# yancie-yjr/StreamYOLO

Hardware: AMD Instinct MI355X
Metric: frame-pairs/sec (600x960) StreamYOLO-l fwd+bwd (higher is better)
Workload: dtype bf16; 1 GPU; StreamYOLO-l 600x960 training step: dual-frame forward + TAL loss + backward, 8 frame pairs/GPU/step, random-init synthetic weights (utils/synth.py); per_gpu_batch=8, global_batch=8, parallelism=dp1, hipgraph=False, launch_tape=True, optimizer_in_step=False, u8_input=False

## Files before the change

include/streamyolo_hip.h:

```cpp
#ifndef STREAMYOLO_HIP_H
#define STREAMYOLO_HIP_H

#include <stdint.h>

#ifdef __cplusplus
extern "C" {
#endif

#define SY_ABI_VERSION 7
#define SY_API __attribute__((visibility("default")))

enum { SY_DT_BF16 = 0, SY_DT_F16 = 1, SY_DT_F32 = 2 };

enum {
    SY_EPI_LINEAR = 0,
    SY_EPI_SILU = 1,
    SY_EPI_SIGMOID = 2,
    SY_EPI_DECODE = 3,
    SY_EPI_BNR = 4
};

enum { SY_TILE_AUTO = 0, SY_TILE_256x256 = 1, SY_TILE_128x256 = 2, SY_TILE_128x128 = 3, SY_TILE_64x256 = 4, SY_TILE_32x256 = 5,
       SY_TILE_128x64 = 6, SY_TILE_64x64 = 7, SY_TILE_256x64 = 8, SY_TILE_256x128 = 9,
       SY_TILE_RS = 16,
       SY_TILE_DMA2 = 32,
       SY_TILE_DMA3 = 48,
       SY_TILE_WR = 80,
       SY_TILE_HALO = 112,
       SY_TILE_1X1K = 121  };

enum {
    SY_CONV_FWD = 0,
    SY_CONV_DGRAD = 1
};

typedef struct sy_conv_desc {
    const void* x;
    const void* w;
    const float* scale;
    const float* shift;
    const void* res;
    void* y;
    float* stat_sum;
    float* stat_sqsum;
    int32_t N, H, W, Cin;
    int32_t Ho, Wo, Cout;
    int32_t KH, KW, stride, pad;
    int32_t ldx, ldy, ldr;
    int64_t xbs, ybs, rbs;
    int32_t dtype;
    int32_t y_f32;
    int32_t mode;
    int32_t epilogue;
    int32_t accumulate;
    float dec_stride;
    int32_t stat_copies;
    int32_t stat_segments;
    int32_t tile;
    int64_t x_bytes, w_bytes;
    const void* wfrag;
    int64_t wfrag_bytes;
    int32_t k_splits;
    int32_t pre_cin;
    const void* pre_w;
    int64_t pre_w_bytes;
    const float* pre_scale;
    const float* pre_shift;
} sy_conv_desc;

SY_API int sy_conv2d(const sy_conv_desc* d, void* stream);

typedef struct sy_wgrad_desc {
    const void* x;  const void* dy;  float* dw;
    int32_t N, H, W, Cin, Ho, Wo, Cout, KH, KW, stride, pad;
    int32_t ldx, lddy;  int64_t xbs, dybs;
    int32_t dtype;
    int32_t dw_oihw;
    void* workspace;
    int64_t workspace_bytes;
    int32_t tile, target_blocks;
    int64_t x_bytes, dy_bytes;
} sy_wgrad_desc;
SY_API int sy_conv2d_wgrad(const sy_wgrad_desc* d, void* stream);

SY_API int sy_focus_pack(const float* in, int N, int Ctot, int c0, int H, int W, void* out, int dtype, void* stream);

enum { SY_FRAMES_NCHW = 0, SY_FRAMES_FOCUS = 1 };
SY_API int sy_frames_u8_pack(const uint8_t* cur, const uint8_t* sup, int B, int Hs, int Ws, int64_t image_stride,
                             int row_stride, int decimate, const uint8_t* mirror, int H, int W, int Ho, int Wo,
                             int layout, void* out_cur, void* out_sup, int dtype, void* stream);

SY_API int sy_resize_bilinear_nchw(const float* in, int N, int C, int H, int W, float* out, int Ho, int Wo, void* stream);

SY_API int sy_resize_nearest(const void* in, int N, int Hi, int Wi, int C, int ldi, int64_t ibs,
                      void* out, int Ho, int Wo, int ldo, int64_t obs, int dtype, void* stream);

SY_API int sy_spp_pool(void* buf, int N, int H, int W, int C, int ld, int64_t bs, void* argmax, int dtype,
                       void* stream);

SY_API int sy_head_decode(float* out, int B, int A, int nch, const int32_t* level_h, const int32_t* level_w,
                          const float* level_stride, int nlevels, int flags, void* stream);

SY_API int64_t sy_postprocess_workspace_bytes(int B, int A);
SY_API int sy_postprocess(const float* pred, int B, int A, int num_classes, float conf_thre, float nms_thre,
                   int max_det, float* out_det, int32_t* out_index, int32_t* out_count,
                   void* workspace, void* stream);

typedef struct sy_optim_entry {
    float* p;
    const float* g;
    float* buf;
    float* ema;
    int64_t n;
    float weight_decay;
    float lr_mult;
    int32_t chunk0;
    int32_t reserved;
} sy_optim_entry;
SY_API int sy_sgd_ema_step(const sy_optim_entry* entries, int n_entries, int total_chunks, float lr, float momentum,
                           float grad_scale, float ema_decay, int first_step, void* stream);

typedef struct sy_scaler_state {
    float scale;
    float inv_scale;
    int32_t growth_tracker;
    int32_t found_inf;
    int32_t steps_taken;
    int32_t steps_skipped;
    int32_t reserved[2];
} sy_scaler_state;
SY_API int sy_grad_nonfinite(const sy_optim_entry* entries, int n_entries, int total_chunks, void* scaler_state, void* stream);
SY_API int sy_sgd_ema_step_scaled(const sy_optim_entry* entries, int n_entries, int total_chunks, float lr, float momentum,
                                  float extra_scale, float ema_decay, const void* scaler_state, void* stream);
SY_API int sy_loss_scale_update(void* scaler_state, float growth_factor, float backoff_factor, int growth_interval, void* stream);

typedef struct sy_pack_entry {
    const float* w;
    void* packed;
    void* packed_t;
    void* frag;
    void* frag_t;
    int32_t co_n, ci_n, taps, r0, R, R_t, CI, dtype;
    int32_t tile0;
    int32_t reserved;
} sy_pack_entry;
SY_API int sy_pack_weights(const sy_pack_entry* entries, int n_entries, int total_tiles, void* stream);

SY_API int sy_bn_finalize(const float* sum, const float* sqsum, int C, int copies, double count, const float* gamma,
                   const float* beta, float eps, float momentum, float* running_mean,
                   float* running_var, float* scale, float* shift, float* mean, float* invstd,
                   int nseg, void* stream);
typedef struct sy_bn_running_entry {
    float* running_mean;
    float* running_var;
    const float* sum[2];
    const float* sqsum[2];
    double count[2];
    int32_t C, copies, calls;
    float momentum;
    int32_t ld;
    int32_t reserved;
    int64_t* num_batches_tracked;
} sy_bn_running_entry;
SY_API int sy_bn_running_update(const sy_bn_running_entry* entries, int n_entries, int max_C, void* stream);
SY_API int sy_bn_finalize_apply(const float* sum, const float* sqsum, int copies, double count, const float* gamma,
                                const float* beta, float eps, float* scale, float* shift, float* mean, float* invstd,
                                const void* y, int ldy, const void* res, int ldr, void* out, int ldo, int64_t pixels, int C,
                                int dtype, int nseg, void* stream);

SY_API int sy_bn_silu_apply(const void* y, int ldy, const float* scale, const float* shift, const void* res,
                     int ldr, void* out, int ldo, int64_t pixels, int C, int dtype, int nseg, void* stream);
SY_API int sy_bn_silu_bwd_reduce(const void* y, int ldy, const void* da, int ldda, const float* scale,
                                 const float* shift, const float* mean, const float* invstd, float* sums,
                                 int copies, int64_t pixels, int C, int dtype, int nseg, void* stream);
SY_API int sy_bn_silu_bwd_apply(const void* y, int ldy, const void* da, int ldda, const float* scale,
                                const float* shift, const float* mean, const float* invstd,
                                const float* gamma, const float* sums, int copies, void* dy, int lddy,
                                int64_t pixels, int C, float* dgamma, float* dbeta, void* dres, int lddres,
                                int dres_accumulate, int dtype, int nseg, void* stream);

SY_API int64_t sy_tal_loss_workspace_bytes(int B, int A, int max_gt);
SY_API int sy_tal_loss(const float* raw, int B, int A, int num_classes, const float* labels,
                       const float* support, int max_labels, const int32_t* level_h,
                       const int32_t* level_w, const float* level_stride, int nlevels, float gamma,
                       float ignore_thr, float ignore_value, int use_l1, float* d_raw, float* losses,
                       int32_t* fg_mask, void* workspace, void* d_pad, int pad_dtype, void* stream);
SY_API int sy_tal_loss_scaled(const float* raw, int B, int A, int num_classes, const float* labels,
                              const float* support, int max_labels, const int32_t* level_h,
                              const int32_t* level_w, const float* level_stride, int nlevels, float gamma,
                              float ignore_thr, float ignore_value, int use_l1, float* d_raw, float* losses,
                              int32_t* fg_mask, void* workspace, void* d_pad, int pad_dtype, const void* scaler_state,
                              void* stream);

SY_API int sy_tal_loss_assignment(const void* workspace, int B, int A, int max_labels, int32_t* matched_gt,
                                  float* matched_iou, void* stream);

SY_API int sy_bn_grid_caps(const int32_t* set4, int32_t* get4);

SY_API int sy_zero_rows(void* ptr, int64_t rows, int64_t row_bytes, int64_t pitch_bytes, void* stream);

SY_API int sy_view_copy(const void* in, int ldi, void* out, int ldo, int64_t pixels, int C, int dtype,
                 int accumulate, void* stream);

SY_API int sy_stream_state_gather(const void* cur, int ld_cur, int64_t cur_bs, const void* pool, int n_slots, void* sup,
                                  int ld_sup, int64_t sup_bs, int B, int H, int W, int C, const int32_t* row_slot,
                                  const uint8_t* row_first, int dtype, void* stream);
typedef struct sy_stream_level {
    const void* cur;
    void* pool;
    int64_t bs;
    int32_t H, W, C, ld;
} sy_stream_level;
SY_API int sy_stream_state_scatter(const sy_stream_level* levels, int n_levels, int n_slots, int B, const int32_t* row_slot,
                                   int dtype, void* stream);

SY_API int sy_resize_nearest_bwd(const void* dout, int N, int Ho, int Wo, int C, int lddo, int64_t dobs,
                          void* din, int Hi, int Wi, int lddi, int64_t dibs, int accumulate,
                          int dtype, void* stream);
SY_API int sy_spp_pool_bwd(void* dbuf, const void* argmax, int N, int H, int W, int C, int ld, int64_t bs,
                    int dtype, void* stream);

SY_API int sy_splitk_epilogue(const float* part, int splits, int64_t pixels, int C, const float* scale, const float* shift,
                              const void* res, int ldr, void* y, int ldy, int dtype, int epilogue, void* stream);

SY_API int sy_rows_add_f32(float* dst, int64_t ldd, float* src, int64_t lds, int rows, int cols, int zero_src, void* stream);
SY_API int64_t sy_pred_grad_fold_workspace_floats(int num_classes);
SY_API int sy_pred_grad_fold(const float* d_raw, int B, int64_t batch_stride, int rows, int num_classes, float* scratch,
                             int scratch_rows, int ld, int cin, float* g_reg, float* g_obj, float* g_cls, float* gb_reg, float* gb_obj, float* gb_cls,
                             float* workspace, void* stream);

enum { SY_TAPE_END = -1, SY_TAPE_LAUNCH = 0,
       SY_TAPE_SIDE = 1,
       SY_TAPE_FORK = 2,
       SY_TAPE_SIDE_NW = 3,
       SY_TAPE_MAIN = 4,
       SY_TAPE_ACQUIRE = 5,
       SY_TAPE_JOIN = 6,
       SY_TAPE_BREAK = 7,
       SY_TAPE_BUCKET = 8,
       SY_TAPE_CUR = 9,
       SY_TAPE_DEP = 10,
       SY_TAPE_SLOT_DONE = 11,
       SY_TAPE_ACQUIRE_CUR = 12   };
SY_API void* sy_tape_begin(void);
SY_API int sy_tape_mark(int kind, int arg);
SY_API void* sy_tape_end(void);
SY_API int sy_tape_size(const void* tape, int* n_entries, int* n_launches);
SY_API int sy_tape_counters(const void* tape, int* n_events, int* n_waits);
SY_API int sy_tape_replay(void* tape, void* main_stream, void* side_stream, int* pos, int stop_buckets, int* stop_kind,
                          int* stop_arg, int* stop_on_side);
SY_API int sy_tape_replay_n(void* tape, void* const* streams, int n_streams, int* pos, int stop_buckets, int* stop_kind,
                            int* stop_arg, int* stop_stream);
SY_API void sy_tape_free(void* tape);

SY_API const char* sy_version(void);
SY_API int sy_abi_version(void);

#ifdef __cplusplus
}
#endif
#endif
```

streamyolo_amd/_lib.py:

```python
import ctypes as C
import os

_HERE = os.path.dirname(os.path.abspath(__file__))
DEFAULT_PATH = os.path.join(_HERE, "lib", "libstreamyolo_hip.so")

DT_BF16, DT_F16, DT_F32 = 0, 1, 2
EPI_LINEAR, EPI_SILU, EPI_SIGMOID, EPI_DECODE, EPI_BNR = 0, 1, 2, 3, 4
CONV_FWD, CONV_DGRAD = 0, 1

ABI_VERSION = 7
_ERR = {1: "bad argument", 2: "kernel launch failed", 3: "unsupported shape"}
SY_ERR_UNSUPPORTED = 3


class HipLibraryError(RuntimeError):
    pass


class ConvDesc(C.Structure):
    _fields_ = [
        ("x", C.c_void_p), ("w", C.c_void_p), ("scale", C.c_void_p), ("shift", C.c_void_p),
        ("res", C.c_void_p), ("y", C.c_void_p), ("stat_sum", C.c_void_p), ("stat_sqsum", C.c_void_p),
        ("N", C.c_int32), ("H", C.c_int32), ("W", C.c_int32), ("Cin", C.c_int32),
        ("Ho", C.c_int32), ("Wo", C.c_int32), ("Cout", C.c_int32),
        ("KH", C.c_int32), ("KW", C.c_int32), ("stride", C.c_int32), ("pad", C.c_int32),
        ("ldx", C.c_int32), ("ldy", C.c_int32), ("ldr", C.c_int32),
        ("xbs", C.c_int64), ("ybs", C.c_int64), ("rbs", C.c_int64),
        ("dtype", C.c_int32), ("y_f32", C.c_int32), ("mode", C.c_int32), ("epilogue", C.c_int32),
        ("accumulate", C.c_int32), ("dec_stride", C.c_float), ("stat_copies", C.c_int32), ("stat_segments", C.c_int32), ("tile", C.c_int32), ("x_bytes", C.c_int64), ("w_bytes", C.c_int64), ("wfrag", C.c_void_p), ("wfrag_bytes", C.c_int64),
        ("k_splits", C.c_int32), ("pre_cin", C.c_int32), ("pre_w", C.c_void_p), ("pre_w_bytes", C.c_int64),
        ("pre_scale", C.c_void_p), ("pre_shift", C.c_void_p),
    ]


class BnRunningEntry(C.Structure):
    _fields_ = [("running_mean", C.c_void_p), ("running_var", C.c_void_p), ("sum", C.c_void_p * 2),
                ("sqsum", C.c_void_p * 2), ("count", C.c_double * 2), ("C", C.c_int32), ("copies", C.c_int32),
                ("calls", C.c_int32), ("momentum", C.c_float), ("ld", C.c_int32), ("reserved", C.c_int32),
                ("num_batches_tracked", C.c_void_p)]


class PackEntry(C.Structure):
    _fields_ = [("w", C.c_void_p), ("packed", C.c_void_p), ("packed_t", C.c_void_p), ("frag", C.c_void_p),
                ("frag_t", C.c_void_p), ("co_n", C.c_int32), ("ci_n", C.c_int32), ("taps", C.c_int32),
                ("r0", C.c_int32), ("R", C.c_int32), ("R_t", C.c_int32), ("CI", C.c_int32), ("dtype", C.c_int32),
                ("tile0", C.c_int32), ("reserved", C.c_int32)]


class ScalerState(C.Structure):
    _fields_ = [("scale", C.c_float), ("inv_scale", C.c_float), ("growth_tracker", C.c_int32), ("found_inf", C.c_int32),
                ("steps_taken", C.c_int32), ("steps_skipped", C.c_int32), ("reserved", C.c_int32 * 2)]


class OptimEntry(C.Structure):
    _fields_ = [("p", C.c_void_p), ("g", C.c_void_p), ("buf", C.c_void_p), ("ema", C.c_void_p), ("n", C.c_int64),
                ("weight_decay", C.c_float), ("lr_mult", C.c_float), ("chunk0", C.c_int32), ("reserved", C.c_int32)]


class StreamLevel(C.Structure):
    _fields_ = [("cur", C.c_void_p), ("pool", C.c_void_p), ("bs", C.c_int64), ("H", C.c_int32), ("W", C.c_int32),
                ("C", C.c_int32), ("ld", C.c_int32)]


def pack_table(rows):
    t = 0
    for e in rows:
        e.tile0 = t
        t += -(-e.co_n // 32) * -(-e.ci_n // 32)
    return (PackEntry * len(rows))(*rows), t


class WgradDesc(C.Structure):
    _fields_ = [
        ("x", C.c_void_p), ("dy", C.c_void_p), ("dw", C.c_void_p),
        ("N", C.c_int32), ("H", C.c_int32), ("W", C.c_int32), ("Cin", C.c_int32),
        ("Ho", C.c_int32), ("Wo", C.c_int32), ("Cout", C.c_int32),
        ("KH", C.c_int32), ("KW", C.c_int32), ("stride", C.c_int32), ("pad", C.c_int32),
        ("ldx", C.c_int32), ("lddy", C.c_int32), ("xbs", C.c_int64), ("dybs", C.c_int64),
        ("dtype", C.c_int32), ("dw_oihw", C.c_int32), ("workspace", C.c_void_p), ("workspace_bytes", C.c_int64), ("tile", C.c_int32), ("target_blocks", C.c_int32), ("x_bytes", C.c_int64), ("dy_bytes", C.c_int64),
    ]


_P, _I, _L, _F, _D = C.c_void_p, C.c_int, C.c_int64, C.c_float, C.c_double

SIGNATURES = {
    "sy_conv2d": (_I, [C.POINTER(ConvDesc), _P]),
    "sy_conv2d_wgrad": (_I, [C.POINTER(WgradDesc), _P]),
    "sy_focus_pack": (_I, [_P, _I, _I, _I, _I, _I, _P, _I, _P]),
    "sy_frames_u8_pack": (_I, [_P, _P, _I, _I, _I, _L, _I, _I, _P, _I, _I, _I, _I, _I, _P, _P, _I, _P]),
    "sy_resize_bilinear_nchw": (_I, [_P, _I, _I, _I, _I, _P, _I, _I, _P]),
    "sy_resize_nearest": (_I, [_P, _I, _I, _I, _I, _I, _L, _P, _I, _I, _I, _L, _I, _P]),
    "sy_resize_nearest_bwd": (_I, [_P, _I, _I, _I, _I, _I, _L, _P, _I, _I, _I, _L, _I, _I, _P]),
    "sy_spp_pool": (_I, [_P, _I, _I, _I, _I, _I, _L, _P, _I, _P]),
    "sy_spp_pool_bwd": (_I, [_P, _P, _I, _I, _I, _I, _I, _L, _I, _P]),
    "sy_postprocess_workspace_bytes": (_L, [_I, _I]),
    "sy_head_decode": (_I, [_P, _I, _I, _I, _P, _P, _P, _I, _I, _P]),
    "sy_postprocess": (_I, [_P, _I, _I, _I, _F, _F, _I, _P, _P, _P, _P, _P]),
    "sy_sgd_ema_step": (_I, [_P, _I, _I, _F, _F, _F, _F, _I, _P]),
    "sy_grad_nonfinite": (_I, [_P, _I, _I, _P, _P]),
    "sy_sgd_ema_step_scaled": (_I, [_P, _I, _I, _F, _F, _F, _F, _P, _P]),
    "sy_loss_scale_update": (_I, [_P, _F, _F, _I, _P]),
    "sy_pack_weights": (_I, [_P, _I, _I, _P]),
    "sy_bn_running_update": (_I, [_P, _I, _I, _P]),
    "sy_bn_finalize": (_I, [_P, _P, _I, _I, _D, _P, _P, _F, _F, _P, _P, _P, _P, _P, _P, _I, _P]),
    "sy_bn_silu_apply": (_I, [_P, _I, _P, _P, _P, _I, _P, _I, _L, _I, _I, _I, _P]),
    "sy_bn_finalize_apply": (_I, [_P, _P, _I, _D, _P, _P, _F, _P, _P, _P, _P, _P, _I, _P, _I, _P, _I, _L, _I, _I, _I, _P]),
    "sy_bn_silu_bwd_reduce": (_I, [_P, _I, _P, _I, _P, _P, _P, _P, _P, _I, _L, _I, _I, _I, _P]),
    "sy_bn_silu_bwd_apply": (_I, [_P, _I, _P, _I, _P, _P, _P, _P, _P, _P, _I, _P, _I, _L, _I, _P, _P, _P, _I, _I, _I, _I, _P]),
    "sy_tal_loss_workspace_bytes": (_L, [_I, _I, _I]),
    "sy_tal_loss": (_I, [_P, _I, _I, _I, _P, _P, _I, _P, _P, _P, _I, _F, _F, _F, _I, _P, _P, _P, _P, _P, _I, _P]),
    "sy_tal_loss_scaled": (_I, [_P, _I, _I, _I, _P, _P, _I, _P, _P, _P, _I, _F, _F, _F, _I, _P, _P, _P, _P, _P, _I, _P, _P]),
    "sy_tal_loss_assignment": (_I, [_P, _I, _I, _I, _P, _P, _P]),
    "sy_zero_rows": (_I, [_P, _L, _L, _L, _P]),
    "sy_bn_grid_caps": (_I, [C.POINTER(C.c_int32), C.POINTER(C.c_int32)]),
    "sy_view_copy": (_I, [_P, _I, _P, _I, _L, _I, _I, _I, _P]),
    "sy_stream_state_gather": (_I, [_P, _I, _L, _P, _I, _P, _I, _L, _I, _I, _I, _I, _P, _P, _I, _P]),
    "sy_stream_state_scatter": (_I, [_P, _I, _I, _I, _P, _I, _P]),
    "sy_splitk_epilogue": (_I, [_P, _I, _L, _I, _P, _P, _P, _I, _P, _I, _I, _I, _P]),
    "sy_rows_add_f32": (_I, [_P, _L, _P, _L, _I, _I, _I, _P]),
    "sy_pred_grad_fold_workspace_floats": (_L, [_I]),
    "sy_pred_grad_fold": (_I, [_P, _I, _L, _I, _I, _P, _I, _I, _I, _P, _P, _P, _P, _P, _P, _P, _P]),
    "sy_tape_begin": (_P, []),
    "sy_tape_mark": (_I, [_I, _I]),
    "sy_tape_end": (_P, []),
    "sy_tape_size": (_I, [_P, C.POINTER(C.c_int), C.POINTER(C.c_int)]),
    "sy_tape_counters": (_I, [_P, C.POINTER(C.c_int), C.POINTER(C.c_int)]),
    "sy_tape_replay": (_I, [_P, _P, _P, C.POINTER(C.c_int), _I, C.POINTER(C.c_int), C.POINTER(C.c_int), C.POINTER(C.c_int)]),
    "sy_tape_replay_n": (_I, [_P, C.POINTER(C.c_void_p), _I, C.POINTER(C.c_int), _I, C.POINTER(C.c_int), C.POINTER(C.c_int),
                               C.POINTER(C.c_int)]),
    "sy_tape_free": (None, [_P]),
    "sy_version": (C.c_char_p, []),
    "sy_abi_version": (_I, []),
}

_lib = None
_lib_path = None


def _bind(path):
    if not os.path.exists(path):
        raise HipLibraryError(
            "streamyolo_amd: %s not found. The MI355X kernels are the ONLY implementation of this "
            "package (no CPU/eager fallback). Build them: make -C streamyolo_amd/csrc" % path)
    lib = C.CDLL(path)
    for name, (res, args) in SIGNATURES.items():
        try:
            fn = getattr(lib, name)
        except AttributeError as e:
            raise HipLibraryError("streamyolo_amd: %s lacks symbol %s (stale build?)" % (path, name)) from e
        fn.restype = res
        fn.argtypes = args
    if lib.sy_abi_version() != ABI_VERSION:
        raise HipLibraryError("streamyolo_amd: ABI version mismatch in %s" % path)
    return lib


def lib():
    global _lib, _lib_path
    if _lib is None:
        path = os.environ.get("STREAMYOLO_HIP_LIB") or DEFAULT_PATH
        _lib = _bind(path)
        _lib_path = path
    return _lib if _tape is None else _TapeProxy(_lib, _tape)


_tape = None


class _TapeProxy:
    __slots__ = ("real", "tape")

    def __init__(self, real, tape):
        self.real, self.tape = real, tape

    def __getattr__(self, name):
        fn = getattr(self.real, name)
        tape = self.tape
        if name.endswith("_supported") or name.endswith("_bytes") or name.endswith("_floats") or name.endswith("version") or name.endswith("_caps") or name.startswith("sy_tape_"):
            return fn

        def call(*args):
            tape.append((fn, args[:-1], name))
            return fn(*args)
        return call


class record:

    def __enter__(self):
        global _tape
        assert _tape is None, "launch tapes do not nest"
        lib()
        _tape = []
        return _tape

    def __exit__(self, *exc):
        global _tape
        _tape = None
        return False


def replay(tape, stream):
    for fn, args, name in tape:
        rc = fn(*args, stream)
        if rc != 0:
            check(rc, name)


TAPE_END, TAPE_LAUNCH, TAPE_SIDE, TAPE_FORK, TAPE_SIDE_NW, TAPE_MAIN, TAPE_ACQUIRE, TAPE_JOIN, TAPE_BREAK, TAPE_BUCKET = \
    -1, 0, 1, 2, 3, 4, 5, 6, 7, 8
TAPE_CUR, TAPE_DEP, TAPE_SLOT_DONE, TAPE_ACQUIRE_CUR = 9, 10, 11, 12
TAPE_MARKS = {"side": TAPE_SIDE, "fork": TAPE_FORK, "side_nw": TAPE_SIDE_NW, "main": TAPE_MAIN, "acquire": TAPE_ACQUIRE,
              "join": TAPE_JOIN, "bucket": TAPE_BUCKET, "cur": TAPE_CUR, "dep": TAPE_DEP, "slot_done": TAPE_SLOT_DONE,
              "acquire_cur": TAPE_ACQUIRE_CUR}


class NativeTape:

    def __init__(self):
        self.handle, self.snippets, self._lib = None, [], lib()
        self._pos, self._kind, self._arg, self._side = C.c_int(0), C.c_int(0), C.c_int(0), C.c_int(0)

    def __enter__(self):
        assert _tape is None, "a Python launch tape is open"
        if not self._lib.sy_tape_begin():
            raise HipLibraryError("streamyolo_amd: sy_tape_begin failed (a recording is already open on this thread)")
        return self

    def __exit__(self, et, ev, tb):
        h = self._lib.sy_tape_end()
        if et is not None:
            self._lib.sy_tape_free(h)
        else:
            self.handle = h
        return False

    def mark(self, name, arg=None):
        if name == "dep":
            arg = arg[0] * 16 + arg[1]
        check(self._lib.sy_tape_mark(TAPE_MARKS[name], -1 if arg is None else int(arg)), "sy_tape_mark")

    def snippet(self, fn):
        self.snippets.append(fn)
        check(self._lib.sy_tape_mark(TAPE_BREAK, len(self.snippets) - 1), "sy_tape_mark")

    def size(self):
        n, l = C.c_int(0), C.c_int(0)
        check(self._lib.sy_tape_size(self.handle, C.byref(n), C.byref(l)), "sy_tape_size")
        return n.value, l.value

    def counters(self):
        e, w = C.c_int(0), C.c_int(0)
        check(self._lib.sy_tape_counters(self.handle, C.byref(e), C.byref(w)), "sy_tape_counters")
        return e.value, w.value

    def replay(self, main, side=None, on_snippet=None, on_bucket=None, more=()):
        fn, h = self._lib.sy_tape_replay_n, self.handle
        pos, kind, arg, ons = self._pos, self._kind, self._arg, self._side
        pos.value = 0
        stop_b = 0 if on_bucket is None else 1
        lst = [main] + ([side] if side is not None else []) + (list(more) if side is not None else [])
# ... 58 lines not shown
```

streamyolo_amd/csrc/conv_igemm.hip:

```cpp
#include "conv_igemm_impl.h"

using sy_conv::ConvArgs;
int sy_conv_launch_bf16(const ConvArgs& a, void* stream);
int sy_conv_launch_f16(const ConvArgs& a, void* stream);
int sy_conv_launch_f32(const ConvArgs& a, void* stream);

constexpr long long kWtMinBytes = 8ll << 20;

extern "C" int sy_conv2d(const sy_conv_desc* d, void* stream) {
    if (d == nullptr || d->x == nullptr || d->w == nullptr || d->y == nullptr) return SY_ERR_ARG;
    if (d->N <= 0 || d->Cin <= 0 || d->Cout <= 0 || d->Ho <= 0 || d->Wo <= 0) return SY_ERR_ARG;
    if (d->dtype < SY_DT_BF16 || d->dtype > SY_DT_F32) return SY_ERR_ARG;
    const int epc = d->dtype == SY_DT_F32 ? 4 : 8;
    if (d->Cin % epc != 0 || d->ldx % epc != 0) return SY_ERR_UNSUPPORTED;
    if (d->stride != 1 && d->stride != 2) return SY_ERR_UNSUPPORTED;
    if (d->KH < 1 || d->KW < 1 || d->KH * d->KW > 49) return SY_ERR_UNSUPPORTED;
    if ((d->stat_sum == nullptr) != (d->stat_sqsum == nullptr)) return SY_ERR_ARG;
    if (d->epilogue < SY_EPI_LINEAR || d->epilogue > SY_EPI_BNR) return SY_ERR_ARG;
    if (d->epilogue == SY_EPI_BNR) {
        if (d->mode != SY_CONV_DGRAD || d->accumulate || d->y_f32 || d->dtype == SY_DT_F32 || d->res == nullptr || d->scale == nullptr ||
            d->shift == nullptr || d->stat_sum == nullptr || d->ldr != d->ldy || d->rbs != d->ybs || d->stat_segments > 1)
            return SY_ERR_UNSUPPORTED;
        const int t = d->tile & 0xff;
        if (t != 98 && t != 100 && t != 101 && t != 109 && t != 104 && t != 107 && t != 117 && t != 118) return SY_ERR_UNSUPPORTED;
        if (d->KH != 3 || d->stride != 1 || (d->ldy & 7) != 0 || (d->Cout & 7) != 0) return SY_ERR_UNSUPPORTED;
        if ((((uintptr_t)d->y | (uintptr_t)d->res) & 15) != 0 || (d->ybs & 7) != 0) return SY_ERR_UNSUPPORTED;
    }
    if ((long long)d->N * d->Ho * d->Wo > 0x7fffffffLL) return SY_ERR_UNSUPPORTED;
    ConvArgs a;
    a.x = (const unsigned char*)d->x; a.w = (const unsigned char*)d->w;
    a.scale = d->scale; a.shift = d->shift; a.res = (const unsigned char*)d->res; a.y = (unsigned char*)d->y;
    a.stat_sum = d->stat_sum; a.stat_sq = d->stat_sqsum;
    a.N = d->N; a.H = d->H; a.W = d->W; a.Cin = d->Cin; a.Ho = d->Ho; a.Wo = d->Wo; a.Cout = d->Cout;
    a.KH = d->KH; a.KW = d->KW; a.stride = d->stride; a.pad = d->pad;
    a.ldx = d->ldx; a.ldy = d->ldy; a.ldr = d->ldr; a.xbs = d->xbs; a.ybs = d->ybs; a.rbs = d->rbs;
    a.y_f32 = d->y_f32; a.mode = d->mode; a.epilogue = d->epilogue; a.accumulate = d->accumulate;
    a.dec_stride = d->dec_stride;
    a.stat_copies = d->stat_copies > 0 ? d->stat_copies : 1;
    a.seg_M = 0;
    a.s2_classes = 0;
    if (d->stat_segments > 1) {
        if (d->stat_sum == nullptr || d->N % d->stat_segments != 0 || d->mode != SY_CONV_FWD) return SY_ERR_ARG;
        a.seg_M = (d->N / d->stat_segments) * d->Ho * d->Wo;
    }
    a.x_extent = (d->x_bytes > 0 && d->x_bytes < 0xFFFFFFF0LL) ? (unsigned)d->x_bytes : 0u;
    a.w_extent = (d->w_bytes > 0 && d->w_bytes < 0xFFFFFFF0LL) ? (unsigned)d->w_bytes : 0u;
    a.wfrag = (const unsigned char*)d->wfrag;
    a.wfrag_extent = (d->wfrag != nullptr && d->wfrag_bytes > 0 && d->wfrag_bytes < 0xFFFFFFF0LL) ? (unsigned)d->wfrag_bytes : 0u;
    a.pre_w = (const unsigned char*)d->pre_w; a.pre_scale = d->pre_scale; a.pre_shift = d->pre_shift; a.pre_cin = d->pre_cin;
    a.pre_w_extent = (d->pre_w != nullptr && d->pre_w_bytes > 0 && d->pre_w_bytes < 0xFFFFFFF0LL) ? (unsigned)d->pre_w_bytes : 0u;
    if ((d->pre_w != nullptr) != ((d->tile & 0xff) == 119)) return SY_ERR_ARG;
    a.ksplit = 0;
    if (d->k_splits > 1) {
        if (((d->tile & 0xff) != 117 && (d->tile & 0xff) != 118) || d->mode != SY_CONV_FWD || !d->y_f32 || d->epilogue != SY_EPI_LINEAR ||
            d->scale != nullptr || d->shift != nullptr || d->res != nullptr || d->stat_sum != nullptr || d->accumulate || d->k_splits > 16)
            return SY_ERR_UNSUPPORTED;
        a.ksplit = d->k_splits;
    }
    {
        static const long long wt_min = [] { const char* e = std::getenv("SY_WT_MIN_BYTES"); return e ? std::atoll(e) : (long long)kWtMinBytes; }();
        const long long out_bytes = (long long)d->N * d->Ho * d->Wo * d->Cout * (d->y_f32 ? 4 : (d->dtype == SY_DT_F32 ? 4 : 2));
        a.wt = out_bytes >= wt_min ? 1 : 0;
    }
    a.tile = d->tile & 0xff;
    a.ablate = (d->tile >> 8) & 1023;
    a.HoWo = d->Ho * d->Wo; a.M = d->N * a.HoWo; a.K = d->KH * d->KW * d->Cin;
    switch (d->dtype) {
        case SY_DT_BF16: return sy_conv_launch_bf16(a, stream);
        case SY_DT_F16: return sy_conv_launch_f16(a, stream);
        default: return sy_conv_launch_f32(a, stream);
    }
}
```

streamyolo_amd/csrc/conv_igemm_impl.h:

```cpp
#pragma once
#include "sy_device.h"
#include "../../include/streamyolo_hip.h"

namespace sy_conv {

struct ConvArgs {
    const unsigned char* x;
    const unsigned char* w;
    const float* scale;
    const float* shift;
    const unsigned char* res;
    unsigned char* y;
    float* stat_sum;
    float* stat_sq;
    int N, H, W, Cin, Ho, Wo, Cout, KH, KW, stride, pad;
    int ldx, ldy, ldr;
    long long xbs, ybs, rbs;
    int y_f32, mode, epilogue, accumulate;
    float dec_stride;
    int M, K, HoWo;
    int stat_copies;
    int seg_M;
    int s2_classes;
    int tile;
    unsigned x_extent, w_extent;
    const unsigned char* wfrag;
    unsigned wfrag_extent;
    const unsigned char* pre_w;
    unsigned pre_w_extent;
    const float* pre_scale;
    const float* pre_shift;
    int pre_cin;
    int ksplit;
    int wt;
    int ablate;
};

template <int WC, int WP, int TC, int TP> struct StageLimit { static constexpr size_t kBytes = 48 * 1024; };

template <int WP, int CT> struct EpiLds { static constexpr int kStatBytes = WP * CT * 8; };

constexpr int kRowB = 64;
constexpr int kPitchRS = 80;

static __device__ uint4 g_zero16[4] = {};

struct LinearPixels {
    int m0, m_end, cls_hw, Wc, Wo, cls_ph, cls_pw, s2, seg, rep;
    template <typename Args> __device__ __forceinline__ LinearPixels(const Args& p, int by, int bz, int PT) {
        cls_ph = 0; cls_pw = 0; Wc = p.Wo; Wo = p.Wo; s2 = p.s2_classes;
        int Hc = p.Ho, cls_M = p.M;
        if (p.s2_classes) {
            cls_ph = bz >> 1; cls_pw = bz & 1;
            Hc = (p.Ho - cls_ph + 1) >> 1; Wc = (p.Wo - cls_pw + 1) >> 1;
            cls_M = p.N * Hc * Wc;
        }
        cls_hw = Hc * Wc;
        m_end = p.seg_M > 0 ? (bz + 1) * p.seg_M : cls_M;
        m0 = (p.s2_classes ? 0 : bz * p.seg_M) + by * PT;
        seg = bz; rep = by;
    }
    __device__ __forceinline__ bool map(int lp, int& n, int& rem) const {
        const int m = m0 + lp;
        if (m >= m_end) { n = 0; rem = 0; return false; }
        n = m / cls_hw;
        rem = m - n * cls_hw;
        if (s2) { const int i2 = rem / Wc; rem = (2 * i2 + cls_ph) * Wo + 2 * (rem - i2 * Wc) + cls_pw; }
        return true;
    }
};
struct TilePixels {
    int n, h0, w0, Ho, Wo, seg, rep;
    __device__ __forceinline__ bool map(int lp, int& n_, int& rem) const {
        const int h = h0 + (lp >> 5), w = w0 + (lp & 31);
        n_ = n;
        if (h >= Ho || w >= Wo) { rem = 0; return false; }
        rem = h * Wo + w;
        return true;
    }
};

template <typename T, int WC, int WP, int TC, int TP, typename Args, typename Map>
__device__ __forceinline__ void conv_epilogue(const Args& p, const Map& mp, int bx, f32x16 (&acc)[TC][TP],
                                              unsigned char* smem, int tid);

template <typename T, int WC, int WP, int TC, int TP, int STG, int FAST>
__global__ __launch_bounds__(WC * WP * 64, ((TC * TP <= 4 && !(STG == 6 && TC * TP == 4)) ? 4 : 2)) void conv_igemm_kernel(ConvArgs p) {
    SY_TL_BEGIN(1 + (p.mode == SY_CONV_DGRAD ? 32 : 0));
    typedef typename T::elem elem;
    constexpr int RS = (STG == 1 || STG == 5 || STG == 6) ? 1 : 0;
    constexpr int WR = (STG == 5 || STG == 6) ? 1 : 0;
    constexpr int WR3 = (STG == 6) ? 1 : 0;
    constexpr int kStages = RS ? 1 : (STG == 0 ? 4 : STG);
    constexpr int kThreads = WC * WP * 64;
    constexpr int RPI = kThreads / 4;
    constexpr int EPC = T::kEPC;
    constexpr int ESZ = 16 / EPC;
    constexpr int BK = 4 * EPC;
    constexpr int CT = WC * TC * 32;
    constexpr int PT = WP * TP * 32;
    constexpr int WCH = (CT * 4 + kThreads - 1) / kThreads;
    constexpr int XCH = (PT * 4 + kThreads - 1) / kThreads;
    static_assert(WC * WP == 4 || WC * WP == 8, "4 or 8 waves per workgroup");
    static_assert(PT % RPI == 0, "every wave stages pixel rows");

    SY_DYN_SMEM(smem);
    unsigned char* const sW = smem;
    unsigned char* const sX = smem + (WR ? 0 : (RS ? CT * kPitchRS : kStages * CT * kRowB));

    const int tid = threadIdx.x;
    const int lane = tid & 63;
    const int wave = tid >> 6;
    const int wc = wave / WP;
    const int wp = wave % WP;
    const sy_block_id bid = sy_xcd_block_id();
    const int c0 = bid.x * CT;
    int cls_ph = 0, cls_pw = 0, Hc = p.Ho, Wc = p.Wo, cls_M = p.M;
    if (p.s2_classes) {
// ... 675 lines not shown
                if (l31 == 16) {
                    red[(wp * CT + cl) * 2 + 0] = a;
                    red[(wp * CT + cl) * 2 + 1] = b;
                }
            }
        }
    });
    if (want_stats || (kCanStage && stage_out)) __syncthreads();
    sy_probe(4);
    if (kCanStage && stage_out && !p.accumulate) {
        constexpr int CPR = CT / 8;
        constexpr int NCH = (PT * CPR + kThreads - 1) / kThreads;
        constexpr int UB = NCH < 5 ? NCH : 5;
#pragma unroll 1
        for (int b0 = 0; b0 < NCH; b0 += UB) {
            uint4 v[UB];
            long long off[UB];
#pragma unroll
            for (int k = 0; k < UB; ++k) {
                const int i = tid + (b0 + k) * kThreads;
                const int ck = i % CPR;
                const bool ok = i < PT * CPR && c0 + ck * 8 < p.Cout;
                const int px = ok ? i / CPR : 0;
                const long long o_ = stg_off[px];
                v[k] = *reinterpret_cast<const uint4*>(stg + px * kStagePitch + ck * 16);
                off[k] = ok ? o_ : -1;
            }
#pragma unroll
            for (int k = 0; k < UB; ++k) {
                const int i = tid + (b0 + k) * kThreads;
                const int ck = i % CPR;
                if (off[k] >= 0) {
                    if (SY_WT_CONV && p.wt) sy_store16_wt(reinterpret_cast<elem*>(p.y) + off[k] + c0 + ck * 8, v[k]);
                    else *reinterpret_cast<uint4*>(reinterpret_cast<elem*>(p.y) + off[k] + c0 + ck * 8) = v[k];
                }
            }
        }
    } else if (kCanStage && stage_out) {
        constexpr int CPR = CT / 8;
        for (int i = tid; i < PT * CPR; i += kThreads) {
            const int px = i / CPR, ck = i - px * CPR;
            const long long off = stg_off[px];
            const int co = c0 + ck * 8;
            if (off < 0 || co >= p.Cout) continue;
            uint4 v = *reinterpret_cast<const uint4*>(stg + px * kStagePitch + ck * 16);
            uint4* const dst = reinterpret_cast<uint4*>(reinterpret_cast<elem*>(p.y) + off + co);
            if (p.accumulate) {
                const uint4 o = *dst;
                elem ev[8], eo[8];
                __builtin_memcpy(ev, &v, 16);
                __builtin_memcpy(eo, &o, 16);
                unsigned w[4];
#pragma unroll
                for (int j = 0; j < 4; ++j)
                    w[j] = T::pack2(T::to_f32(ev[2 * j]) + T::to_f32(eo[2 * j]), T::to_f32(ev[2 * j + 1]) + T::to_f32(eo[2 * j + 1]));
                v = make_uint4(w[0], w[1], w[2], w[3]);
            }
            if (SY_WT_CONV && p.wt) sy_store16_wt(dst, v); else *dst = v;
        }
    }
    sy_probe(5);
    if (bnr && lean) {
        const float* red = reinterpret_cast<const float*>(smem);
        float* const dst = p.stat_sum + (long long)((unsigned)mp.rep % (unsigned)p.stat_copies) * 2 * p.Cout;
        for (int cl = tid; cl < CT; cl += kThreads) {
            const int co = c0 + cl;
            if (co >= p.Cout) continue;
            float a = 0.0f, b = 0.0f;
#pragma unroll
            for (int w = 0; w < WP; ++w) { a += red[(w * CT + cl) * 2]; b += red[(w * CT + cl) * 2 + 1]; }
            atomicAdd(dst + co, a);
            atomicAdd(dst + p.Cout + co, b);
        }
    }
    if (want_stats && !(p.ablate & 8)) {
        const float* red = reinterpret_cast<const float*>(smem);
        const int copy = mp.seg * p.stat_copies + (int)((unsigned)mp.rep % (unsigned)p.stat_copies);
        for (int cl = tid; cl < CT; cl += kThreads) {
            const int co = c0 + cl;
            if (co >= p.Cout) continue;
            float a = 0.0f, b = 0.0f;
#pragma unroll
            for (int w = 0; w < WP; ++w) { a += red[(w * CT + cl) * 2]; b += red[(w * CT + cl) * 2 + 1]; }
            atomicAdd(p.stat_sum + (long long)copy * p.Cout + co, a);
            atomicAdd(p.stat_sq + (long long)copy * p.Cout + co, b);
        }
    }
}

template <typename T, int WC, int WP, int TC, int TP, int STG, int FAST>
int launch_one(const ConvArgs& a, void* stream) {
    constexpr int RS = (STG == 1 || STG == 5 || STG == 6) ? 1 : 0;
    constexpr int kStages = RS ? 1 : (STG == 0 ? 4 : STG);
    constexpr int CT = WC * TC * 32, PT = WP * TP * 32;
    const int nseg = a.seg_M > 0 ? a.M / a.seg_M : 1;
    dim3 grid((a.Cout + CT - 1) / CT, ((a.seg_M > 0 ? a.seg_M : a.M) + PT - 1) / PT, nseg);
    if (a.s2_classes) grid = dim3(grid.x, (a.N * ((a.Ho + 1) / 2) * ((a.Wo + 1) / 2) + PT - 1) / PT, 4);
    constexpr size_t smem_k = (STG == 6) ? (size_t)(2 * PT * kPitchRS > WP * CT * 8 ? 2 * PT * kPitchRS : WP * CT * 8)
                              : (STG == 5) ? (size_t)(PT * kPitchRS > WP * CT * 8 ? PT * kPitchRS : WP * CT * 8)
                                         : (RS ? (size_t)(CT + PT) * kPitchRS : (size_t)kStages * (CT + PT) * kRowB);
    constexpr size_t smem_e = (size_t)EpiLds<WP, CT>::kStatBytes + (size_t)PT * (CT * 2 + 16) + (size_t)PT * 8;
    constexpr size_t smem = (T::kEPC == 8 && smem_e <= 48 * 1024 && smem_e > smem_k) ? smem_e : smem_k;
#ifndef SY_EMU
    static sy_dev_once attr_done;
    if (attr_done.need()) {
        if (hipFuncSetAttribute((const void*)conv_igemm_kernel<T, WC, WP, TC, TP, STG, FAST>,
                                hipFuncAttributeMaxDynamicSharedMemorySize, (int)smem) != hipSuccess)
            return SY_ERR_LAUNCH;
        attr_done.mark();
    }
#endif
    SY_LAUNCH((conv_igemm_kernel<T, WC, WP, TC, TP, STG, FAST>), grid, dim3(WC * WP * 64), smem, stream, a);
    return SY_LAUNCH_OK() == 0 ? SY_OK : SY_ERR_LAUNCH;
}

template <typename T, int WC, int WP, int TC, int TP, int STG = 0>
int launch_cfg(const ConvArgs& a_in, void* stream) {
    ConvArgs a = a_in;
    const bool fast = (a.Cin % (4 * T::kEPC) == 0) && a.x_extent != 0 && a.w_extent != 0 && a.KH * a.KW <= 32;
    a.s2_classes = (fast && a.mode != SY_CONV_FWD && a.stride == 2 && a.KH >= 2 && a.KW >= 2 && !(a_in.ablate & 4)) ? 1 : 0;
    if constexpr (STG == 5 || STG == 6) {
        if (fast && a.wfrag != nullptr && a.wfrag_extent != 0) return launch_one<T, WC, WP, TC, TP, STG, 1>(a, stream);
        return fast ? launch_one<T, WC, WP, TC, TP, 1, 1>(a, stream) : launch_one<T, WC, WP, TC, TP, 1, 0>(a, stream);
    } else {
        return fast ? launch_one<T, WC, WP, TC, TP, STG, 1>(a, stream) : launch_one<T, WC, WP, TC, TP, STG, 0>(a, stream);
    }
}

template <typename T> int launch_halo_typed(const ConvArgs& a, void* stream);
template <typename T> int launch_halo3_typed(const ConvArgs& a, void* stream);
template <typename T> int launch_s2dgrad(const ConvArgs& a, void* stream);
template <typename T> int launch_s2dgrad4(const ConvArgs& a, void* stream);
template <typename T> int launch_1x1_tile(const ConvArgs& a, void* stream);
template <typename T> int launch_bottleneck_fused(const ConvArgs& a, void* stream);

template <typename T>
int launch_typed(const ConvArgs& a, void* stream) {
    if ((a.tile >= 104 && a.tile <= 107) || (a.tile >= 110 && a.tile <= 118)) return launch_halo_typed<T>(a, stream);
    if (a.tile == 109 || (a.tile >= 96 && a.tile <= 98) || a.tile == 100 || a.tile == 101) return launch_halo3_typed<T>(a, stream);
    if (a.tile == 119) return launch_bottleneck_fused<T>(a, stream);
    if (a.tile == 108) return launch_s2dgrad<T>(a, stream);
    if (a.tile >= 125 && a.tile <= 127) return launch_s2dgrad4<T>(a, stream);
    if (a.tile >= 121 && a.tile <= 124) return launch_1x1_tile<T>(a, stream);
    switch (a.tile) {
        case SY_TILE_256x256: return launch_cfg<T, 2, 4, 4, 2>(a, stream);
        case SY_TILE_128x256: return launch_cfg<T, 1, 8, 4, 1>(a, stream);
        case SY_TILE_128x128: return launch_cfg<T, 2, 2, 2, 2>(a, stream);
        case SY_TILE_64x256: return launch_cfg<T, 1, 4, 2, 2>(a, stream);
        case SY_TILE_32x256: return launch_cfg<T, 1, 4, 1, 2>(a, stream);
        case SY_TILE_128x64: return launch_cfg<T, 4, 1, 1, 2>(a, stream);
        case SY_TILE_64x64: return launch_cfg<T, 2, 2, 1, 1>(a, stream);
        case SY_TILE_RS + SY_TILE_128x64: return launch_cfg<T, 4, 1, 1, 2, 1>(a, stream);
        case SY_TILE_RS + SY_TILE_64x64: return launch_cfg<T, 2, 2, 1, 1, 1>(a, stream);
        case 32 + SY_TILE_128x128: return launch_cfg<T, 2, 2, 2, 2, 2>(a, stream);
        case 32 + SY_TILE_128x64: return launch_cfg<T, 4, 1, 1, 2, 2>(a, stream);
        case 32 + SY_TILE_64x64: return launch_cfg<T, 2, 2, 1, 1, 2>(a, stream);
        case 32 + SY_TILE_64x256: return launch_cfg<T, 1, 4, 2, 2, 2>(a, stream);
        case 48 + SY_TILE_128x128: return launch_cfg<T, 2, 2, 2, 2, 3>(a, stream);
        case 48 + SY_TILE_128x64: return launch_cfg<T, 4, 1, 1, 2, 3>(a, stream);
        case 48 + SY_TILE_64x64: return launch_cfg<T, 2, 2, 1, 1, 3>(a, stream);
        case 48 + SY_TILE_64x256: return launch_cfg<T, 1, 4, 2, 2, 3>(a, stream);
        case SY_TILE_RS + SY_TILE_256x64: return launch_cfg<T, 4, 1, 2, 2, 1>(a, stream);
        case 80 + SY_TILE_256x64: return launch_cfg<T, 4, 1, 2, 2, 5>(a, stream);
        case 80 + SY_TILE_256x128: return launch_cfg<T, 4, 1, 2, 4, 5>(a, stream);
        case 80 + SY_TILE_128x128: return launch_cfg<T, 2, 2, 2, 2, 5>(a, stream);
        case 80 + SY_TILE_128x64: return launch_cfg<T, 4, 1, 1, 2, 5>(a, stream);
        case 96 + SY_TILE_128x64: return launch_cfg<T, 4, 1, 1, 2, 6>(a, stream);
        case 96 + SY_TILE_64x64: return launch_cfg<T, 2, 2, 1, 1, 6>(a, stream);
// ... 21 lines not shown
```

streamyolo_amd/csrc/sy_device.h:

```cpp
#pragma once

#ifdef SY_EMU
#include "simt_emu.h"
#define SY_DYN_SMEM(name) unsigned char* name = emu::g_blk->dyn_smem
#include "sy_tape.h"
#include <tuple>
#define SY_LAUNCH(kernel, grid, block, smem, stream, ...)                                                            \
    do {                                                                                                             \
        const dim3 sy_grid_ = (grid), sy_block_ = (block);                                                           \
        const size_t sy_smem_ = (smem);                                                                              \
        auto sy_args_ = std::make_tuple(__VA_ARGS__);                            \
        auto sy_launch_fn_ = [=](void*) {                                                                            \
            emu::launch(sy_grid_, sy_block_, sy_smem_,                                                               \
                        [=]() { std::apply([](auto... sy_a_) { kernel(sy_a_...); }, sy_args_); });                   \
        };                                                                                                           \
        if (sy_tape_recording()) sy_tape_push(std::function<void(void*)>(sy_launch_fn_));                            \
        sy_launch_fn_(nullptr);                                                                                      \
    } while (0)
#define SY_LAUNCH_OK() 0
#else
#include <hip/hip_runtime.h>
#include <hip/hip_ext.h>
#define SY_DYN_SMEM(name) extern __shared__ __attribute__((aligned(16))) unsigned char name[]
#include "sy_tape.h"
// ... 288 lines not shown
        const float send = b2 ? A : B;
        w2[m] = (b2 ? B : A) + sy_mov_dpp<0x114, 0xA>(sy_mov_dpp<0x104, 0x5>(0.0f, send), send);
    }
    const float A = w2[0], B = w2[1];
    const float send = b3 ? A : B;
    const float r = (b3 ? B : A) + sy_mov_dpp<0x118, 0xC>(sy_mov_dpp<0x108, 0x3>(0.0f, send), send);
    return r + __shfl_xor(r, 16);
}
#endif

#ifdef SY_EMU
static inline void sy_sched_fence() {}
#else
__device__ __forceinline__ void sy_sched_fence() { __builtin_amdgcn_sched_barrier(0); }
#endif

#ifdef SY_EMU
static inline int sy_uniform(int v) { return v; }
#else
__device__ __forceinline__ int sy_uniform(int v) { return __builtin_amdgcn_readfirstlane(v); }
#endif

#ifdef SY_EMU
static inline unsigned long long sy_readlane64(unsigned long long v, int l) { return __shfl(v, l); }
#else
__device__ __forceinline__ unsigned long long sy_readlane64(unsigned long long v, int l) {
    const unsigned lo = __builtin_amdgcn_readlane((unsigned)v, l), hi = __builtin_amdgcn_readlane((unsigned)(v >> 32), l);
    return ((unsigned long long)hi << 32) | lo;
}
#endif

#ifndef SY_WT_STORES
#define SY_WT_STORES 1
#endif
#ifndef SY_WT_CONV
#define SY_WT_CONV 1
#endif
#ifndef SY_WT_BNF
#define SY_WT_BNF 1
#endif
#ifndef SY_WT_BNB
#define SY_WT_BNB 1
#endif
#ifndef SY_WT_SLAB
#define SY_WT_SLAB 0
#endif
#ifndef SY_WT_FOLD
#define SY_WT_FOLD 0
#endif
#ifndef SY_WT_ZERO
#define SY_WT_ZERO 0
#endif
#if defined(SY_EMU) || !SY_WT_STORES
static inline __host__ __device__ void sy_store16_wt(void* dst, const uint4& v) { *reinterpret_cast<uint4*>(dst) = v; }
static inline __host__ __device__ void sy_store8_wt(void* dst, const uint2& v) { *reinterpret_cast<uint2*>(dst) = v; }
static inline __host__ __device__ void sy_store4_wt(void* dst, unsigned v) { *reinterpret_cast<unsigned*>(dst) = v; }
#else
__device__ __forceinline__ void sy_store8_wt(void* dst, const uint2& v) {
    typedef unsigned v2u __attribute__((ext_vector_type(2)));
    v2u d;
    __builtin_memcpy(&d, &v, 8);
    asm volatile("global_store_dwordx2 %0, %1, off sc1" : : "v"(dst), "v"(d) : "memory");
}
__device__ __forceinline__ void sy_store4_wt(void* dst, unsigned v) {
    asm volatile("global_store_dword %0, %1, off sc1" : : "v"(dst), "v"(v) : "memory");
}
__device__ __forceinline__ void sy_store16_wt(void* dst, const uint4& v) {
    typedef unsigned v4u __attribute__((ext_vector_type(4)));
    v4u d;
    __builtin_memcpy(&d, &v, 16);
    asm volatile("global_store_dwordx4 %0, %1, off sc1\n\ts_nop 1" : : "v"(dst), "v"(d) : "memory");
}
#endif

#ifdef SY_EMU
static inline unsigned long long sy_uniform64(unsigned long long v) { return v; }
#else
__device__ __forceinline__ unsigned long long sy_uniform64(unsigned long long v) {
    const unsigned lo = __builtin_amdgcn_readfirstlane((unsigned)v), hi = __builtin_amdgcn_readfirstlane((unsigned)(v >> 32));
    return ((unsigned long long)hi << 32) | lo;
}
#endif

struct sy_block_id { int x, y, z; };
__device__ __forceinline__ sy_block_id sy_xcd_block_id() {
    constexpr unsigned kXcd = 8;
    const unsigned gx = gridDim.x, gy = gridDim.y, gz = gridDim.z;
    const unsigned nwg = gx * gy * gz;
    const unsigned w = blockIdx.x + gx * (blockIdx.y + gy * blockIdx.z);
    const unsigned k = w % kXcd, q = nwg / kXcd, r = nwg % kXcd;
    const unsigned L = k * q + (k < r ? k : r) + w / kXcd;
    sy_block_id b;
    b.x = (int)(L % gx);
    b.y = (int)((L / gx) % gy);
    b.z = (int)(L / (gx * gy));
    return b;
}

#if defined(SY_PROBE) && !defined(SY_EMU)
constexpr int kProbeWG = 8192, kProbeSlots = 8;
static __device__ unsigned long long sy_probe_buf[kProbeWG * kProbeSlots];
__device__ __forceinline__ void sy_probe(int slot) {
    if (threadIdx.x == 0) {
        const unsigned w = blockIdx.x + gridDim.x * (blockIdx.y + gridDim.y * blockIdx.z);
        if (w < (unsigned)kProbeWG) sy_probe_buf[w * kProbeSlots + slot] = __builtin_amdgcn_s_memrealtime();
    }
}
struct sy_tl_entry { unsigned long long key, t0, t1; unsigned tag, count; };
constexpr int kTlSlots = 65536;
static __device__ sy_tl_entry sy_tl[kTlSlots];
__device__ __forceinline__ int sy_tl_begin(unsigned tag) {
    const unsigned w = blockIdx.x + gridDim.x * (blockIdx.y + gridDim.y * blockIdx.z);
    const unsigned nwg = gridDim.x * gridDim.y * gridDim.z;
    const bool first = w == 0;
    const bool sample = first || (w & 15u) == 15u || w + 4u >= nwg;
    if (!sample || threadIdx.x != 0) return -1;
    const unsigned long long key = (unsigned long long)__builtin_amdgcn_kernarg_segment_ptr();
    const unsigned h = (unsigned)((key >> 6) * 2654435761ull) & (unsigned)(kTlSlots - 1);
    if (first) {
        const unsigned long long t = __builtin_amdgcn_s_memrealtime();
        const unsigned long long old = atomicCAS(&sy_tl[h].key, 0ull, key);
        if (old != 0ull && old != key) return -1;
        sy_tl[h].t0 = t;
        sy_tl[h].tag = tag;
        sy_tl[h].count = nwg;
        return (int)h;
    }
    return __hip_atomic_load(&sy_tl[h].key, __ATOMIC_RELAXED, __HIP_MEMORY_SCOPE_AGENT) == key ? (int)h : -1;
}
__device__ __forceinline__ void sy_tl_end(int slot) {
    if (slot >= 0) atomicMax(&sy_tl[slot].t1, (unsigned long long)__builtin_amdgcn_s_memrealtime());
}
#define SY_TL_BEGIN(tag) const int sy_tl_slot_ = sy_tl_begin(tag)
#define SY_TL_END() sy_tl_end(sy_tl_slot_)
#define SY_PROBE_READER(name)                                                                                          \
    extern "C" __attribute__((visibility("default"))) int name(unsigned long long* dst, int clear) {                 \
        if (hipMemcpyFromSymbol(dst, HIP_SYMBOL(sy_probe_buf), sizeof(sy_probe_buf)) != hipSuccess) return 2;          \
        if (clear) { static unsigned long long z[kProbeWG * kProbeSlots]; (void)hipMemcpyToSymbol(HIP_SYMBOL(sy_probe_buf), z, sizeof(z)); } \
        return 0;                                                                                                    \
    }                                                                                                                \
    extern "C" __attribute__((visibility("default"))) int name##_tl(void* dst, int clear) {                          \
        if (hipMemcpyFromSymbol(dst, HIP_SYMBOL(sy_tl), sizeof(sy_tl)) != hipSuccess) return 2;                       \
        if (clear) {                                                                                                 \
            static sy_tl_entry z[kTlSlots];                                                                          \
            for (int i = 0; i < kTlSlots; ++i) { z[i].key = 0; z[i].t0 = ~0ull; z[i].t1 = 0; z[i].tag = 0; z[i].count = 0; } \
            (void)hipMemcpyToSymbol(HIP_SYMBOL(sy_tl), z, sizeof(z));                                                \
        }                                                                                                            \
        return 0;                                                                                                    \
    }
#else
#define sy_probe(slot) ((void)0)
#define SY_PROBE_READER(name)
#define SY_TL_BEGIN(tag) ((void)0)
#define SY_TL_END() ((void)0)
#endif

#ifdef SY_EMU
#define SY_LATE_ARGS(Type, p) const Type& p##_late = (p)
#define SY_LAUNDER_INT(x) ((void)0)
#else
#define SY_LATE_ARGS(Type, p)                                                                                       \
    const __attribute__((address_space(4))) Type* p##_late_ptr =                                                     \
        (const __attribute__((address_space(4))) Type*)__builtin_amdgcn_kernarg_segment_ptr();                      \
    asm volatile("" : "+s"(p##_late_ptr));                                                                          \
    const __attribute__((address_space(4))) Type& p##_late = *p##_late_ptr
#define SY_LAUNDER_INT(x) asm volatile("" : "+s"(x))
// ... 29 lines not shown
```

streamyolo_amd/csrc/train_ops.hip:

```cpp
#include <stdlib.h>
#include "sy_pointwise.h"

#ifndef SY_BN_ROWS_IN_FLIGHT
#define SY_BN_ROWS_IN_FLIGHT 2
#endif

namespace {

template <typename T>
__global__ __launch_bounds__(kBlock) void spp_pool_kernel(typename T::elem* buf, int N, int H, int W, int C, int ld,
                                                          long long bs, unsigned char* argmax) {
    const int cpp = C / T::kEPC;
    const long long total = (long long)N * H * W * cpp;
    for (long long i = (long long)blockIdx.x * kBlock + threadIdx.x; i < total; i += (long long)gridDim.x * kBlock) {
        const int cc = (int)(i % cpp);
        long long pix = i / cpp;
        const int w = (int)(pix % W);
        const int h = (int)((pix / W) % H);
        const int n = (int)(pix / ((long long)W * H));
        float m5[T::kEPC], m9[T::kEPC], m13[T::kEPC];
        unsigned char a5[T::kEPC], a9[T::kEPC], a13[T::kEPC];
#pragma unroll
        for (int j = 0; j < T::kEPC; ++j) { m5[j] = -INFINITY; m9[j] = -INFINITY; m13[j] = -INFINITY; a5[j] = 0; a9[j] = 0; a13[j] = 0; }
        const typename T::elem* base = buf + n * bs + cc * T::kEPC;
// ... 207 lines not shown
        const int l = i / HW, p = i - l * HW;
        const int w = p % W, hr = p / W;
        const int r = 2 * (l + 1);
        float t[E];
        unsigned char rec[E];
#pragma unroll
        for (int j = 0; j < E; ++j) { t[j] = 0.0f; rec[j] = 0xFF; }
        for (int dh = -r; dh <= r; ++dh) {
            const int h = hr - dh;
            if (h < 0 || h >= H) continue;
            const int q = h * W + w;
            unsigned char cb[E];
            __builtin_memcpy(cb, s_am + ((size_t)q * 3 + l) * E, E);
            Chunk<T> g = Chunk<T>::load(s_g + ((size_t)q * 3 + l) * 16);
            const int code0 = (dh + 6) * 13;
#pragma unroll
            for (int j = 0; j < E; ++j) {
                const unsigned d = (unsigned)((int)cb[j] - code0);
                if (d < 13u) { t[j] += T::to_f32(g.e[j]); rec[j] = (unsigned char)d; }
            }
        }
        __builtin_memcpy(s_T + (size_t)i * E, t, sizeof(t));
        __builtin_memcpy(s_dw + (size_t)i * E, rec, E);
    }
    __syncthreads();
    for (int p = threadIdx.x; p < HW; p += nt) {
        const int x = p % W, row = p - x;
        elem* gslot0 = base + (long long)p * ld;
        Chunk<T> g0 = Chunk<T>::load(gslot0);
        float acc[E];
#pragma unroll
        for (int j = 0; j < E; ++j) acc[j] = T::to_f32(g0.e[j]);
#pragma unroll
        for (int l = 0; l < 3; ++l) {
            const int r = 2 * (l + 1);
            for (int dw = -r; dw <= r; ++dw) {
                const int w = x - dw;
                if (w < 0 || w >= W) continue;
                const size_t i = (size_t)l * HW + row + w;
                unsigned char rec[E];
                float t[E];
                __builtin_memcpy(rec, s_dw + i * E, E);
                __builtin_memcpy(t, s_T + i * E, sizeof(t));
#pragma unroll
                for (int j = 0; j < E; ++j)
                    if (rec[j] == (unsigned char)(dw + 6)) acc[j] += t[j];
            }
        }
        Chunk<T> o;
#pragma unroll
        for (int j = 0; j < E; ++j) o.e[j] = T::from_f32(acc[j]);
        o.store(gslot0);
    }
    SY_TL_END();
}

constexpr int kFoldTo = 32, kFoldAbove = 64;
__global__ __launch_bounds__(kBlock) void fold_rows_kernel(float* a0, float* a1, int C, int copies) {
    __shared__ float part[4][64];
    float* const arr = (blockIdx.z & 1) ? a1 : a0;
    float* const base = arr + (long long)(blockIdx.z >> 1) * copies * C;
    const int cl = threadIdx.x & 63, q = threadIdx.x >> 6;
    const int c = blockIdx.x * 64 + cl, r = blockIdx.y;
    float acc = 0.0f;
    if (c < C) {
        int j = q;
        const int J = (copies - r + kFoldTo - 1) / kFoldTo;
        for (; j + 12 < J; j += 16) {
            const float v0 = base[(long long)(r + kFoldTo * j) * C + c], v1 = base[(long long)(r + kFoldTo * (j + 4)) * C + c];
            const float v2 = base[(long long)(r + kFoldTo * (j + 8)) * C + c], v3 = base[(long long)(r + kFoldTo * (j + 12)) * C + c];
            acc += v0; acc += v1; acc += v2; acc += v3;
        }
        for (; j < J; j += 4) acc += base[(long long)(r + kFoldTo * j) * C + c];
    }
    part[q][cl] = acc;
    __syncthreads();
    if (q == 0 && c < C) base[(long long)r * C + c] = ((part[0][cl] + part[1][cl]) + part[2][cl]) + part[3][cl];
}

__global__ __launch_bounds__(kBlock) void bn_finalize_kernel(const float* sum, const float* sqsum, int C, int copies, int stride,
                                                             double count, const float* gamma, const float* beta,
                                                             float eps, float momentum, float* running_mean,
                                                             float* running_var, float* scale, float* shift,
                                                             float* mean_out, float* invstd_out) {
    SY_TL_BEGIN(11);
    __shared__ float s_s[8][32], s_q[8][32];
    const int cl = threadIdx.x & 31, rg = threadIdx.x >> 5;
    const int c = blockIdx.x * 32 + cl;
    {
        const long long so = (long long)blockIdx.y * stride * C, ao = (long long)blockIdx.y * C;
        sum += so; sqsum += so; scale += ao; shift += ao;
        if (mean_out != nullptr) mean_out += ao;
        if (invstd_out != nullptr) invstd_out += ao;
    }
    float s = 0.0f, q = 0.0f;
    if (c < C)
        for (int k = rg; k < copies; k += 8) { s += sum[(long long)k * C + c]; q += sqsum[(long long)k * C + c]; }
    s_s[rg][cl] = s;
    s_q[rg][cl] = q;
    __syncthreads();
    if (rg != 0 || c >= C) return;
    double ds = 0.0, dq = 0.0;
    for (int k = 0; k < 8; ++k) { ds += (double)s_s[k][cl]; dq += (double)s_q[k][cl]; }
    const double mean = ds / count;
    double var = dq / count - mean * mean;
    if (var < 0.0) var = 0.0;
    const float invstd = (float)(1.0 / sqrt(var + (double)eps));
    const float sc = gamma[c] * invstd;
    scale[c] = sc;
    shift[c] = beta[c] - (float)mean * sc;
    if (mean_out != nullptr) mean_out[c] = (float)mean;
    if (invstd_out != nullptr) invstd_out[c] = invstd;
    if (running_mean != nullptr) {
        const double unbiased = count > 1.0 ? var * count / (count - 1.0) : var;
        running_mean[c] = (1.0f - momentum) * running_mean[c] + momentum * (float)mean;
        running_var[c] = (1.0f - momentum) * running_var[c] + momentum * (float)unbiased;
    }
    SY_TL_END();
}

__global__ __launch_bounds__(kBlock) void bn_running_update_kernel(const sy_bn_running_entry* entries) {
    SY_TL_BEGIN(15);
    __shared__ float s_s[8][32], s_q[8][32];
    const sy_bn_running_entry e = entries[blockIdx.x];
    const int cl = threadIdx.x & 31, rg = threadIdx.x >> 5;
    const int c = blockIdx.y * 32 + cl;
    if ((int)blockIdx.y * 32 >= e.C) return;
    float rm = 0.0f, rv = 0.0f;
    const long long ld = e.ld > 0 ? e.ld : e.C;
    if (rg == 0 && c < e.C) { rm = e.running_mean[c]; rv = e.running_var[c]; }
    for (int j = 0; j < e.calls; ++j) {
        float s = 0.0f, q = 0.0f;
        if (c < e.C)
            for (int k = rg; k < e.copies; k += 8) { s += e.sum[j][k * ld + c]; q += e.sqsum[j][k * ld + c]; }
        s_s[rg][cl] = s;
        s_q[rg][cl] = q;
        __syncthreads();
        if (rg == 0 && c < e.C) {
            double ds = 0.0, dq = 0.0;
            for (int k = 0; k < 8; ++k) { ds += (double)s_s[k][cl]; dq += (double)s_q[k][cl]; }
            const double count = e.count[j];
            const double mean = ds / count;
            double var = dq / count - mean * mean;
            if (var < 0.0) var = 0.0;
            const double unbiased = count > 1.0 ? var * count / (count - 1.0) : var;
            rm = (1.0f - e.momentum) * rm + e.momentum * (float)mean;
            rv = (1.0f - e.momentum) * rv + e.momentum * (float)unbiased;
        }
        __syncthreads();
    }
    if (rg == 0 && c < e.C) { e.running_mean[c] = rm; e.running_var[c] = rv; }
    if (blockIdx.y == 0 && threadIdx.x == 0 && e.num_batches_tracked != nullptr) *e.num_batches_tracked += e.calls;
    SY_TL_END();
}

template <typename T>
__global__ __launch_bounds__(kBlock) void bn_silu_apply_kernel(const typename T::elem* y, int ldy, const float* scale,
                                                               const float* shift, const typename T::elem* res, int ldr,
                                                               typename T::elem* out, int ldo, long long pixels, int C) {
    SY_TL_BEGIN(10);
    const int cpp = C / T::kEPC;
    const int cc = threadIdx.x % cpp;
    const int c0 = cc * T::kEPC;
    const int rows = kBlock / cpp;
    if ((int)threadIdx.x >= rows * cpp) return;
    {
        const long long ro = (long long)blockIdx.y * pixels;
        y += ro * ldy; out += ro * ldo; scale += blockIdx.y * C; shift += blockIdx.y * C;
        if (res != nullptr) res += ro * ldr;
    }
    const long long step = (long long)gridDim.x * rows;
    long long pix = (long long)blockIdx.x * rows + threadIdx.x / cpp;
    constexpr int D = SY_BN_ROWS_IN_FLIGHT;
    Chunk<T> vq[D], rq[D];
#pragma unroll
    for (int d = 0; d < D; ++d) {
        const long long pd = pix + d * step;
        if (pd < pixels) {
            vq[d] = Chunk<T>::load(y + pd * ldy + c0);
            if (res != nullptr) rq[d] = Chunk<T>::load(res + pd * ldr + c0);
        }
    }
    float sc[T::kEPC], sh[T::kEPC];
#pragma unroll
    for (int j = 0; j < T::kEPC; ++j) { sc[j] = scale[c0 + j]; sh[j] = shift[c0 + j]; }
    for (; pix < pixels; pix += step) {
        const Chunk<T> v = vq[0], rv = rq[0];
#pragma unroll
        for (int d = 0; d + 1 < D; ++d) { vq[d] = vq[d + 1]; rq[d] = rq[d + 1]; }
        const long long nxt = pix + D * step;
        if (nxt < pixels) {
            vq[D - 1] = Chunk<T>::load(y + nxt * ldy + c0);
            if (res != nullptr) rq[D - 1] = Chunk<T>::load(res + nxt * ldr + c0);
        }
        Chunk<T> o;
        float r[T::kEPC];
#pragma unroll
        for (int j = 0; j < T::kEPC; ++j) r[j] = res != nullptr ? T::to_f32(rv.e[j]) : 0.0f;
#pragma unroll
        for (int j = 0; j < T::kEPC; ++j) o.e[j] = T::from_f32(sy_silu(T::to_f32(v.e[j]) * sc[j] + sh[j]) + r[j]);
        if constexpr (SY_WT_BNF) o.store_wt(out + pix * ldo + c0); else o.store(out + pix * ldo + c0);
    }
    SY_TL_END();
}

template <typename T>
__global__ __launch_bounds__(kBlock) void bn_finalize_apply_kernel(const float* sum, const float* sqsum, int copies, double count,
                                                                   const float* gamma, const float* beta, float eps,
                                                                   float* scale, float* shift, float* mean_out,
                                                                   float* invstd_out, const typename T::elem* y, int ldy,
                                                                   const typename T::elem* res, int ldr,
                                                                   typename T::elem* out, int ldo, long long pixels, int C,
                                                                   int CS) {
    SY_TL_BEGIN(10);
    __shared__ float s_part[2][8][64];
    __shared__ float s_aff[2][64];
    const int cpp = CS / T::kEPC;
    const int rows = kBlock / cpp;
    const int cc = threadIdx.x % cpp;
    const int cb = blockIdx.z * CS;
    const int c0 = cb + cc * T::kEPC;
    {
        const long long ro = (long long)blockIdx.y * pixels;
        const long long so = (long long)blockIdx.y * copies * C;
        const int ao = blockIdx.y * C;
        y += ro * ldy; out += ro * ldo;
        if (res != nullptr) res += ro * ldr;
        sum += so; sqsum += so; scale += ao; shift += ao; mean_out += ao; invstd_out += ao;
    }
    const bool live = (int)threadIdx.x < rows * cpp;
    const long long step = (long long)gridDim.x * rows;
    long long pix = (long long)blockIdx.x * rows + threadIdx.x / cpp;
    Chunk<T> v, rv, vn, rn;
    if (live && pix < pixels) {
        v = Chunk<T>::load(y + pix * ldy + c0);
        if (res != nullptr) rv = Chunk<T>::load(res + pix * ldr + c0);
    }
    for (int it = threadIdx.x; it < 2 * 8 * CS; it += kBlock) {
        const int c = it % CS, rg = (it / CS) & 7, kind = it / (8 * CS);
        const float* src = (kind ? sqsum : sum) + cb + c;
        float a = 0.0f;
        for (int k = rg; k < copies; k += 8) a += src[(long long)k * C];
        s_part[kind][rg][c] = a;
    }
    __syncthreads();
    if ((int)threadIdx.x < CS) {
        const int c = threadIdx.x;
        double ds = 0.0, dq = 0.0;
        for (int k = 0; k < 8; ++k) { ds += (double)s_part[0][k][c]; dq += (double)s_part[1][k][c]; }
        const double mean = ds / count;
        double var = dq / count - mean * mean;
        if (var < 0.0) var = 0.0;
        const float invstd = (float)(1.0 / sqrt(var + (double)eps));
        const float sc = gamma[cb + c] * invstd;
        const float sh = beta[cb + c] - (float)mean * sc;
        s_aff[0][c] = sc;
        s_aff[1][c] = sh;
        if (blockIdx.x == 0) {
            scale[cb + c] = sc; shift[cb + c] = sh; mean_out[cb + c] = (float)mean; invstd_out[cb + c] = invstd;
        }
    }
    __syncthreads();
    if (!live) return;
    float sc[T::kEPC], sh[T::kEPC];
#pragma unroll
    for (int j = 0; j < T::kEPC; ++j) { sc[j] = s_aff[0][cc * T::kEPC + j]; sh[j] = s_aff[1][cc * T::kEPC + j]; }
    for (; pix < pixels; pix += step) {
        const long long nxt = pix + step;
        if (nxt < pixels) {
            vn = Chunk<T>::load(y + nxt * ldy + c0);
            if (res != nullptr) rn = Chunk<T>::load(res + nxt * ldr + c0);
        }
        Chunk<T> o;
        float r[T::kEPC];
#pragma unroll
        for (int j = 0; j < T::kEPC; ++j) r[j] = res != nullptr ? T::to_f32(rv.e[j]) : 0.0f;
#pragma unroll
        for (int j = 0; j < T::kEPC; ++j) o.e[j] = T::from_f32(sy_silu(T::to_f32(v.e[j]) * sc[j] + sh[j]) + r[j]);
        if constexpr (SY_WT_BNF) o.store_wt(out + pix * ldo + c0); else o.store(out + pix * ldo + c0);
        v = vn; rv = rn;
    }
    SY_TL_END();
}

template <typename T>
__global__ __launch_bounds__(kBlock) void bn_silu_bwd_reduce_kernel(const typename T::elem* y, int ldy,
                                                                    const typename T::elem* da, int ldda,
                                                                    const float* scale, const float* shift,
                                                                    const float* mean, const float* invstd, float* sums,
                                                                    long long pixels, int C, int CS, int copies) {
    SY_TL_BEGIN(12);
    __shared__ float red[kBlock * 2 * 8];
    const int cpp = CS / T::kEPC;
    const int rows = kBlock / cpp;
    const int cc = threadIdx.x % cpp;
    const int pr = threadIdx.x / cpp;
    const int cb = blockIdx.z * CS;
    const int c0 = cb + cc * T::kEPC;
    {
        const long long ro = (long long)blockIdx.y * pixels;
        const int ao = blockIdx.y * C;
        y += ro * ldy; da += ro * ldda; scale += ao; shift += ao; mean += ao; invstd += ao;
        sums += (long long)blockIdx.y * copies * 2 * C;
    }
    sy_probe(0);
    const long long first = pr < rows ? (long long)blockIdx.x * rows + pr : pixels;
    const long long step = (long long)gridDim.x * rows;
    constexpr int D = SY_BN_ROWS_IN_FLIGHT;
    Chunk<T> yq[D], gq[D];
#pragma unroll
    for (int d = 0; d < D; ++d) {
        const long long pd = first + d * step;
        if (pd < pixels) { yq[d] = Chunk<T>::load(y + pd * ldy + c0); gq[d] = Chunk<T>::load(da + pd * ldda + c0); }
    }
    float sc[T::kEPC], sh[T::kEPC], mu[T::kEPC], is[T::kEPC], s0[T::kEPC], s1[T::kEPC];
#pragma unroll
    for (int j = 0; j < T::kEPC; ++j) {
        sc[j] = scale[c0 + j]; sh[j] = shift[c0 + j]; mu[j] = mean[c0 + j]; is[j] = invstd[c0 + j];
        s0[j] = 0.0f; s1[j] = 0.0f;
    }
    sy_probe(1);
    for (long long pix = first; pix < pixels; pix += step) {
        const Chunk<T> yv = yq[0], gv = gq[0];
#pragma unroll
        for (int d = 0; d + 1 < D; ++d) { yq[d] = yq[d + 1]; gq[d] = gq[d + 1]; }
        const long long nxt = pix + D * step;
        if (nxt < pixels) { yq[D - 1] = Chunk<T>::load(y + nxt * ldy + c0); gq[D - 1] = Chunk<T>::load(da + nxt * ldda + c0); }
#pragma unroll
        for (int j = 0; j < T::kEPC; ++j) {
            const float yy = T::to_f32(yv.e[j]);
            const float dz = T::to_f32(gv.e[j]) * sy_silu_grad(yy * sc[j] + sh[j]);
            s0[j] += dz;
            s1[j] += dz * ((yy - mu[j]) * is[j]);
        }
    }
    sy_probe(3);
#pragma unroll
    for (int j = 0; j < T::kEPC; ++j) {
        red[(j * 2 + 0) * kBlock + threadIdx.x] = s0[j];
        red[(j * 2 + 1) * kBlock + threadIdx.x] = s1[j];
    }
    __syncthreads();
    for (int t = threadIdx.x; t < cpp * T::kEPC * 2; t += kBlock) {
        const int kind = t & 1, j = (t >> 1) % T::kEPC, ch = (t >> 1) / T::kEPC;
        float v = 0.0f;
        for (int r = 0; r < rows; ++r) v += red[(j * 2 + kind) * kBlock + r * cpp + ch];
        atomicAdd(sums + (long long)(blockIdx.x % copies) * 2 * C + kind * C + cb + ch * T::kEPC + j, v);
    }
    sy_probe(6);
    SY_TL_END();
}

template <typename T>
__global__ __launch_bounds__(kBlock) void bn_silu_bwd_apply_kernel(const typename T::elem* y, int ldy,
                                                                   const typename T::elem* da, int ldda,
                                                                   const float* scale, const float* shift,
                                                                   const float* mean, const float* invstd,
                                                                   const float* gamma, const float* sums,
                                                                   typename T::elem* dy, int lddy, long long pixels,
                                                                   int C, int copies, float* dgamma, float* dbeta,
                                                                   long long seg_sum_stride, typename T::elem* dres,
                                                                   int lddres, int dres_acc) {
    SY_TL_BEGIN(13);
    __shared__ float s_fold[2 * 1024];
    {
        const long long ro = (long long)blockIdx.y * pixels;
        const int ao = blockIdx.y * C;
        y += ro * ldy; da += ro * ldda; dy += ro * lddy; scale += ao; shift += ao; mean += ao; invstd += ao;
        sums += blockIdx.y * seg_sum_stride;
        if (dres != nullptr) dres += ro * lddres;
    }
    const int cpp = C / T::kEPC;
    const int rows = kBlock / cpp;
    const int cc = threadIdx.x % cpp;
    const int c0 = cc * T::kEPC;
    const float inv_m = 1.0f / (float)pixels;
    const long long step = (long long)gridDim.x * rows;
    long long pix = (long long)blockIdx.x * rows + threadIdx.x / cpp;
    const bool live = (int)threadIdx.x < rows * cpp;
    constexpr int D = SY_BN_ROWS_IN_FLIGHT;
    Chunk<T> yq[D], gq[D];
#pragma unroll
    for (int d = 0; d < D; ++d) {
        const long long pd = pix + d * step;
        if (live && pd < pixels) { yq[d] = Chunk<T>::load(y + pd * ldy + c0); gq[d] = Chunk<T>::load(da + pd * ldda + c0); }
    }
    for (int i = threadIdx.x; i < 2 * C; i += kBlock) {
        float a = 0.0f;
        for (int k = 0; k < copies; ++k) a += sums[(long long)k * 2 * C + i];
        s_fold[i] = a;
    }
    __syncthreads();
    if (dres_acc & 4) {
        for (int c = threadIdx.x; c < C; c += kBlock)
            s_fold[C + c] = (float)((double)invstd[c] * ((double)s_fold[C + c] - (double)mean[c] * (double)s_fold[c]));
        __syncthreads();
    }
    if (blockIdx.x == 0 && dgamma != nullptr) {
        if (gridDim.y == 1 && !(dres_acc & 2)) {
            for (int c = threadIdx.x; c < C; c += kBlock) { dbeta[c] += s_fold[c]; dgamma[c] += s_fold[C + c]; }
        } else {
            for (int c = threadIdx.x; c < C; c += kBlock) { atomicAdd(dbeta + c, s_fold[c]); atomicAdd(dgamma + c, s_fold[C + c]); }
        }
    }
    if ((int)threadIdx.x >= rows * cpp) return;
    float sc[T::kEPC], sh[T::kEPC], mu[T::kEPC], is[T::kEPC], gi[T::kEPC], m0[T::kEPC], m1[T::kEPC];
#pragma unroll
    for (int j = 0; j < T::kEPC; ++j) {
        const int c = c0 + j;
        sc[j] = scale[c]; sh[j] = shift[c]; mu[j] = mean[c]; is[j] = invstd[c];
        gi[j] = gamma[c] * invstd[c];
        m0[j] = s_fold[c] * inv_m;
        m1[j] = s_fold[C + c] * inv_m;
    }
    for (; pix < pixels; pix += step) {
        Chunk<T> yv = yq[0], gv = gq[0];
#pragma unroll
        for (int d = 0; d + 1 < D; ++d) { yq[d] = yq[d + 1]; gq[d] = gq[d + 1]; }
        const long long nxt = pix + D * step;
        if (nxt < pixels) { yq[D - 1] = Chunk<T>::load(y + nxt * ldy + c0); gq[D - 1] = Chunk<T>::load(da + nxt * ldda + c0); }
        Chunk<T> o;
#pragma unroll
        for (int j = 0; j < T::kEPC; ++j) {
            const float yy = T::to_f32(yv.e[j]);
            const float dz = T::to_f32(gv.e[j]) * sy_silu_grad(yy * sc[j] + sh[j]);
            o.e[j] = T::from_f32(gi[j] * (dz - m0[j] - (yy - mu[j]) * is[j] * m1[j]));
        }
        if constexpr (SY_WT_BNB) o.store_wt(dy + pix * lddy + c0); else o.store(dy + pix * lddy + c0);
        if (dres != nullptr) {
            typename T::elem* dst = dres + pix * lddres + c0;
            if (dres_acc & 1) {
                Chunk<T> r = Chunk<T>::load(dst);
#pragma unroll
                for (int j = 0; j < T::kEPC; ++j) gv.e[j] = T::from_f32(T::to_f32(gv.e[j]) + T::to_f32(r.e[j]));
            }
            if constexpr (SY_WT_BNB) gv.store_wt(dst); else gv.store(dst);
        }
    }
    SY_TL_END();
}

__global__ __launch_bounds__(kBlock) void fold_replicas_kernel(float* sums, int n, int copies) {
    __shared__ float part[4][64];
    const int el = threadIdx.x & 63, q = threadIdx.x >> 6;
    const int i = blockIdx.x * 64 + el;
    sums += (long long)blockIdx.y * copies * n;
    float a = 0.0f;
    if (i < n) {
        int k = q;
        for (; k + 12 < copies; k += 16) {
            const float v0 = sums[(long long)k * n + i], v1 = sums[(long long)(k + 4) * n + i];
            const float v2 = sums[(long long)(k + 8) * n + i], v3 = sums[(long long)(k + 12) * n + i];
            a += v0; a += v1; a += v2; a += v3;
        }
        for (; k < copies; k += 4) a += sums[(long long)k * n + i];
    }
    part[q][el] = a;
    __syncthreads();
    if (q == 0 && i < n) sums[i] = ((part[0][el] + part[1][el]) + part[2][el]) + part[3][el];
}

inline bool chunk_rows_ok(int C, int e) { const int cpp = C / e; return cpp >= 1 && cpp <= kBlock; }

inline int env_cap(const char* name, int dflt) {
    const char* v = getenv(name);
    return (v != nullptr && atoi(v) > 0) ? atoi(v) : dflt;
}

enum { kCapApply = 0, kCapFApply = 1, kCapReduce = 2, kCapBApply = 3 };
inline std::atomic<int>& bn_cap(int which) {
    static std::atomic<int> caps[4] = {{env_cap("SY_BN_APPLY_BLOCKS", 2048)}, {env_cap("SY_BN_FAPPLY_BLOCKS", 2048)},
                                       {env_cap("SY_BN_REDUCE_BLOCKS", 768)}, {env_cap("SY_BN_BAPPLY_BLOCKS", 1024)}};
    return caps[which];
}

inline int row_grid(long long pixels, int C, int e, int cap) {
    const int rows = kBlock / (C / e);
    long long b = (pixels + rows - 1) / rows;
    if (b > cap) b = cap;
    if (b < 1) b = 1;
    return (int)b;
}

constexpr size_t kSppTileLds = 144 * 1024;
inline bool spp_force_scan() { const char* v = getenv("SY_SPP_SCAN"); return v != nullptr && v[0] == '1'; }
inline bool spp_lds_ok(const void* fn, int slot) {
#ifdef SY_EMU
    return true;
#else
    static sy_dev_once done[6];
    if (done[slot].need()) {
        if (hipFuncSetAttribute(fn, hipFuncAttributeMaxDynamicSharedMemorySize, (int)kSppTileLds) != hipSuccess) return false;
        done[slot].mark();
    }
    return true;
#endif
}

}

extern "C" int sy_bn_grid_caps(const int32_t* set4, int32_t* get4) {
    for (int k = 0; k < 4; ++k) {
        if (set4 != nullptr && set4[k] > 0) bn_cap(k).store(set4[k], std::memory_order_relaxed);
        if (get4 != nullptr) get4[k] = bn_cap(k).load(std::memory_order_relaxed);
    }
    return SY_OK;
}

extern "C" int sy_spp_pool(void* buf, int N, int H, int W, int C, int ld, int64_t bs, void* argmax, int dtype,
                           void* stream) {
    if (buf == nullptr || N <= 0 || C <= 0 || ld < 4 * C) return SY_ERR_ARG;
    const int e = epc_of(dtype);
    if (C % e || ld % e) return SY_ERR_UNSUPPORTED;
    const long long work = (long long)N * H * W * (C / e);
    const size_t tile_lds = (size_t)H * W * (16 + 3 * 16 + 3 * e);
    if (tile_lds <= kSppTileLds && !spp_force_scan()) {
        SY_DISPATCH_DTYPE(dtype, if (!spp_lds_ok((const void*)spp_pool_tile_kernel<T>, T::kCode)) return SY_ERR_LAUNCH;
                          SY_LAUNCH((spp_pool_tile_kernel<T>), dim3(N * (C / e), N * (C / e) < 256 ? 3 : 1), dim3(spp_tile_threads((long long)H * W)), tile_lds, stream,
                                    (typename T::elem*)buf, H, W, C, ld, (long long)bs, (unsigned char*)argmax));
    }
    SY_DISPATCH_DTYPE(dtype, SY_LAUNCH((spp_pool_kernel<T>), dim3(grid_for(work)), dim3(kBlock), 0, stream,
                                       (typename T::elem*)buf, N, H, W, C, ld, (long long)bs, (unsigned char*)argmax));
}

extern "C" int sy_spp_pool_bwd(void* dbuf, const void* argmax, int N, int H, int W, int C, int ld, int64_t bs, int dtype,
                               void* stream) {
    if (argmax == nullptr || dbuf == nullptr || N <= 0 || C <= 0 || ld < 4 * C) return SY_ERR_ARG;
    const int e = epc_of(dtype);
    if (C % e || ld % e) return SY_ERR_UNSUPPORTED;
    const long long work = (long long)N * H * W * (C / e);
    const size_t tile_lds = (size_t)H * W * 3 * (16 + e + 4 * e + e);
    if (tile_lds <= kSppTileLds && !spp_force_scan()) {
        SY_DISPATCH_DTYPE(dtype, if (!spp_lds_ok((const void*)spp_pool_bwd_tile_kernel<T>, 3 + T::kCode)) return SY_ERR_LAUNCH;
                          SY_LAUNCH((spp_pool_bwd_tile_kernel<T>), dim3(N * (C / e)), dim3(spp_tile_threads(3LL * H * W)), tile_lds, stream,
                                    (typename T::elem*)dbuf, (const unsigned char*)argmax, H, W, C, ld, (long long)bs));
    }
    SY_DISPATCH_DTYPE(dtype, SY_LAUNCH((spp_pool_bwd_kernel<T>), dim3(grid_for(work)), dim3(kBlock), 0, stream,
                                       (typename T::elem*)dbuf, (const unsigned char*)argmax, N, H, W, C, ld,
                                       (long long)bs));
}

extern "C" int sy_bn_finalize(const float* sum, const float* sqsum, int C, int copies, double count, const float* gamma,
                              const float* beta, float eps, float momentum, float* running_mean, float* running_var,
                              float* scale, float* shift, float* mean, float* invstd, int nseg, void* stream) {
    if (sum == nullptr || sqsum == nullptr || gamma == nullptr || beta == nullptr || scale == nullptr ||
        shift == nullptr || C <= 0 || copies <= 0 || count <= 0.0)
        return SY_ERR_ARG;
    if ((running_mean == nullptr) != (running_var == nullptr)) return SY_ERR_ARG;
    if (nseg < 1 || (nseg > 1 && running_mean != nullptr)) return SY_ERR_ARG;
    int read = copies;
    if (copies > kFoldAbove) {
        SY_LAUNCH(fold_rows_kernel, dim3((C + 63) / 64, kFoldTo, 2 * nseg), dim3(kBlock), 0, stream, const_cast<float*>(sum),
                  const_cast<float*>(sqsum), C, copies);
        read = kFoldTo;
    }
    SY_LAUNCH(bn_finalize_kernel, dim3((C + 31) / 32, nseg), dim3(kBlock), 0, stream, sum, sqsum, C, read, copies, count,
              gamma, beta, eps, momentum, running_mean, running_var, scale, shift, mean, invstd);
    return SY_LAUNCH_OK() == 0 ? SY_OK : SY_ERR_LAUNCH;
}

extern "C" int sy_bn_running_update(const sy_bn_running_entry* entries, int n_entries, int max_C, void* stream) {
    if (entries == nullptr || n_entries <= 0 || max_C <= 0) return SY_ERR_ARG;
    SY_LAUNCH(bn_running_update_kernel, dim3(n_entries, (max_C + 31) / 32), dim3(kBlock), 0, stream, entries);
    return SY_LAUNCH_OK() == 0 ? SY_OK : SY_ERR_LAUNCH;
}

extern "C" int sy_bn_silu_apply(const void* y, int ldy, const float* scale, const float* shift, const void* res, int ldr,
                                void* out, int ldo, int64_t pixels, int C, int dtype, int nseg, void* stream) {
    if (y == nullptr || out == nullptr || scale == nullptr || shift == nullptr || pixels <= 0 || C <= 0 || nseg < 1) return SY_ERR_ARG;
    const int e = epc_of(dtype);
    if (C % e || ldy % e || ldo % e || (res != nullptr && ldr % e)) return SY_ERR_UNSUPPORTED;
    if (!chunk_rows_ok(C, e)) return SY_ERR_UNSUPPORTED;
    const int cap_apply = bn_cap(kCapApply).load(std::memory_order_relaxed);
    SY_DISPATCH_DTYPE(dtype, SY_LAUNCH((bn_silu_apply_kernel<T>), dim3(row_grid(pixels, C, e, cap_apply / nseg), nseg), dim3(kBlock), 0, stream,
                                       (const typename T::elem*)y, ldy, scale, shift, (const typename T::elem*)res, ldr,
                                       (typename T::elem*)out, ldo, (long long)pixels, C));
}

extern "C" int sy_bn_finalize_apply(const float* sum, const float* sqsum, int copies, double count, const float* gamma,
                                    const float* beta, float eps, float* scale, float* shift, float* mean, float* invstd,
                                    const void* y, int ldy, const void* res, int ldr, void* out, int ldo, int64_t pixels, int C,
                                    int dtype, int nseg, void* stream) {
    if (sum == nullptr || sqsum == nullptr || gamma == nullptr || beta == nullptr || scale == nullptr || shift == nullptr ||
        mean == nullptr || invstd == nullptr || y == nullptr || out == nullptr || copies <= 0 || count <= 0.0 || pixels <= 0 ||
        C <= 0 || nseg < 1)
        return SY_ERR_ARG;
    const int e = epc_of(dtype);
    if (C % e || ldy % e || ldo % e || (res != nullptr && ldr % e)) return SY_ERR_UNSUPPORTED;
    int CS = C;
    for (int c = (64 / e) * e; c >= e; c -= e)
        if (c <= C && C % c == 0) { CS = c; break; }
    if (CS > 64) return SY_ERR_UNSUPPORTED;
    const int nsl = C / CS;
    const int cap_fa = bn_cap(kCapFApply).load(std::memory_order_relaxed);
    int cap = cap_fa / (nseg * nsl);
    if (cap < 1) cap = 1;
    SY_DISPATCH_DTYPE(dtype, SY_LAUNCH((bn_finalize_apply_kernel<T>), dim3(row_grid(pixels, CS, e, cap), nseg, nsl), dim3(kBlock), 0,
                                       stream, sum, sqsum, copies, count, gamma, beta, eps, scale, shift, mean, invstd,
                                       (const typename T::elem*)y, ldy, (const typename T::elem*)res, ldr,
                                       (typename T::elem*)out, ldo, (long long)pixels, C, CS));
}

extern "C" int sy_bn_silu_bwd_reduce(const void* y, int ldy, const void* da, int ldda, const float* scale,
                                     const float* shift, const float* mean, const float* invstd, float* sums,
                                     int copies, int64_t pixels, int C, int dtype, int nseg, void* stream) {
    if (y == nullptr || da == nullptr || sums == nullptr || pixels <= 0 || C <= 0 || copies <= 0 || nseg < 1) return SY_ERR_ARG;
    const int e = epc_of(dtype);
    if (C % e || ldy % e || ldda % e) return SY_ERR_UNSUPPORTED;
    if (!chunk_rows_ok(C, e)) return SY_ERR_UNSUPPORTED;
    const int cap_reduce = bn_cap(kCapReduce).load(std::memory_order_relaxed);
    static const int slice_max = env_cap("SY_BN_REDUCE_SLICE", 64);
    int CS = C;
    for (int c = (slice_max / e) * e; c >= e; c -= e)
        if (c <= C && C % c == 0) { CS = c; break; }
    const int nsl = C / CS;
    int cap = cap_reduce / (nseg * nsl);
    if (cap < 1) cap = 1;
    SY_DISPATCH_DTYPE(dtype, SY_LAUNCH((bn_silu_bwd_reduce_kernel<T>), dim3(row_grid(pixels, CS, e, cap), nseg, nsl), dim3(kBlock), 0, stream,
                                       (const typename T::elem*)y, ldy, (const typename T::elem*)da, ldda, scale, shift,
                                       mean, invstd, sums, (long long)pixels, C, CS, copies));
}

extern "C" int sy_bn_silu_bwd_apply(const void* y, int ldy, const void* da, int ldda, const float* scale,
                                    const float* shift, const float* mean, const float* invstd, const float* gamma,
                                    const float* sums, int copies, void* dy, int lddy, int64_t pixels, int C,
                                    float* dgamma, float* dbeta, void* dres, int lddres, int dres_accumulate, int dtype,
                                    int nseg, void* stream) {
    if (y == nullptr || da == nullptr || sums == nullptr || dy == nullptr || pixels <= 0 || C <= 0 || copies <= 0 || nseg < 1)
        return SY_ERR_ARG;
    const long long seg_sum_stride = (long long)copies * 2 * C;
    if ((dgamma == nullptr) != (dbeta == nullptr)) return SY_ERR_ARG;
    const int e = epc_of(dtype);
    if (C % e || ldy % e || ldda % e || lddy % e || (dres != nullptr && lddres % e)) return SY_ERR_UNSUPPORTED;
    if (!chunk_rows_ok(C, e) || C > 1024) return SY_ERR_UNSUPPORTED;
    static const int fold_inline = env_cap("SY_BN_FOLD_INLINE", 2);
    if (copies > fold_inline) {
        SY_LAUNCH(fold_replicas_kernel, dim3((2 * C + 63) / 64, nseg), dim3(kBlock), 0, stream,
                  const_cast<float*>(sums), 2 * C, copies);
        copies = 1;
    }
    const int cap_bapply = bn_cap(kCapBApply).load(std::memory_order_relaxed);
    SY_DISPATCH_DTYPE(dtype, SY_LAUNCH((bn_silu_bwd_apply_kernel<T>), dim3(row_grid(pixels, C, e, cap_bapply / nseg), nseg), dim3(kBlock), 0, stream,
                                       (const typename T::elem*)y, ldy, (const typename T::elem*)da, ldda, scale, shift,
                                       mean, invstd, gamma, sums, (typename T::elem*)dy, lddy, (long long)pixels, C, copies,
                                       dgamma, dbeta, seg_sum_stride, (typename T::elem*)dres, lddres, dres_accumulate));
}
SY_PROBE_READER(sy_probe_read_train_ops)
```

streamyolo_amd/ops.py:

```python
import ctypes as C

import torch

from . import _lib
from ._lib import (CONV_DGRAD, CONV_FWD, DT_BF16, DT_F16, DT_F32, EPI_BNR, EPI_DECODE, EPI_LINEAR, EPI_SIGMOID,
                   EPI_SILU, ConvDesc, WgradDesc, check)

TORCH_DTYPE = {DT_BF16: torch.bfloat16, DT_F16: torch.float16, DT_F32: torch.float32}
DTYPE_CODE = {v: k for k, v in TORCH_DTYPE.items()}
DTYPE_NAME = {"bf16": DT_BF16, "fp16": DT_F16, "f16": DT_F16, "fp32": DT_F32, "f32": DT_F32}


def dtype_code(d):
    if isinstance(d, str):
        return DTYPE_NAME[d]
    if isinstance(d, torch.dtype):
        return DTYPE_CODE[d]
    return int(d)


def stream_of(t):
    if t.is_cuda:
        return C.c_void_p(torch.cuda.current_stream(t.device).cuda_stream)
    return C.c_void_p(0)
# ... 11 lines not shown

    @staticmethod
    def alloc(N, H, W, C_, dtype, device, zero=False):
        fn = torch.zeros if zero else torch.empty
        return View(fn((N, H, W, C_), dtype=TORCH_DTYPE[dtype_code(dtype)], device=device), N, H, W, C_)

    @property
    def bs(self):
        return self.H * self.W * self.ld if self.bs_ is None else self.bs_

    @property
    def dtype(self):
        return DTYPE_CODE[self.buf.dtype]

    @property
    def pixels(self):
        return self.N * self.H * self.W

    def ptr(self):
        return self.buf.data_ptr() + self.c_off * self.buf.element_size()

    def bytes_from_ptr(self):
        st = self.buf.untyped_storage()
        return st.nbytes() - (self.ptr() - st.data_ptr())

    def slice(self, c0, c):
        assert 0 <= c0 and c0 + c <= self.C
        return View(self.buf, self.N, self.H, self.W, c, self.ld, self.c_off + c0, self.bs_, self.root)

    def like(self, zero=False):
        fn = torch.zeros_like if zero else torch.empty_like
        return View(fn(self.buf), self.N, self.H, self.W, self.C, self.ld, self.c_off)

    def pair(self):
        full, n0 = self.root
        assert n0 == 0 and full.shape[0] == 2 * self.N
        return View(full, 2 * self.N, self.H, self.W, self.C, self.ld, self.c_off, self.bs_)

    def export(self):
        assert self.bs_ is None
        return self.buf.view(self.N, self.H, self.W, self.ld)[..., self.c_off:self.c_off + self.C] \
            .clone(memory_format=torch.contiguous_format).permute(0, 3, 1, 2)

    def nchw(self):
        return self.buf.view(self.N, self.H, self.W, self.ld)[..., self.c_off:self.c_off + self.C] \
            .permute(0, 3, 1, 2).float().contiguous()

    def set_nchw(self, t):
        self.buf.view(self.N, self.H, self.W, self.ld)[..., self.c_off:self.c_off + self.C] = \
            t.permute(0, 2, 3, 1).to(self.buf.dtype)


def _p(t):
    return None if t is None else t.data_ptr()


_weights_epoch = [0]


def weights_epoch():
    return _weights_epoch[0]


def bump_weights_epoch():
    _weights_epoch[0] += 1


def conv_out_size(h, k, stride):
    return (h + 2 * ((k - 1) // 2) - k) // stride + 1


def conv2d(x, w, y, ksize, stride, scale=None, shift=None, res=None, epilogue=EPI_LINEAR, mode=CONV_FWD,
           accumulate=False, stats=None, dec_stride=0.0, y_f32=False, y_ptr=None, y_ld=None, y_bs=None,
           cout=None, tile=0, wfrag=None, segments=1, k_splits=0, pre=None, bn_reduce=None):
    if bn_reduce is not None:
        z, scale, shift, sums = bn_reduce
        assert mode == CONV_DGRAD and not accumulate and res is None and stats is None and z.ld == y.ld and z.bs == y.bs
        res, epilogue, stats = z, EPI_BNR, (sums, sums)
    d = ConvDesc()
    d.x, d.w = x.ptr(), w.data_ptr()
    d.scale, d.shift = _p(scale), _p(shift)
    d.res = None if res is None else res.ptr()
    d.stat_sum, d.stat_sqsum = (None, None) if stats is None else (stats[0].data_ptr(), stats[1].data_ptr())
    d.stat_copies = 1 if stats is None else max(1, stats[0].numel() // ((2 if bn_reduce is not None else 1) * segments * (y.C if cout is None else cout)))
    d.stat_segments = segments
    d.N, d.H, d.W, d.Cin = x.N, x.H, x.W, x.C
    if y is not None:
        d.y, d.Ho, d.Wo, d.Cout = y.ptr(), y.H, y.W, y.C
        d.ldy, d.ybs = y.ld, y.bs
    if y_ptr is not None:
        d.y, d.ldy, d.ybs = y_ptr, y_ld, y_bs
        if y is None:
            d.Ho, d.Wo = conv_out_size(x.H, ksize, stride), conv_out_size(x.W, ksize, stride)
    if cout is not None:
        d.Cout = cout
    d.KH = d.KW = ksize
    d.stride, d.pad = stride, (ksize - 1) // 2
    d.ldx, d.xbs = x.ld, x.bs
    d.ldr, d.rbs = (0, 0) if res is None else (res.ld, res.bs)
    d.dtype = x.dtype
    d.y_f32 = 1 if y_f32 else 0
    d.mode, d.epilogue, d.accumulate = mode, epilogue, 1 if accumulate else 0
    d.dec_stride = float(dec_stride)
    d.tile = int(tile)
    d.x_bytes = x.bytes_from_ptr()
    d.w_bytes = w.numel() * w.element_size()
    if wfrag is not None:
        d.wfrag, d.wfrag_bytes = wfrag.data_ptr(), wfrag.numel() * wfrag.element_size()
    d.k_splits = int(k_splits)
    if pre is not None:
        pw, ps, ph = pre
        d.pre_w, d.pre_w_bytes, d.pre_scale, d.pre_shift = pw.data_ptr(), pw.numel() * pw.element_size(), ps.data_ptr(), ph.data_ptr()
        d.pre_cin = x.C
        d.Cin = ps.numel()
    check(_lib.lib().sy_conv2d(C.byref(d), stream_of(x.buf)), "sy_conv2d")


def conv2d_wgrad(x, dy, dw, ksize, stride, oihw=False, workspace=None, tile=0, target_blocks=0):
    d = WgradDesc()
    d.x, d.dy, d.dw = x.ptr(), dy.ptr(), dw.data_ptr()
    d.N, d.H, d.W, d.Cin = x.N, x.H, x.W, x.C
    d.Ho, d.Wo, d.Cout = dy.H, dy.W, dy.C
    d.KH = d.KW = ksize
    d.stride, d.pad = stride, (ksize - 1) // 2
    d.ldx, d.lddy, d.xbs, d.dybs = x.ld, dy.ld, x.bs, dy.bs
    d.dtype = x.dtype
    d.dw_oihw = 1 if oihw else 0
    d.tile, d.target_blocks = int(tile), int(target_blocks)
    d.x_bytes, d.dy_bytes = x.bytes_from_ptr(), dy.bytes_from_ptr()
    if workspace is not None:
        d.workspace, d.workspace_bytes = workspace.data_ptr(), workspace.numel() * workspace.element_size()
    check(_lib.lib().sy_conv2d_wgrad(C.byref(d), stream_of(x.buf)), "sy_conv2d_wgrad")


def conv2d_splitk(x, w, y, ksize, stride, scale, shift, part, splits, res=None, epilogue=EPI_SILU, tile=118, wfrag=None):
    assert part.dtype == torch.float32 and part.numel() >= splits * y.pixels * y.C
    pv = View(part, splits * y.N, y.H, y.W, y.C)
    d = dict(y_f32=True, y_ptr=part.data_ptr(), y_ld=y.C, y_bs=y.H * y.W * y.C)
    conv2d(x, w, pv, ksize, stride, epilogue=EPI_LINEAR, tile=tile, wfrag=wfrag, k_splits=splits, **d)
    check(_lib.lib().sy_splitk_epilogue(part.data_ptr(), splits, y.pixels, y.C, _p(scale), _p(shift),
                                        None if res is None else res.ptr(), 0 if res is None else res.ld, y.ptr(), y.ld, y.dtype,
                                        epilogue, stream_of(y.buf)), "sy_splitk_epilogue")


def focus_pack(frames, c0, out):
    assert frames.dtype == torch.float32 and frames.is_contiguous()
    N, Ct, H, W = frames.shape
    assert out.C == 16 and out.ld == 16 and out.c_off == 0
    check(_lib.lib().sy_focus_pack(frames.data_ptr(), N, Ct, c0, H, W, out.ptr(), out.dtype, stream_of(frames)),
          "sy_focus_pack")


FRAMES_NCHW, FRAMES_FOCUS = 0, 1


def frames_u8_pack(cur, sup, canvas, out_size, out_cur, out_sup=None, decimate=1, mirror=None):
    assert cur.dtype == torch.uint8 and cur.dim() == 4 and cur.shape[3] == 3 and cur.stride(3) == 1 and cur.stride(2) == 3
    B, Hs, Ws, _ = cur.shape
    if sup is not None:
        assert sup.dtype == torch.uint8 and sup.shape == cur.shape and sup.stride() == cur.stride()
    if mirror is not None:
        assert mirror.dtype == torch.uint8 and mirror.numel() == B and mirror.is_contiguous()
    H, W = canvas
    Ho, Wo = out_size
    if isinstance(out_cur, View):
        layout, dt = FRAMES_FOCUS, out_cur.dtype
        for v in (out_cur, out_sup):
# ... 16 lines not shown
    check(_lib.lib().sy_resize_bilinear_nchw(x.data_ptr(), N, Cc, H, W, out.data_ptr(), out.shape[2], out.shape[3],
                                             stream_of(x)), "sy_resize_bilinear_nchw")


def resize_nearest(src, dst):
    assert src.C == dst.C and src.N == dst.N
    check(_lib.lib().sy_resize_nearest(src.ptr(), src.N, src.H, src.W, src.C, src.ld, src.bs, dst.ptr(), dst.H,
                                       dst.W, dst.ld, dst.bs, src.dtype, stream_of(src.buf)), "sy_resize_nearest")


def resize_nearest_bwd(ddst, dsrc, accumulate):
    check(_lib.lib().sy_resize_nearest_bwd(ddst.ptr(), ddst.N, ddst.H, ddst.W, ddst.C, ddst.ld, ddst.bs, dsrc.ptr(),
                                           dsrc.H, dsrc.W, dsrc.ld, dsrc.bs, 1 if accumulate else 0, ddst.dtype,
                                           stream_of(ddst.buf)), "sy_resize_nearest_bwd")


def spp_pool(v, argmax=None):
    c = v.C // 4
    check(_lib.lib().sy_spp_pool(v.ptr(), v.N, v.H, v.W, c, v.ld, v.bs, _p(argmax), v.dtype, stream_of(v.buf)),
          "sy_spp_pool")


def spp_pool_bwd(dv, argmax):
    c = dv.C // 4
    check(_lib.lib().sy_spp_pool_bwd(dv.ptr(), argmax.data_ptr(), dv.N, dv.H, dv.W, c, dv.ld, dv.bs, dv.dtype,
                                     stream_of(dv.buf)), "sy_spp_pool_bwd")


def view_copy(src, dst, accumulate=False):
    assert src.C == dst.C and src.pixels == dst.pixels
    check(_lib.lib().sy_view_copy(src.ptr(), src.ld, dst.ptr(), dst.ld, src.pixels, src.C, src.dtype,
                                  1 if accumulate else 0, stream_of(src.buf)), "sy_view_copy")


def _stream_tables(row_slot, row_first, B, device):
    assert row_slot.dtype == torch.int32 and row_slot.is_contiguous() and row_slot.numel() >= B and row_slot.device == device
    if row_first is not None:
        assert row_first.dtype == torch.uint8 and row_first.is_contiguous() and row_first.numel() >= B and row_first.device == device


def stream_state_gather(cur, pool, sup, row_slot, row_first):
    assert (cur.N, cur.H, cur.W, cur.C) == (sup.N, sup.H, sup.W, sup.C) and cur.dtype == sup.dtype
    assert pool.dim() == 4 and tuple(pool.shape[1:]) == (cur.H, cur.W, cur.C) and pool.is_contiguous() and pool.dtype == cur.buf.dtype
    _stream_tables(row_slot, row_first, cur.N, pool.device)
    check(_lib.lib().sy_stream_state_gather(cur.ptr(), cur.ld, cur.bs, pool.data_ptr(), pool.shape[0], sup.ptr(), sup.ld, sup.bs,
                                            cur.N, cur.H, cur.W, cur.C, row_slot.data_ptr(), row_first.data_ptr(), cur.dtype,
                                            stream_of(pool)), "sy_stream_state_gather")


def stream_state_scatter(curs, pools, row_slot):
    assert len(curs) == len(pools) and 1 <= len(curs) <= 8
    B, S, dt = curs[0].N, pools[0].shape[0], curs[0].dtype
    rows = []
    for c, p in zip(curs, pools):
        assert c.N == B and c.dtype == dt and p.dim() == 4 and tuple(p.shape) == (S, c.H, c.W, c.C) and p.is_contiguous()
        assert p.dtype == c.buf.dtype
        e = _lib.StreamLevel()
        e.cur, e.pool, e.bs, e.H, e.W, e.C, e.ld = c.ptr(), p.data_ptr(), c.bs, c.H, c.W, c.C, c.ld
        rows.append(e)
    _stream_tables(row_slot, None, B, pools[0].device)
    arr = (_lib.StreamLevel * len(rows))(*rows)
    check(_lib.lib().sy_stream_state_scatter(arr, len(rows), S, B, row_slot.data_ptr(), dt, stream_of(pools[0])),
          "sy_stream_state_scatter")


def rows_add_f32(dst, src, rows, cols, ldd, lds, zero_src=False):
    assert dst.dtype == torch.float32 and src.dtype == torch.float32
    check(_lib.lib().sy_rows_add_f32(dst.data_ptr(), ldd, src.data_ptr(), lds, rows, cols, 1 if zero_src else 0, stream_of(dst)),
          "sy_rows_add_f32")


def pred_grad_fold(d_raw, a0, rows, num_classes, scratch, cin, g_reg, g_obj, g_cls, gb_reg, gb_obj, gb_cls, workspace):
    B, A, nch = d_raw.shape
    assert d_raw.dtype == torch.float32 and d_raw.is_contiguous() and nch == 5 + num_classes
    assert scratch.dim() == 3 and scratch.shape[0] == 2 and scratch.is_contiguous()
    assert workspace.numel() >= _lib.lib().sy_pred_grad_fold_workspace_floats(num_classes)
    check(_lib.lib().sy_pred_grad_fold(d_raw.data_ptr() + a0 * nch * 4, B, A * nch, rows, num_classes, scratch.data_ptr(),
                                       scratch.shape[1], scratch.shape[2], cin, g_reg.data_ptr(), g_obj.data_ptr(), g_cls.data_ptr(),
                                       gb_reg.data_ptr(), gb_obj.data_ptr(), gb_cls.data_ptr(), workspace.data_ptr(),
                                       stream_of(d_raw)), "sy_pred_grad_fold")


def bn_finalize(ssum, ssq, count, gamma, beta, eps, momentum, running_mean, running_var, scale, shift, mean, invstd,
                nseg=1):
    C_ = gamma.numel()
    check(_lib.lib().sy_bn_finalize(ssum.data_ptr(), ssq.data_ptr(), C_, ssum.numel() // (nseg * C_), float(count),
                                    gamma.data_ptr(), beta.data_ptr(), float(eps), float(momentum), _p(running_mean),
                                    _p(running_var), scale.data_ptr(), shift.data_ptr(), _p(mean), _p(invstd), nseg,
                                    stream_of(ssum)), "sy_bn_finalize")


def bn_finalize_apply(ssum, ssq, count, gamma, beta, eps, scale, shift, mean, invstd, y, out, res=None, nseg=1):
    C_ = gamma.numel()
    check(_lib.lib().sy_bn_finalize_apply(ssum.data_ptr(), ssq.data_ptr(), ssum.numel() // (nseg * C_), float(count),
                                          gamma.data_ptr(), beta.data_ptr(), float(eps), scale.data_ptr(), shift.data_ptr(),
                                          mean.data_ptr(), invstd.data_ptr(), y.ptr(), y.ld,
                                          None if res is None else res.ptr(), 0 if res is None else res.ld, out.ptr(), out.ld,
                                          y.pixels // nseg, y.C, y.dtype, nseg, stream_of(y.buf)), "sy_bn_finalize_apply")


class BnRunningTable:

    def __init__(self, modules, device, count_batches=False):
        arr = (_lib.BnRunningEntry * len(modules))()
        self.max_c, self.keep = 0, []
        for e, (bn, calls) in zip(arr, modules):
            assert 1 <= len(calls) <= 2
            e.running_mean, e.running_var = bn.running_mean.data_ptr(), bn.running_var.data_ptr()
            for j, call in enumerate(calls):
                ssum, ssq, count = call[:3]
                e.sum[j], e.sqsum[j], e.count[j] = ssum.data_ptr(), ssq.data_ptr(), float(count)
            e.C = bn.num_features
            e.copies = calls[0][3] if len(calls[0]) > 3 else calls[0][0].numel() // e.C
            e.ld = calls[0][4] if len(calls[0]) > 4 else 0
            e.calls = len(calls)
            e.momentum = bn.momentum if bn.momentum is not None else 0.1
            nbt = getattr(bn, "num_batches_tracked", None)
            if nbt is not None and count_batches:
                assert nbt.dtype == torch.int64
                e.num_batches_tracked = nbt.data_ptr()
                self.keep.append((bn.running_mean, bn.running_var, nbt))
            else:
                self.keep.append((bn.running_mean, bn.running_var))
            self.max_c = max(self.max_c, e.C)
        raw = torch.frombuffer(bytearray(bytes(arr)), dtype=torch.uint8)
        self.table = raw.to(device)
        self.n = len(modules)
        self.sig = tuple(t.data_ptr() for pair in self.keep for t in pair)

    def valid(self):
        return self.sig == tuple(t.data_ptr() for pair in self.keep for t in pair)

    def run(self):
        check(_lib.lib().sy_bn_running_update(self.table.data_ptr(), self.n, self.max_c, stream_of(self.table)),
              "sy_bn_running_update")
        bump_weights_epoch()


BN_CAP_NAMES = ("apply", "finalize_apply", "bwd_reduce", "bwd_apply")


def bn_grid_caps(**set_):
    assert all(k in BN_CAP_NAMES for k in set_), set_
    s4 = (C.c_int32 * 4)(*[int(set_.get(k, 0)) for k in BN_CAP_NAMES])
    g4 = (C.c_int32 * 4)()
    check(_lib.lib().sy_bn_grid_caps(s4, g4), "sy_bn_grid_caps")
    return dict(zip(BN_CAP_NAMES, [int(v) for v in g4]))


def zero(t):
    esz = t.element_size()
    if t.is_contiguous():
        rows, row_b, pitch_b = 1, t.numel() * esz, t.numel() * esz
    else:
        assert t.dim() == 2 and t.stride(1) == 1, "zero(): dense tensor or a row-strided 2-D view"
        rows, row_b, pitch_b = t.shape[0], t.shape[1] * esz, t.stride(0) * esz
    if rows == 0 or row_b == 0:
        return
    check(_lib.lib().sy_zero_rows(t.data_ptr(), rows, row_b, pitch_b, stream_of(t)), "sy_zero_rows")


def bn_silu_apply(y, scale, shift, out, res=None, nseg=1):
    check(_lib.lib().sy_bn_silu_apply(y.ptr(), y.ld, scale.data_ptr(), shift.data_ptr(),
                                      None if res is None else res.ptr(), 0 if res is None else res.ld, out.ptr(),
                                      out.ld, y.pixels // nseg, y.C, y.dtype, nseg, stream_of(y.buf)), "sy_bn_silu_apply")


def bn_silu_bwd_reduce(y, da, scale, shift, mean, invstd, sums, nseg=1):
    check(_lib.lib().sy_bn_silu_bwd_reduce(y.ptr(), y.ld, da.ptr(), da.ld, scale.data_ptr(), shift.data_ptr(),
                                           mean.data_ptr(), invstd.data_ptr(), sums.data_ptr(),
                                           sums.numel() // (2 * y.C * nseg), y.pixels // nseg, y.C, y.dtype, nseg,
                                           stream_of(y.buf)), "sy_bn_silu_bwd_reduce")


def bn_silu_bwd_apply(y, da, scale, shift, mean, invstd, gamma, sums, dy, dgamma=None, dbeta=None, nseg=1,
                      dres=None, dres_accumulate=False, atomic_param_grads=False, raw_moment=False):
    assert dres is None or (dres.C == y.C and dres.pixels == y.pixels)
    check(_lib.lib().sy_bn_silu_bwd_apply(y.ptr(), y.ld, da.ptr(), da.ld, scale.data_ptr(), shift.data_ptr(),
                                          mean.data_ptr(), invstd.data_ptr(), gamma.data_ptr(), sums.data_ptr(),
                                          sums.numel() // (2 * y.C * nseg), dy.ptr(), dy.ld, y.pixels // nseg, y.C,
                                          _p(dgamma), _p(dbeta), None if dres is None else dres.ptr(),
                                          0 if dres is None else dres.ld,
                                          (1 if dres_accumulate else 0) | (2 if atomic_param_grads else 0) | (4 if raw_moment else 0), y.dtype, nseg,
                                          stream_of(y.buf)), "sy_bn_silu_bwd_apply")


def head_decode(out, hw=None, strides=None, boxes=True, obj_sigmoid=False, corners=False):
    assert out.dtype == torch.float32 and out.is_contiguous() and out.dim() == 3
    B, A, nch = out.shape
    flags = (1 if boxes else 0) | (2 if obj_sigmoid else 0) | (4 if corners else 0)
    if boxes:
        n = len(hw)
        lh = (C.c_int32 * n)(*[int(h) for h, _ in hw])
        lw = (C.c_int32 * n)(*[int(w) for _, w in hw])
        ls = (C.c_float * n)(*[float(s) for s in strides])
    else:
        n, lh, lw, ls = 0, None, None, None
    check(_lib.lib().sy_head_decode(out.data_ptr(), B, A, nch, lh, lw, ls, n, flags, stream_of(out)), "sy_head_decode")
    return out


class PostprocessWorkspace:

    def __init__(self, B, A, device, max_det=None):
        self.B, self.A = B, A
        self.max_det = A if max_det is None else max_det
        nbytes = _lib.lib().sy_postprocess_workspace_bytes(B, A)
        self.ws = torch.empty(nbytes, dtype=torch.uint8, device=device)
        self.det = torch.zeros((B, self.max_det, 7), dtype=torch.float32, device=device)
        self.index = torch.zeros((B, self.max_det), dtype=torch.int32, device=device)
        self.count = torch.zeros((B,), dtype=torch.int32, device=device)


def postprocess(pred, num_classes, conf_thre, nms_thre, ws=None):
    assert pred.dtype == torch.float32 and pred.is_contiguous() and pred.shape[2] == 5 + num_classes
    B, A = pred.shape[:2]
    if ws is None or ws.B != B or ws.A != A:
        ws = PostprocessWorkspace(B, A, pred.device)
    check(_lib.lib().sy_postprocess(pred.data_ptr(), B, A, num_classes, float(conf_thre), float(nms_thre),
                                    ws.max_det, ws.det.data_ptr(), ws.index.data_ptr(), ws.count.data_ptr(),
                                    ws.ws.data_ptr(), stream_of(pred)), "sy_postprocess")
    return ws.det, ws.index, ws.count


class TalLossWorkspace:

    def __init__(self, B, A, nch, hw_list, strides, device, max_labels=120):
        self.B, self.A, self.max_labels = B, A, max_labels
        self.ws = torch.empty(_lib.lib().sy_tal_loss_workspace_bytes(B, A, max_labels), dtype=torch.uint8, device=device)
        self.d_raw = torch.empty((B, A, nch), dtype=torch.float32, device=device)
        self.losses = torch.zeros(8, dtype=torch.float32, device=device)
        self.fg = torch.zeros((B, A), dtype=torch.int32, device=device)
        self.lh = (C.c_int32 * len(hw_list))(*[int(h) for h, _ in hw_list])
        self.lw = (C.c_int32 * len(hw_list))(*[int(w) for _, w in hw_list])
        self.ls = (C.c_float * len(hw_list))(*[float(s) for s in strides])
        self.nlevels = len(hw_list)


def tal_loss(raw, labels, support, num_classes, gamma, ignore_thr, ignore_value, use_l1, ws, d_pad=None, scaler_state=None):
    assert raw.dtype == torch.float32 and raw.is_contiguous()
    labels = labels[..., :5].to(raw.device, torch.float32).contiguous()
    support = support[..., :5].to(raw.device, torch.float32).contiguous()
    assert labels.shape[1] == ws.max_labels and support.shape == labels.shape
    if scaler_state is not None:
        assert scaler_state.device == raw.device and scaler_state.numel() * scaler_state.element_size() == 32
        check(_lib.lib().sy_tal_loss_scaled(raw.data_ptr(), ws.B, ws.A, num_classes, labels.data_ptr(), support.data_ptr(),
                                            ws.max_labels, C.cast(ws.lh, C.c_void_p), C.cast(ws.lw, C.c_void_p),
                                            C.cast(ws.ls, C.c_void_p), ws.nlevels, float(gamma), float(ignore_thr),
                                            float(ignore_value), 1 if use_l1 else 0, ws.d_raw.data_ptr(), ws.losses.data_ptr(),
                                            ws.fg.data_ptr(), ws.ws.data_ptr(), _p(d_pad),
                                            0 if d_pad is None else DTYPE_CODE[d_pad.dtype], scaler_state.data_ptr(),
                                            stream_of(raw)), "sy_tal_loss_scaled")
        return ws.losses, ws.d_raw, ws.fg
    check(_lib.lib().sy_tal_loss(raw.data_ptr(), ws.B, ws.A, num_classes, labels.data_ptr(), support.data_ptr(),
                                 ws.max_labels, C.cast(ws.lh, C.c_void_p), C.cast(ws.lw, C.c_void_p),
                                 C.cast(ws.ls, C.c_void_p), ws.nlevels, float(gamma), float(ignore_thr),
                                 float(ignore_value), 1 if use_l1 else 0, ws.d_raw.data_ptr(), ws.losses.data_ptr(),
                                 ws.fg.data_ptr(), ws.ws.data_ptr(), _p(d_pad), 0 if d_pad is None else DTYPE_CODE[d_pad.dtype],
                                 stream_of(raw)), "sy_tal_loss")
    return ws.losses, ws.d_raw, ws.fg


def tal_assignment(ws):
    mg = torch.empty((ws.B, ws.A), dtype=torch.int32, device=ws.ws.device)
    mi = torch.empty((ws.B, ws.A), dtype=torch.float32, device=ws.ws.device)
    check(_lib.lib().sy_tal_loss_assignment(ws.ws.data_ptr(), ws.B, ws.A, ws.max_labels, mg.data_ptr(), mi.data_ptr(),
# ... 323 lines not shown
```

streamyolo_amd/train_engine.py:

```python
import ctypes as C
import os

import torch

from . import ops
from .data import FramePairsU8
from .engine import _Builder, MergedConv, base_convs, build_frame_net, build_fuse_net, build_head_net
from .model.plan_cache import compute_dtype_for
from .ops import View, EPI_LINEAR, CONV_DGRAD


_FUSED_FINALIZE = __import__("os").environ.get("STREAMYOLO_FUSED_FINALIZE", "auto")
BNR_FUSION = __import__("os").environ.get("STREAMYOLO_BNR_FUSION", "0") != "0"
BNR_TILES = (98, 100, 101, 109, 104, 107, 117, 118)
EXACT_STATS = __import__("os").environ.get("STREAMYOLO_EXACT_STATS", "1") != "0"
BN_BAPPLY_BLOCKS_SCHEDULED = 512


def _schedule_bn_caps():
    if os.environ.get("SY_BN_BAPPLY_BLOCKS"):
        return ops.bn_grid_caps()["bwd_reduce"]
    return ops.bn_grid_caps(bwd_apply=BN_BAPPLY_BLOCKS_SCHEDULED)["bwd_reduce"]



class _GradSpace:

    def __init__(self):
        self.mirror = {}
        self.written = {}
        self.py = lambda fn: fn()

    def reset(self):
        self.written = {}

    def view(self, v):
        if v.root is not None:
            full, n0 = v.root
            gf = self.mirror.get(id(full))
            if gf is None:
                gf = torch.empty_like(full)
                self.mirror[id(full)] = gf
            return View(gf[n0:n0 + v.N], v.N, v.H, v.W, v.C, v.ld, v.c_off, v.bs_, root=(gf, n0))
        g = self.mirror.get(id(v.buf))
        if g is None:
            g = torch.empty_like(v.buf)
            self.mirror[id(v.buf)] = g
        return View(g, v.N, v.H, v.W, v.C, v.ld, v.c_off, v.bs_)

    def target(self, v):
        key = (id(v.root[0]), v.root[1]) if v.root is not None else id(v.buf)
        iv = self.written.setdefault(key, [])
        c0, c1 = v.c_off, v.c_off + v.C
        assert v.bs_ is None and c1 <= v.ld
        gaps, pos = [], c0
        for a, b in iv:
            if b <= pos or a >= c1:
                continue
            if a > pos:
                gaps.append((pos, a))
            pos = max(pos, b)
        if pos < c1:
            gaps.append((pos, c1))
        g = self.view(v)
        if len(gaps) == 1 and gaps[0] == (c0, c1):
            accumulate = False
        else:
            accumulate = True
            flat = g.buf.view(-1, v.ld)
            for a, b in gaps:
                ops.zero(flat[:, a:b])
        if gaps:
            merged = []
            for a, b in sorted(iv + [(c0, c1)]):
                if merged and a <= merged[-1][1]:
                    merged[-1] = (merged[-1][0], max(merged[-1][1], b))
                else:
                    merged.append((a, b))
            iv[:] = merged
        return g, accumulate


class _PairBuilder(_Builder):

    def __init__(self, dtype, device):
        super().__init__(dtype, device)
        self.fulls, self.replay, self.paired = [], None, True

    def buf(self, N, H, W, C):
        if not self.paired:
            return super().buf(N, H, W, C)
        if self.replay is None:
            full = torch.empty((2 * N, H, W, C), dtype=ops.TORCH_DTYPE[ops.dtype_code(self.dtype)], device=self.device)
            self.fulls.append(full)
            half = 0
        else:
            full = self.fulls[self.replay]
            self.replay += 1
# ... 96 lines not shown
HEAD_BWD_CHAINS = os.environ.get("STREAMYOLO_HEAD_BWD_CHAINS", "1") != "0"
HEAD_EARLY = os.environ.get("STREAMYOLO_HEAD_EARLY", "1") != "0"
CHAIN_SLOT_DONE = os.environ.get("STREAMYOLO_CHAIN_SLOT_DONE", "0") != "0"
SLOT_BATCH = max(1, int(os.environ.get("STREAMYOLO_SLOT_BATCH", "3")))
DUAL_WGRAD = os.environ.get("STREAMYOLO_DUAL_WGRAD", "1") != "0"
WGRAD_STREAMS = [1, 3, 4, 5][:max(1, min(4, int(os.environ.get("STREAMYOLO_WGRAD_STREAMS", "2")) if DUAL_WGRAD else 1))]


NINE_TAP_WGRAD_TILES = (52, 59, 60)


def scheduled_wgrad(wt, cin, env=None):
    env = os.environ if env is None else env
    tile, blocks = wt
    cap = int(env.get("STREAMYOLO_WGRAD_BLOCKS_CAP", "512"))
    if cap > 0 and blocks > cap:
        blocks = cap
    if tile in NINE_TAP_WGRAD_TILES:
        cap9 = int(env.get("STREAMYOLO_WGRAD9_BLOCKS", "128"))
        wide9 = int(env.get("STREAMYOLO_WGRAD9_WIDE", "60"))
        if wide9 and cin % 64 == 0:
            tile, cap9 = wide9, int(env.get("STREAMYOLO_WGRAD9_WIDE_BLOCKS", "96"))
        if cap9 > 0 and blocks > cap9:
            blocks = cap9
    return (tile, blocks)


def _csp_role(tag):
    head, _, leaf = tag.rpartition(".")
    if leaf not in ("conv2", "conv3") or ".m." in tag or head in ("", "spp"):
        return None
    return leaf


class TrainPlan:
    BWD_COPIES = int(os.environ.get("STREAMYOLO_BWD_COPIES", "2"))
    STAT_COPIES = int(os.environ.get("STREAMYOLO_STAT_COPIES", "0"))
    WGRAD_WS_BYTES = 256 << 20
    RING = int(os.environ.get("STREAMYOLO_RING", "0"))
    STREAMS = int(os.environ.get("STREAMYOLO_STREAMS", "2"))
    TAPE_ON_CPU = True

    def __init__(self, model, B, H, W, dtype, device, parts="full", feat_shapes=None, pool=None):
        self.model, self.B, self.H, self.W, self.device = model, B, H, W, device
        self.parts = parts
        self.pool = pool
        self.dtype = ops.dtype_code(dtype)
        self.tdtype = ops.TORCH_DTYPE[self.dtype]
        pafpn = model.backbone if parts == "full" else (model if parts == "backbone" else None)
        head = model.head if parts == "full" else (model if parts == "head" else None)
        self.head = head
        self.cache = None
        b = _PairBuilder(self.dtype, device)
        b.merge_siblings = MERGE_SIBLINGS_TRAIN
        if pafpn is not None:
            self.f0_cur, cur = build_frame_net(b, pafpn, B, H, W)
            self.n_frame_ops = len(b.ops)
            b.replay = 0
            self.f0_sup, sup = build_frame_net(b, pafpn, B, H, W)
            assert len(b.ops) == 2 * self.n_frame_ops and b.replay == len(b.fulls)
            b.paired = False
            fused = build_fuse_net(b, pafpn, cur, sup)
        else:
            self.n_frame_ops = 0
            b.paired = False
            fused = tuple(b.buf(B, h, w, c) for c, h, w in feat_shapes)
        self.fused = fused
        self.n_head_start = len(b.ops)
        self.preds, self.A = (build_head_net(b, head, fused) if head is not None else ([], 0))
        lvl = 0
        for op in b.ops[self.n_head_start:]:
            op.level = lvl
            lvl += 1 if op.kind == "pred" else 0
        self.hw = [(f.H, f.W) for f in fused]
        self.ops = b.ops
        self.nc = head.num_classes if head is not None else 0
        nch = 5 + self.nc
        self.raw = torch.empty((B, self.A, nch), dtype=torch.float32, device=device)
        self.dpad = torch.zeros((B, self.A, 16), dtype=self.tdtype, device=device)

        convs = [op for op in self.ops if op.kind == "conv"]
        tot_c = sum(op.y.C for op in convs)
        self.exact_stats = EXACT_STATS
        self.stat_copies = self.STAT_COPIES if self.STAT_COPIES > 0 else (32 if self.dtype == ops.DT_F32 else 4)
        self.fused_finalize = ((_FUSED_FINALIZE == "1") or (_FUSED_FINALIZE == "auto" and self.dtype != ops.DT_F32)) and not self.exact_stats
        reduce_cap = _schedule_bn_caps()

        def copies_of(op):
            if not self.exact_stats:
                return self.stat_copies, self.BWD_COPIES
            return max(self.stat_copies, op.y.N * op.y.H * ((op.y.W + 31) // 32)), max(self.BWD_COPIES, reduce_cap)
        for op in convs:
            op.stat_copies, op.bwd_copies = copies_of(op)
        self.stat_arena = torch.zeros(2 * sum(op.stat_copies * op.y.C for op in convs), dtype=torch.float32, device=device)
        self.bwd_arena = torch.zeros(2 * sum(op.bwd_copies * op.y.C for op in convs), dtype=torch.float32, device=device)
        self.aff_arena = torch.empty(4 * tot_c, dtype=torch.float32, device=device)
        sq0 = self.stat_arena.numel() // 2
        off = 0
        max_raw = 0
        nf = self.n_frame_ops
        for i in range(nf):
            a, b2 = self.ops[i], self.ops[nf + i]
            if a.kind == "conv":
                full = torch.empty((2 * a.y.N, a.y.H, a.y.W, a.y.C), dtype=self.tdtype, device=device)
                a.yraw = View(full[:a.y.N], a.y.N, a.y.H, a.y.W, a.y.C, root=(full, 0))
                b2.yraw = View(full[a.y.N:], a.y.N, a.y.H, a.y.W, a.y.C, root=(full, a.y.N))
        units = [(self.ops[i], self.ops[nf + i]) for i in range(nf) if self.ops[i].kind == "conv"]
        units += [(op,) for op in self.ops[2 * nf:] if op.kind == "conv"]
        s_off = b_off = 0
        for unit in units:
            C, S = unit[0].y.C, len(unit)
            SC, BC = unit[0].stat_copies, unit[0].bwd_copies
            u_sum = self.stat_arena[s_off:s_off + SC * S * C]
            u_sq = self.stat_arena[sq0 + s_off:sq0 + s_off + SC * S * C]
            u_bsum = self.bwd_arena[b_off:b_off + 2 * BC * S * C]
            s_off += SC * S * C
            b_off += 2 * BC * S * C
            u_aff = tuple(self.aff_arena[k * tot_c + off:k * tot_c + off + S * C] for k in range(4))
            for s_, op in enumerate(unit):
                op.stat = (u_sum[s_ * SC * C:(s_ + 1) * SC * C], u_sq[s_ * SC * C:(s_ + 1) * SC * C])
                op.bsum = u_bsum[s_ * 2 * BC * C:(s_ + 1) * 2 * BC * C]
                op.aff = tuple(t[s_ * C:(s_ + 1) * C] for t in u_aff)
                if op.yraw is None:
                    op.yraw = View.alloc(op.y.N, op.y.H, op.y.W, C, self.dtype, device)
                max_raw = max(max_raw, 2 * op.y.pixels * C)
            unit[0].unit = (u_sum, u_sq, u_bsum, u_aff)
            off += S * C
        self.max_raw = max_raw
        self._bind_scratch()
        self.ring_i = 0
        self.side = torch.cuda.Stream(device=device) if (device.type == "cuda" and self.STREAMS > 1) else None
        w_ = float(getattr(pafpn, "width", 1.0)) if pafpn is not None else 0.0
        self.bwd_split = (BWD_SPLIT_FRAMES == "1") or (BWD_SPLIT_FRAMES == "auto" and B * H * W * w_ * w_ >= 2.0e6)
        self.side2 = torch.cuda.Stream(device=device) if (self.side is not None and (self.bwd_split or HEAD_BWD_CHAINS)) else None
        self.side_w = {k: torch.cuda.Stream(device=device) for k in WGRAD_STREAMS[1:]} if self.side is not None else {}
        self.side3 = self.side_w.get(3)
        self._chain, self._wg_stream, self._wg_flip = 0, 1, 0
        self.tuned = False
        self.force_serial = False
        self._ev_pool = []
        for op in self.ops:
            if op.kind == "spp":
                op.argmax = torch.empty((op.v.N, op.v.H, op.v.W, 3, op.v.C // 4), dtype=torch.uint8, device=device)
        self.cache = StagedWeights(self.ops, self.dtype, device)
        self.loss_ws = None
        self._zeroed, self._zero_ev, self._packed_for = None, None, None
        self.run_table = None
        self.grads = _GradSpace()
        self.grads.py = self._py
        self.programs, self._rec, self._param_sig = {}, None, None
        self._side_region = False
        self.pending = 0

        group_of = {}
        for op in self.ops:
            if op.kind == "conv" and isinstance(op.mod, MergedConv):
                parts = base_convs(op.mod)
                block = [m.conv.weight for m in parts] + [m.bn.weight for m in parts] + [m.bn.bias for m in parts]
                for t in block:
                    group_of[id(t)] = block
        self.params, seen = [], set()
        for p in model.parameters():
            if not p.requires_grad or id(p) in seen:
                continue
            for t in group_of.get(id(p), (p,)):
                assert t.requires_grad and id(t) not in seen
                seen.add(id(t))
                self.params.append(t)
        n = sum(p.numel() for p in self.params)
        self.arena = torch.zeros(n, dtype=torch.float32, device=device)
        self.gview = {}
        o = 0
        for p in self.params:
            self.gview[id(p)] = self.arena[o:o + p.numel()].view(p.shape)
            o += p.numel()
        self._build_buckets()
        self.on_bucket = None
        self.bn_mods = [m.bn for op in convs for m in base_convs(op.mod)]
        self.stem_scratch = None
        self.pred_scratch = torch.zeros((2, max(8, self.nc), int(256 * head.width)), dtype=torch.float32, device=device) \
            if head is not None else None
        self.pred_ws = torch.empty(int(ops._lib.lib().sy_pred_grad_fold_workspace_floats(self.nc)), dtype=torch.float32,
                                   device=device) if head is not None else None

    def _bind_scratch(self):
        esz = torch.empty(0, dtype=self.tdtype).element_size()
        ring_bytes = -(-self.max_raw * esz // 256) * 256
        if self.pool is not None:
            self.wgrad_ws = self.pool.shared_scratch("wgrad_ws", self.WGRAD_WS_BYTES, self.device)
            slots = [self.pool.shared_scratch("dyraw_ring_%d" % i, ring_bytes, self.device) for i in range(max(self.RING, 0))]
            self._scratch_gen = self.pool.scratch_gen
        else:
            self.wgrad_ws = torch.empty(self.WGRAD_WS_BYTES, dtype=torch.uint8, device=self.device)
            slots = [torch.empty(ring_bytes, dtype=torch.uint8, device=self.device) for _ in range(max(self.RING, 0))]
            self._scratch_gen = 0
        self.dyraw_ring = [t[:self.max_raw * esz].view(self.tdtype) for t in slots]
        self.dyraw_own = []
        self.wgrad_ws_by = {WGRAD_STREAMS[0]: self.wgrad_ws}
        for k in WGRAD_STREAMS[1:]:
            self.wgrad_ws_by[k] = (self.pool.shared_scratch("wgrad_ws%d" % k, self.WGRAD_WS_BYTES, self.device)
                                   if self.pool is not None else torch.empty(self.WGRAD_WS_BYTES, dtype=torch.uint8, device=self.device))
        if self.pool is not None:
            self._scratch_gen = self.pool.scratch_gen

    def release(self):
        self.programs.clear()
        self.dyraw_own = []
        self.grads.py = None
        self.grads.mirror.clear()
        self.on_bucket = None

    def forward(self, x):
        if self.parts != "head":
            x = x.float().contiguous()
        if self.pool is not None and self._scratch_gen != self.pool.scratch_gen:
            self._bind_scratch()
            self.programs.clear()
        sig = tuple(p.data_ptr() for p in self.params)
        if sig != self._param_sig or not self.cache.valid():
            self._param_sig = sig
            self.programs.clear()
            if not self.cache.valid():
                self.cache = StagedWeights(self.ops, self.dtype, self.device)
        self.cache.refresh()
        ops.zero(self.stat_arena)
        if self.parts == "head":
            for v, t in zip(self.fused, x):
                assert tuple(t.shape) == (v.N, v.C, v.H, v.W)
                v.set_nchw(t.detach())
        elif isinstance(x, FramePairsU8):
            x.pack_focus(self.f0_cur, self.f0_sup)
        else:
            ops.focus_pack(x, 0, self.f0_cur)
            ops.focus_pack(x, 3, self.f0_sup)
        self._run("fwd", self._forward_ops)
        if self.run_table is None or not self.run_table.valid():
            mods = {}
            for op in self.ops:
                if op.kind == "conv":
                    c0, ctot, SC = 0, op.y.C, (32 if op.stat_copies > 64 else op.stat_copies)
                    for m in base_convs(op.mod):
                        mods.setdefault(id(m.bn), (m.bn, []))[1].append((op.stat[0][c0:], op.stat[1][c0:], op.y.pixels, SC, ctot))
                        c0 += m.bn.num_features
            self.run_table = ops.BnRunningTable(list(mods.values()), self.device, count_batches=True)
        self.run_table.run()
        return self.raw if self.head is not None else self.fused

    def _forward_ops(self):
        nf = self.n_frame_ops
        if FWD_SPLIT_FRAMES and nf:
            early = self._early_levels() if (HEAD_EARLY and self.head is not None and self.side2 is not None) else {}
            self._mark("fork")
            for i in range(nf):
                self._forward_op(self.ops[i])
                self._mark("side_nw")
                self._forward_op(self.ops[nf + i])
                self._mark("main", None)
                for lvl_ops in early.get(i, ()):
                    self._mark("dep", (0, 2))
                    self._mark("dep", (1, 2))
                    self._mark("cur", 2)
                    for op in lvl_ops:
                        self._forward_op(op)
                    self._mark("cur", 0)
            self._mark("join")
            if early:
                done = {id(op) for v in early.values() for lvl_ops in v for op in lvl_ops}
                for op in self.ops[2 * nf:]:
                    if id(op) not in done:
                        self._forward_op(op)
                self._mark("dep", (2, 0))
                return
        for i in range(nf if not (FWD_SPLIT_FRAMES and nf) else 0):
            a, b2 = self.ops[i], self.ops[nf + i]
            if a.kind == "conv":
                role = _csp_role(a.tag) if CSP_FORK else None
                if role == "conv2":
                    self._mark("side")
                    self._forward_pair(a)
                    self._mark("main", None)
                    continue
                if role == "conv3":
                    self._mark("join")
                self._forward_pair(a)
            else:
                self._forward_op(a)
                self._forward_op(b2)
        for op in self.ops[2 * nf:self.n_head_start]:
            self._forward_op(op)
        self._mark("fork")
        for op in self.ops[self.n_head_start:]:
            if op.level == 0:
                self._forward_op(op)
        self._mark("side_nw")
        self._side_region = True
        for op in self.ops[self.n_head_start:]:
            if op.level != 0:
                self._forward_op(op)
        self._side_region = False
        self._mark("main", None)
        self._mark("join")

    def _early_levels(self):
        nf = self.n_frame_ops
        fuse = self.ops[2 * nf:self.n_head_start]
        head_ops = self.ops[self.n_head_start:]
        nlev = len(self.preds)
        if len(fuse) != 2 * nlev:
            return {}
        out = {}
        for k in range(nlev):
            src = fuse[2 * k].x.buf.data_ptr()
            writers = [i for i in range(nf) if self.ops[i].kind == "conv" and self.ops[i].y.buf.data_ptr() == src]
            if not writers or max(writers) >= nf - 1:
                continue
            out.setdefault(max(writers), []).append([fuse[2 * k], fuse[2 * k + 1]] + [op for op in head_ops if op.level == k])
        return out

    def _bn_params(self, op):
        parts = base_convs(op.mod)
        bn = parts[0].bn
        mom = bn.momentum if bn.momentum is not None else 0.1
        if len(parts) == 1:
            return bn.weight, bn.bias, bn.eps, mom
        assert all(m.bn.eps == bn.eps and m.bn.momentum == bn.momentum for m in parts)
        g, b_ = self.cache.bn[id(op.mod)]
        return g, b_, bn.eps, mom

    def _bn_bwd(self, op, y, da, aff, gamma, bsum, dy, dgamma, dbeta, nseg=1, dres=None, acc=False, atomic=False):
        fused = getattr(op, "bnr_by", None) is not None
        if not fused:
            ops.bn_silu_bwd_reduce(y, da, *aff, bsum, nseg=nseg)
        ops.bn_silu_bwd_apply(y, da, *aff, gamma, bsum, dy, dgamma, dbeta, nseg=nseg, dres=dres, dres_accumulate=acc,
                              atomic_param_grads=atomic, raw_moment=fused)

    def _bnr_producer(self, op, dx, acc, t):
        pre = op.pre_op
        if (not BNR_FUSION or pre is None or acc or self.dtype == ops.DT_F32 or t not in BNR_TILES or op.k != 3 or op.stride != 1
                or pre.res is not None or pre.yraw is None or pre.yraw.ld != dx.ld or pre.yraw.bs != dx.bs or pre.y.C % 8 or dx.ld % 8
                or (dx.ptr() | pre.yraw.ptr()) % 16 or dx.bs % 8):
            return None
        return pre

    def _bn_grads(self, op):
        bn = base_convs(op.mod)[0].bn
        return self.gview[id(bn.weight)], self.gview[id(bn.bias)]

    def _forward_pair(self, a):
        gamma, beta, eps, mom = self._bn_params(a)
        x2, raw2, y2 = a.x.pair(), a.yraw.pair(), a.y.pair()
        u_sum, u_sq, _, (scale, shift, mean, invstd) = a.unit
        t = a._tiles.get("fwd_stats2")
        if t is None:
            t = ops.tuned_tile(ops.CONV_FWD, x2.dtype, x2.N, x2.H, x2.W, x2.C, y2.C, a.k, a.stride, self.device,
                               with_stats=True)
            a._tiles["fwd_stats2"] = t
        ops.conv2d(x2, self.cache.conv_weight(a.mod), raw2, a.k, a.stride, stats=(u_sum, u_sq), tile=t,
                   wfrag=self.cache.conv_weight_frag(a.mod) if t >= ops.TILE_WR else None, segments=2)
        if self.fused_finalize:
            ops.bn_finalize_apply(u_sum, u_sq, a.y.pixels, gamma, beta, eps, scale, shift, mean, invstd, raw2, y2,
                                  res=None if a.res is None else a.res.pair(), nseg=2)
        else:
            ops.bn_finalize(u_sum, u_sq, a.y.pixels, gamma, beta, eps, mom, None, None, scale, shift, mean, invstd,
                            nseg=2)
            ops.bn_silu_apply(raw2, scale, shift, y2, res=None if a.res is None else a.res.pair(), nseg=2)

    def _mark(self, kind, arg=None):
        if self._rec is not None:
            self._rec.mark(kind, arg)

    def _py(self, fn):
        fn()
        if self._rec is not None:
            self._rec.snippet(fn)

    def _run(self, name, body, key=None):
        from . import _lib
        if self.force_serial or not self.tuned or self.device.type != "cuda" and not self.TAPE_ON_CPU:
            self._rec = None
            body()
            return
        prog = self.programs.get(name)
        if prog is None or prog[0] != key:
            tape = _lib.NativeTape()
            with tape:
                self._rec = tape
                try:
                    body()
                finally:
                    self._rec = None
            self.programs[name] = (key, tape)
            return
        self._interpret(prog[1])

    def _interpret(self, tape):
        side, side2 = self.side, self.side2
        extra = [self.side_w.get(k) for k in (3, 4, 5)]
        if self.device.type == "cuda":
            main = torch.cuda.current_stream(self.device)
            main_h = C.c_void_p(main.cuda_stream)
            side_h = C.c_void_p(side.cuda_stream) if side is not None else None
            more = [C.c_void_p(st_.cuda_stream) if st_ is not None else None for st_ in [side2] + extra]
            while more and more[-1] is None:
                more.pop()
            if torch.cuda.is_current_stream_capturing():
                more = []
        else:
            main, main_h, side_h, more = None, C.c_void_p(0), None, []
        chains = [main, side, side2] + extra

        def snippet(fn, k):
            if k and chains[k] is not None:
                with torch.cuda.stream(chains[k]):
                    fn()
            else:
                fn()
        on_bucket = None
        if self.on_bucket is not None:
            on_bucket = lambda k: self.on_bucket(k, main, [s_ for s_ in [side, side2] + extra if s_ is not None])
        tape.replay(main_h, side_h, snippet, on_bucket, more=more)

    def _forward_op(self, op):
        nch = 5 + self.nc
        k = op.kind
        if k == "conv":
            gamma, beta, eps, mom = self._bn_params(op)
            w = self.cache.conv_weight(op.mod)
            t = op.tile("fwd_stats")
            scale, shift, mean, invstd = op.aff
            ops.conv2d(op.x, w, op.yraw, op.k, op.stride, stats=op.stat, tile=t,
                       wfrag=self.cache.conv_weight_frag(op.mod) if t >= ops.TILE_WR else None)
            if self.fused_finalize:
                ops.bn_finalize_apply(op.stat[0], op.stat[1], op.y.pixels, gamma, beta, eps, scale, shift, mean, invstd,
                                      op.yraw, op.y, res=op.res)
            else:
                ops.bn_finalize(op.stat[0], op.stat[1], op.y.pixels, gamma, beta, eps, mom,
                                None, None, scale, shift, mean, invstd)
                ops.bn_silu_apply(op.yraw, scale, shift, op.y, res=op.res)
        elif k == "resize":
            ops.resize_nearest(op.src, op.dst)
        elif k == "spp":
            ops.spp_pool(op.v, op.argmax)
        else:
            w_ro, b_ro, w_c, b_c = self.cache.pred(op)[:4]
            base = self.raw.data_ptr() + op.a0 * nch * 4
            ops.conv2d(op.reg_x, w_ro, None, 1, 1, None, b_ro, epilogue=EPI_LINEAR, y_f32=True, y_ptr=base,
                       y_ld=nch, y_bs=self.A * nch, cout=5)
            ops.conv2d(op.cls_x, w_c, None, 1, 1, None, b_c, epilogue=EPI_LINEAR, y_f32=True, y_ptr=base + 20,
                       y_ld=nch, y_bs=self.A * nch, cout=self.nc)

    def loss(self, labels, support, scaler=None):
        head = self.head
        if self.loss_ws is None or self.loss_ws.max_labels != labels.shape[1]:
            self.loss_ws = ops.TalLossWorkspace(self.B, self.A, 5 + self.nc, self.hw, head.strides, self.device,
                                                max_labels=labels.shape[1])
        pad = self.dpad if self.nc <= 8 else None
        self._zero_gradient_arenas()
        losses, d_raw, _ = ops.tal_loss(self.raw, labels, support, self.nc, head.gamma, head.ignore_thr,
                                        head.ignore_value, head.use_l1, self.loss_ws, d_pad=pad,
                                        scaler_state=None if scaler is None else scaler.state(self.device))
        self._packed_for = (d_raw, d_raw._version) if pad is not None else None
        out = {"total_loss": losses[0], "iou_loss": losses[1], "l1_loss": losses[2], "conf_loss": losses[3],
               "cls_loss": losses[4], "num_fg": losses[5]}
        return out, d_raw

    def backward(self, d_raw, d_fused=None):
        self._zero_gradient_arenas(wait=True)
        nc = self.nc
        pf = getattr(self, "_packed_for", None)
        if self.head is not None and not (pf is not None and pf[0] is d_raw and pf[1] == d_raw._version):
            self.dpad[..., 0:5] = d_raw[..., 0:5]
            self.dpad[..., 8:8 + nc] = d_raw[..., 5:]
        self._packed_for = None
        self._seed = d_fused
        self._run("bwd", lambda: self._backward_ops(d_raw), key=None if d_raw is None else d_raw.data_ptr())
        if not self.tuned:
            self.tuned = True
            ops.save_tuned()
        return self.arena

    def _zero_gradient_arenas(self, wait=False):
        st = self.side_w.get(3) or self.side2 or self.side
        if wait:
            if self._zeroed is None:
                ops.zero(self.arena)
                ops.zero(self.bwd_arena)
            elif self._zeroed is not True:
                torch.cuda.current_stream(self.device).wait_event(self._zeroed)
            self._zeroed = None
            return
        if self._zeroed is not None:
            return
        if st is None or self.device.type != "cuda" or torch.cuda.is_current_stream_capturing():
            ops.zero(self.arena)
            ops.zero(self.bwd_arena)
            self._zeroed = True
            return
        st.wait_stream(torch.cuda.current_stream(self.device))
        with torch.cuda.stream(st):
            ops.zero(self.arena)
            ops.zero(self.bwd_arena)
            if self._zero_ev is None:
                self._zero_ev = torch.cuda.Event()
            self._zero_ev.record()
        self._zeroed = self._zero_ev

    def fused_grads(self):
        return tuple(self.grads.view(f).nchw() for f in self.fused)

    BUCKET_BYTES = 32 << 20
    FIRST_BUCKET_BYTES = 4 << 20

    def _backward_sequence(self):
        nf = self.n_frame_ops
        return list(reversed(self.ops[2 * nf:])) + [self.ops[i] for i in reversed(range(nf))]

    def _build_buckets(self):
        last = {}
        for pos, op in enumerate(self._backward_sequence()):
            if op.kind == "conv":
# ... 629 lines not shown
```

Measured before the change: 353.6 frame-pairs/s.

## Use fixed-point binned int64 atomics for deterministic BN statistics

Replaces the exact-stats path, which used one float copy per output tile (thousands of copies per channel), with fixed-point accumulation. Values are split into exponent bins and added with int64 atomics into a small number of copies. This makes order-independent exact sums cheap and cuts stat arena size and finalize reduction work. It also re-enables the fused finalize+apply kernel under exact stats. The cost is five bins per value, 64-bit atomics, and a poison flag for out-of-range values.

```diff
diff --git a/include/streamyolo_hip.h b/include/streamyolo_hip.h
--- a/include/streamyolo_hip.h
+++ b/include/streamyolo_hip.h
@@ -66,6 +66,8 @@
     int64_t pre_w_bytes;
     const float* pre_scale;
     const float* pre_shift;
+    int32_t stat_fixed;
+    uint32_t* stat_poison;
 } sy_conv_desc;
 
 SY_API int sy_conv2d(const sy_conv_desc* d, void* stream);
@@ -159,14 +161,24 @@
     int32_t C, copies, calls;
     float momentum;
     int32_t ld;
-    int32_t reserved;
+    int32_t fixed;
     int64_t* num_batches_tracked;
+    const uint32_t* poison[2];
 } sy_bn_running_entry;
 SY_API int sy_bn_running_update(const sy_bn_running_entry* entries, int n_entries, int max_C, void* stream);
 SY_API int sy_bn_finalize_apply(const float* sum, const float* sqsum, int copies, double count, const float* gamma,
                                 const float* beta, float eps, float* scale, float* shift, float* mean, float* invstd,
                                 const void* y, int ldy, const void* res, int ldr, void* out, int ldo, int64_t pixels, int C,
                                 int dtype, int nseg, void* stream);
+
+SY_API int sy_fix_layout(int32_t* layout3);
+SY_API int sy_bn_finalize_fixed(const void* sum, const void* sqsum, const uint32_t* poison, int C, int copies, double count,
+                                const float* gamma, const float* beta, float eps, float momentum, float* running_mean,
+                                float* running_var, float* scale, float* shift, float* mean, float* invstd, int nseg, void* stream);
+SY_API int sy_bn_finalize_apply_fixed(const void* sum, const void* sqsum, const uint32_t* poison, int copies, double count,
+                                      const float* gamma, const float* beta, float eps, float* scale, float* shift, float* mean,
+                                      float* invstd, const void* y, int ldy, const void* res, int ldr, void* out, int ldo,
+                                      int64_t pixels, int C, int dtype, int nseg, void* stream);
 
 SY_API int sy_bn_silu_apply(const void* y, int ldy, const float* scale, const float* shift, const void* res,
                      int ldr, void* out, int ldo, int64_t pixels, int C, int dtype, int nseg, void* stream);
@@ -178,6 +190,15 @@
                                 const float* gamma, const float* sums, int copies, void* dy, int lddy,
                                 int64_t pixels, int C, float* dgamma, float* dbeta, void* dres, int lddres,
                                 int dres_accumulate, int dtype, int nseg, void* stream);
+
+SY_API int sy_bn_silu_bwd_reduce_fixed(const void* y, int ldy, const void* da, int ldda, const float* scale,
+                                       const float* shift, const float* mean, const float* invstd, void* sums, uint32_t* poison,
+                                       int copies, int64_t pixels, int C, int dtype, int nseg, void* stream);
+SY_API int sy_bn_silu_bwd_apply_fixed(const void* y, int ldy, const void* da, int ldda, const float* scale,
+                                      const float* shift, const float* mean, const float* invstd, const float* gamma,
+                                      const void* sums, const uint32_t* poison, int copies, void* dy, int lddy, int64_t pixels,
+                                      int C, float* dgamma, float* dbeta, void* dres, int lddres, int dres_accumulate, int dtype,
+                                      int nseg, void* stream);
 
 SY_API int64_t sy_tal_loss_workspace_bytes(int B, int A, int max_gt);
 SY_API int sy_tal_loss(const float* raw, int B, int A, int num_classes, const float* labels,
diff --git a/streamyolo_amd/_lib.py b/streamyolo_amd/_lib.py
--- a/streamyolo_amd/_lib.py
+++ b/streamyolo_amd/_lib.py
@@ -30,14 +30,15 @@
         ("accumulate", C.c_int32), ("dec_stride", C.c_float), ("stat_copies", C.c_int32), ("stat_segments", C.c_int32), ("tile", C.c_int32), ("x_bytes", C.c_int64), ("w_bytes", C.c_int64), ("wfrag", C.c_void_p), ("wfrag_bytes", C.c_int64),
         ("k_splits", C.c_int32), ("pre_cin", C.c_int32), ("pre_w", C.c_void_p), ("pre_w_bytes", C.c_int64),
         ("pre_scale", C.c_void_p), ("pre_shift", C.c_void_p),
+        ("stat_fixed", C.c_int32), ("stat_poison", C.c_void_p),
     ]
 
 
 class BnRunningEntry(C.Structure):
     _fields_ = [("running_mean", C.c_void_p), ("running_var", C.c_void_p), ("sum", C.c_void_p * 2),
                 ("sqsum", C.c_void_p * 2), ("count", C.c_double * 2), ("C", C.c_int32), ("copies", C.c_int32),
-                ("calls", C.c_int32), ("momentum", C.c_float), ("ld", C.c_int32), ("reserved", C.c_int32),
-                ("num_batches_tracked", C.c_void_p)]
+                ("calls", C.c_int32), ("momentum", C.c_float), ("ld", C.c_int32), ("fixed", C.c_int32),
+                ("num_batches_tracked", C.c_void_p), ("poison", C.c_void_p * 2)]
 
 
 class PackEntry(C.Structure):
@@ -103,6 +104,11 @@
     "sy_pack_weights": (_I, [_P, _I, _I, _P]),
     "sy_bn_running_update": (_I, [_P, _I, _I, _P]),
     "sy_bn_finalize": (_I, [_P, _P, _I, _I, _D, _P, _P, _F, _F, _P, _P, _P, _P, _P, _P, _I, _P]),
+    "sy_fix_layout": (_I, [C.POINTER(C.c_int32)]),
+    "sy_bn_finalize_fixed": (_I, [_P, _P, _P, _I, _I, _D, _P, _P, _F, _F, _P, _P, _P, _P, _P, _P, _I, _P]),
+    "sy_bn_finalize_apply_fixed": (_I, [_P, _P, _P, _I, _D, _P, _P, _F, _P, _P, _P, _P, _P, _I, _P, _I, _P, _I, _L, _I, _I, _I, _P]),
+    "sy_bn_silu_bwd_reduce_fixed": (_I, [_P, _I, _P, _I, _P, _P, _P, _P, _P, _P, _I, _L, _I, _I, _I, _P]),
+    "sy_bn_silu_bwd_apply_fixed": (_I, [_P, _I, _P, _I, _P, _P, _P, _P, _P, _P, _P, _I, _P, _I, _L, _I, _P, _P, _P, _I, _I, _I, _I, _P]),
     "sy_bn_silu_apply": (_I, [_P, _I, _P, _P, _P, _I, _P, _I, _L, _I, _I, _I, _P]),
     "sy_bn_finalize_apply": (_I, [_P, _P, _I, _D, _P, _P, _F, _P, _P, _P, _P, _P, _I, _P, _I, _P, _I, _L, _I, _I, _I, _P]),
     "sy_bn_silu_bwd_reduce": (_I, [_P, _I, _P, _I, _P, _P, _P, _P, _P, _I, _L, _I, _I, _I, _P]),
@@ -176,7 +182,7 @@
     def __getattr__(self, name):
         fn = getattr(self.real, name)
         tape = self.tape
-        if name.endswith("_supported") or name.endswith("_bytes") or name.endswith("_floats") or name.endswith("version") or name.endswith("_caps") or name.startswith("sy_tape_"):
+        if name.endswith("_supported") or name.endswith("_bytes") or name.endswith("_floats") or name.endswith("version") or name.endswith("_caps") or name.endswith("_layout") or name.startswith("sy_tape_"):
             return fn
 
         def call(*args):
diff --git a/streamyolo_amd/csrc/conv_igemm.hip b/streamyolo_amd/csrc/conv_igemm.hip
--- a/streamyolo_amd/csrc/conv_igemm.hip
+++ b/streamyolo_amd/csrc/conv_igemm.hip
@@ -17,6 +17,11 @@
     if (d->KH < 1 || d->KW < 1 || d->KH * d->KW > 49) return SY_ERR_UNSUPPORTED;
     if ((d->stat_sum == nullptr) != (d->stat_sqsum == nullptr)) return SY_ERR_ARG;
     if (d->epilogue < SY_EPI_LINEAR || d->epilogue > SY_EPI_BNR) return SY_ERR_ARG;
+    if (d->stat_fixed) {
+        if (d->stat_sum == nullptr || d->stat_poison == nullptr || (((uintptr_t)d->stat_sum | (uintptr_t)d->stat_sqsum) & 7) != 0) return SY_ERR_ARG;
+        if (d->epilogue == SY_EPI_BNR) return SY_ERR_UNSUPPORTED;
+        if ((long long)(d->stat_segments > 1 ? d->N / d->stat_segments : d->N) * d->Ho * ((d->Wo + 31) / 32) > kFixMaxAdders) return SY_ERR_UNSUPPORTED;
+    }
     if (d->epilogue == SY_EPI_BNR) {
         if (d->mode != SY_CONV_DGRAD || d->accumulate || d->y_f32 || d->dtype == SY_DT_F32 || d->res == nullptr || d->scale == nullptr ||
             d->shift == nullptr || d->stat_sum == nullptr || d->ldr != d->ldy || d->rbs != d->ybs || d->stat_segments > 1)
@@ -37,6 +42,8 @@
     a.y_f32 = d->y_f32; a.mode = d->mode; a.epilogue = d->epilogue; a.accumulate = d->accumulate;
     a.dec_stride = d->dec_stride;
     a.stat_copies = d->stat_copies > 0 ? d->stat_copies : 1;
+    a.stat_fixed = d->stat_fixed ? 1 : 0;
+    a.stat_poison = (unsigned*)d->stat_poison;
     a.seg_M = 0;
     a.s2_classes = 0;
     if (d->stat_segments > 1) {
diff --git a/streamyolo_amd/csrc/conv_igemm_impl.h b/streamyolo_amd/csrc/conv_igemm_impl.h
--- a/streamyolo_amd/csrc/conv_igemm_impl.h
+++ b/streamyolo_amd/csrc/conv_igemm_impl.h
@@ -34,6 +34,8 @@
     int ksplit;
     int wt;
     int ablate;
+    int stat_fixed;
+    unsigned* stat_poison;
 };
 
 template <int WC, int WP, int TC, int TP> struct StageLimit { static constexpr size_t kBytes = 48 * 1024; };
@@ -875,8 +877,14 @@
             float a = 0.0f, b = 0.0f;
 #pragma unroll
             for (int w = 0; w < WP; ++w) { a += red[(w * CT + cl) * 2]; b += red[(w * CT + cl) * 2 + 1]; }
-            atomicAdd(p.stat_sum + (long long)copy * p.Cout + co, a);
-            atomicAdd(p.stat_sq + (long long)copy * p.Cout + co, b);
+            if (p.stat_fixed) {
+                unsigned* const poison = p.stat_poison + (long long)mp.seg * p.Cout + co;
+                sy_fix_add(reinterpret_cast<unsigned long long*>(p.stat_sum) + (long long)copy * kFixBins * p.Cout + co, p.Cout, a, poison);
+                sy_fix_add(reinterpret_cast<unsigned long long*>(p.stat_sq) + (long long)copy * kFixBins * p.Cout + co, p.Cout, b, poison);
+            } else {
+                atomicAdd(p.stat_sum + (long long)copy * p.Cout + co, a);
+                atomicAdd(p.stat_sq + (long long)copy * p.Cout + co, b);
+            }
         }
     }
 }
diff --git a/streamyolo_amd/csrc/sy_device.h b/streamyolo_amd/csrc/sy_device.h
--- a/streamyolo_amd/csrc/sy_device.h
+++ b/streamyolo_amd/csrc/sy_device.h
@@ -394,6 +394,34 @@
 }
 #endif
 
+constexpr int kFixBins = 5, kFixBinBits = 20, kFixMinExp = -36;
+constexpr long long kFixMaxAdders = 1ll << 18;
+__device__ __forceinline__ void sy_fix_add(unsigned long long* dst, long long bin_stride, float v, unsigned* poison) {
+    const int e = (int)((__builtin_bit_cast(unsigned, v) >> 23) & 255u) - 127;
+    if (e >= kFixMinExp + kFixBins * kFixBinBits) {
+        atomicOr(poison, 1u);
+        return;
+    }
+    const int b = e < kFixMinExp ? 0 : (e - kFixMinExp) / kFixBinBits;
+    const long long q = (long long)__builtin_rint(ldexp((double)v, 23 - kFixMinExp - b * kFixBinBits));
+    if (q == 0) return;
+#ifdef SY_EMU
+    (void)__atomic_fetch_add(dst + b * bin_stride, (unsigned long long)q, __ATOMIC_RELAXED);
+#else
+    (void)__hip_atomic_fetch_add(dst + b * bin_stride, (unsigned long long)q, __ATOMIC_RELAXED, __HIP_MEMORY_SCOPE_AGENT);
+#endif
+}
+__device__ __forceinline__ double sy_fix_total(const unsigned long long* w, int copies, long long copy_stride, long long bin_stride,
+                                               unsigned poisoned) {
+    double acc = 0.0;
+    for (int b = kFixBins - 1; b >= 0; --b) {
+        long long t = 0;
+        for (int k = 0; k < copies; ++k) t += (long long)w[k * copy_stride + b * bin_stride];
+        acc += ldexp((double)t, kFixMinExp + b * kFixBinBits - 23);
+    }
+    return poisoned ? (double)__builtin_nanf("") : acc;
+}
+
 struct sy_block_id { int x, y, z; };
 __device__ __forceinline__ sy_block_id sy_xcd_block_id() {
     constexpr unsigned kXcd = 8;
diff --git a/streamyolo_amd/csrc/train_ops.hip b/streamyolo_amd/csrc/train_ops.hip
--- a/streamyolo_amd/csrc/train_ops.hip
+++ b/streamyolo_amd/csrc/train_ops.hip
@@ -313,26 +313,33 @@
                                                              double count, const float* gamma, const float* beta,
                                                              float eps, float momentum, float* running_mean,
                                                              float* running_var, float* scale, float* shift,
-                                                             float* mean_out, float* invstd_out) {
+                                                             float* mean_out, float* invstd_out, const unsigned* poison) {
     SY_TL_BEGIN(11);
     __shared__ float s_s[8][32], s_q[8][32];
     const int cl = threadIdx.x & 31, rg = threadIdx.x >> 5;
     const int c = blockIdx.x * 32 + cl;
+    const bool fixed = poison != nullptr;
     {
-        const long long so = (long long)blockIdx.y * stride * C, ao = (long long)blockIdx.y * C;
+        const long long so = (long long)blockIdx.y * stride * C * (fixed ? 2 * kFixBins : 1), ao = (long long)blockIdx.y * C;
         sum += so; sqsum += so; scale += ao; shift += ao;
         if (mean_out != nullptr) mean_out += ao;
         if (invstd_out != nullptr) invstd_out += ao;
+        if (fixed) poison += ao;
     }
     float s = 0.0f, q = 0.0f;
-    if (c < C)
+    if (c < C && !fixed)
         for (int k = rg; k < copies; k += 8) { s += sum[(long long)k * C + c]; q += sqsum[(long long)k * C + c]; }
     s_s[rg][cl] = s;
     s_q[rg][cl] = q;
     __syncthreads();
     if (rg != 0 || c >= C) return;
     double ds = 0.0, dq = 0.0;
-    for (int k = 0; k < 8; ++k) { ds += (double)s_s[k][cl]; dq += (double)s_q[k][cl]; }
+    if (fixed) {
+        ds = sy_fix_total(reinterpret_cast<const unsigned long long*>(sum) + c, copies, (long long)kFixBins * C, C, poison[c]);
+        dq = sy_fix_total(reinterpret_cast<const unsigned long long*>(sqsum) + c, copies, (long long)kFixBins * C, C, poison[c]);
+    } else {
+        for (int k = 0; k < 8; ++k) { ds += (double)s_s[k][cl]; dq += (double)s_q[k][cl]; }
+    }
     const double mean = ds / count;
     double var = dq / count - mean * mean;
     if (var < 0.0) var = 0.0;
@@ -362,14 +369,20 @@
     if (rg == 0 && c < e.C) { rm = e.running_mean[c]; rv = e.running_var[c]; }
     for (int j = 0; j < e.calls; ++j) {
         float s = 0.0f, q = 0.0f;
-        if (c < e.C)
+        if (c < e.C && !e.fixed)
             for (int k = rg; k < e.copies; k += 8) { s += e.sum[j][k * ld + c]; q += e.sqsum[j][k * ld + c]; }
         s_s[rg][cl] = s;
         s_q[rg][cl] = q;
         __syncthreads();
         if (rg == 0 && c < e.C) {
             double ds = 0.0, dq = 0.0;
-            for (int k = 0; k < 8; ++k) { ds += (double)s_s[k][cl]; dq += (double)s_q[k][cl]; }
+            if (e.fixed) {
+                const unsigned ps = e.poison[j][c];
+                ds = sy_fix_total(reinterpret_cast<const unsigned long long*>(e.sum[j]) + c, e.copies, kFixBins * ld, ld, ps);
+                dq = sy_fix_total(reinterpret_cast<const unsigned long long*>(e.sqsum[j]) + c, e.copies, kFixBins * ld, ld, ps);
+            } else {
+                for (int k = 0; k < 8; ++k) { ds += (double)s_s[k][cl]; dq += (double)s_q[k][cl]; }
+            }
             const double count = e.count[j];
             const double mean = ds / count;
             double var = dq / count - mean * mean;
@@ -442,8 +455,9 @@
                                                                    float* invstd_out, const typename T::elem* y, int ldy,
                                                                    const typename T::elem* res, int ldr,
                                                                    typename T::elem* out, int ldo, long long pixels, int C,
-                                                                   int CS) {
+                                                                   int CS, const unsigned* poison) {
     SY_TL_BEGIN(10);
+    const bool fixed = poison != nullptr;
     __shared__ float s_part[2][8][64];
     __shared__ float s_aff[2][64];
     const int cpp = CS / T::kEPC;
@@ -453,11 +467,12 @@
     const int c0 = cb + cc * T::kEPC;
     {
         const long long ro = (long long)blockIdx.y * pixels;
-        const long long so = (long long)blockIdx.y * copies * C;
+        const long long so = (long long)blockIdx.y * copies * C * (fixed ? 2 * kFixBins : 1);
         const int ao = blockIdx.y * C;
         y += ro * ldy; out += ro * ldo;
         if (res != nullptr) res += ro * ldr;
         sum += so; sqsum += so; scale += ao; shift += ao; mean_out += ao; invstd_out += ao;
+        if (fixed) poison += ao;
     }
     const bool live = (int)threadIdx.x < rows * cpp;
     const long long step = (long long)gridDim.x * rows;
@@ -467,7 +482,7 @@
         v = Chunk<T>::load(y + pix * ldy + c0);
         if (res != nullptr) rv = Chunk<T>::load(res + pix * ldr + c0);
     }
-    for (int it = threadIdx.x; it < 2 * 8 * CS; it += kBlock) {
+    for (int it = threadIdx.x; it < (fixed ? 0 : 2 * 8 * CS); it += kBlock) {
         const int c = it % CS, rg = (it / CS) & 7, kind = it / (8 * CS);
         const float* src = (kind ? sqsum : sum) + cb + c;
         float a = 0.0f;
@@ -478,7 +493,12 @@
     if ((int)threadIdx.x < CS) {
         const int c = threadIdx.x;
         double ds = 0.0, dq = 0.0;
-        for (int k = 0; k < 8; ++k) { ds += (double)s_part[0][k][c]; dq += (double)s_part[1][k][c]; }
+        if (fixed) {
+            ds = sy_fix_total(reinterpret_cast<const unsigned long long*>(sum) + cb + c, copies, (long long)kFixBins * C, C, poison[cb + c]);
+            dq = sy_fix_total(reinterpret_cast<const unsigned long long*>(sqsum) + cb + c, copies, (long long)kFixBins * C, C, poison[cb + c]);
+        } else {
+            for (int k = 0; k < 8; ++k) { ds += (double)s_part[0][k][c]; dq += (double)s_part[1][k][c]; }
+        }
         const double mean = ds / count;
         double var = dq / count - mean * mean;
         if (var < 0.0) var = 0.0;
@@ -519,7 +539,8 @@
                                                                     const typename T::elem* da, int ldda,
                                                                     const float* scale, const float* shift,
                                                                     const float* mean, const float* invstd, float* sums,
-                                                                    long long pixels, int C, int CS, int copies) {
+                                                                    long long pixels, int C, int CS, int copies,
+                                                                    unsigned* poison) {
     SY_TL_BEGIN(12);
     __shared__ float red[kBlock * 2 * 8];
     const int cpp = CS / T::kEPC;
@@ -532,7 +553,8 @@
         const long long ro = (long long)blockIdx.y * pixels;
         const int ao = blockIdx.y * C;
         y += ro * ldy; da += ro * ldda; scale += ao; shift += ao; mean += ao; invstd += ao;
-        sums += (long long)blockIdx.y * copies * 2 * C;
+        sums += (long long)blockIdx.y * copies * 2 * C * (poison != nullptr ? 2 * kFixBins : 1);
+        if (poison != nullptr) poison += ao;
     }
     sy_probe(0);
     const long long first = pr < rows ? (long long)blockIdx.x * rows + pr : pixels;
@@ -576,7 +598,12 @@
         const int kind = t & 1, j = (t >> 1) % T::kEPC, ch = (t >> 1) / T::kEPC;
         float v = 0.0f;
         for (int r = 0; r < rows; ++r) v += red[(j * 2 + kind) * kBlock + r * cpp + ch];
-        atomicAdd(sums + (long long)(blockIdx.x % copies) * 2 * C + kind * C + cb + ch * T::kEPC + j, v);
+        const int cch = cb + ch * T::kEPC + j;
+        if (poison != nullptr)
+            sy_fix_add(reinterpret_cast<unsigned long long*>(sums) + ((long long)(blockIdx.x % copies) * 2 + kind) * kFixBins * C + cch, C, v,
+                       poison + cch);
+        else
+            atomicAdd(sums + (long long)(blockIdx.x % copies) * 2 * C + kind * C + cch, v);
     }
     sy_probe(6);
     SY_TL_END();
@@ -591,7 +618,7 @@
                                                                    typename T::elem* dy, int lddy, long long pixels,
                                                                    int C, int copies, float* dgamma, float* dbeta,
                                                                    long long seg_sum_stride, typename T::elem* dres,
-                                                                   int lddres, int dres_acc) {
+                                                                   int lddres, int dres_acc, const unsigned* poison) {
     SY_TL_BEGIN(13);
     __shared__ float s_fold[2 * 1024];
     {
@@ -599,6 +626,7 @@
         const int ao = blockIdx.y * C;
         y += ro * ldy; da += ro * ldda; dy += ro * lddy; scale += ao; shift += ao; mean += ao; invstd += ao;
         sums += blockIdx.y * seg_sum_stride;
+        if (poison != nullptr) poison += ao;
         if (dres != nullptr) dres += ro * lddres;
     }
     const int cpp = C / T::kEPC;
@@ -618,7 +646,11 @@
     }
     for (int i = threadIdx.x; i < 2 * C; i += kBlock) {
         float a = 0.0f;
-        for (int k = 0; k < copies; ++k) a += sums[(long long)k * 2 * C + i];
+        if (poison != nullptr)
+            a = (float)sy_fix_total(reinterpret_cast<const unsigned long long*>(sums) + (long long)(i >= C ? kFixBins * C + i - C : i), copies,
+                                    2ll * kFixBins * C, C, poison[i >= C ? i - C : i]);
+        else
+            for (int k = 0; k < copies; ++k) a += sums[(long long)k * 2 * C + i];
         s_fold[i] = a;
     }
     __syncthreads();
@@ -738,6 +770,12 @@
     return SY_OK;
 }
 
+extern "C" int sy_fix_layout(int32_t* layout3) {
+    if (layout3 == nullptr) return SY_ERR_ARG;
+    layout3[0] = kFixBins; layout3[1] = kFixBinBits; layout3[2] = kFixMinExp;
+    return SY_OK;
+}
+
 extern "C" int sy_spp_pool(void* buf, int N, int H, int W, int C, int ld, int64_t bs, void* argmax, int dtype,
                            void* stream) {
     if (buf == nullptr || N <= 0 || C <= 0 || ld < 4 * C) return SY_ERR_ARG;
@@ -771,23 +809,37 @@
                                        (long long)bs));
 }
 
-extern "C" int sy_bn_finalize(const float* sum, const float* sqsum, int C, int copies, double count, const float* gamma,
-                              const float* beta, float eps, float momentum, float* running_mean, float* running_var,
-                              float* scale, float* shift, float* mean, float* invstd, int nseg, void* stream) {
+static int bn_finalize_any(const float* sum, const float* sqsum, const unsigned* poison, int C, int copies, double count, const float* gamma,
+                           const float* beta, float eps, float momentum, float* running_mean, float* running_var,
+                           float* scale, float* shift, float* mean, float* invstd, int nseg, void* stream) {
     if (sum == nullptr || sqsum == nullptr || gamma == nullptr || beta == nullptr || scale == nullptr ||
         shift == nullptr || C <= 0 || copies <= 0 || count <= 0.0)
         return SY_ERR_ARG;
     if ((running_mean == nullptr) != (running_var == nullptr)) return SY_ERR_ARG;
     if (nseg < 1 || (nseg > 1 && running_mean != nullptr)) return SY_ERR_ARG;
     int read = copies;
-    if (copies > kFoldAbove) {
+    if (copies > kFoldAbove && poison == nullptr) {
         SY_LAUNCH(fold_rows_kernel, dim3((C + 63) / 64, kFoldTo, 2 * nseg), dim3(kBlock), 0, stream, const_cast<float*>(sum),
                   const_cast<float*>(sqsum), C, copies);
         read = kFoldTo;
     }
     SY_LAUNCH(bn_finalize_kernel, dim3((C + 31) / 32, nseg), dim3(kBlock), 0, stream, sum, sqsum, C, read, copies, count,
-              gamma, beta, eps, momentum, running_mean, running_var, scale, shift, mean, invstd);
+              gamma, beta, eps, momentum, running_mean, running_var, scale, shift, mean, invstd, poison);
     return SY_LAUNCH_OK() == 0 ? SY_OK : SY_ERR_LAUNCH;
+}
+extern "C" int sy_bn_finalize(const float* sum, const float* sqsum, int C, int copies, double count, const float* gamma,
+                              const float* beta, float eps, float momentum, float* running_mean, float* running_var,
+                              float* scale, float* shift, float* mean, float* invstd, int nseg, void* stream) {
+    return bn_finalize_any(sum, sqsum, nullptr, C, copies, count, gamma, beta, eps, momentum, running_mean, running_var, scale, shift,
+                           mean, invstd, nseg, stream);
+}
+extern "C" int sy_bn_finalize_fixed(const void* sum, const void* sqsum, const uint32_t* poison, int C, int copies, double count,
+                                    const float* gamma, const float* beta, float eps, float momentum, float* running_mean,
+                                    float* running_var, float* scale, float* shift, float* mean, float* invstd, int nseg,
+                                    void* stream) {
+    if (poison == nullptr || (((uintptr_t)sum | (uintptr_t)sqsum) & 7) != 0) return SY_ERR_ARG;
+    return bn_finalize_any((const float*)sum, (const float*)sqsum, poison, C, copies, count, gamma, beta, eps, momentum, running_mean,
+                           running_var, scale, shift, mean, invstd, nseg, stream);
 }
 
 extern "C" int sy_bn_running_update(const sy_bn_running_entry* entries, int n_entries, int max_C, void* stream) {
@@ -808,10 +860,10 @@
                                        (typename T::elem*)out, ldo, (long long)pixels, C));
 }
 
-extern "C" int sy_bn_finalize_apply(const float* sum, const float* sqsum, int copies, double count, const float* gamma,
-                                    const float* beta, float eps, float* scale, float* shift, float* mean, float* invstd,
-                                    const void* y, int ldy, const void* res, int ldr, void* out, int ldo, int64_t pixels, int C,
-                                    int dtype, int nseg, void* stream) {
+static int bn_finalize_apply_any(const float* sum, const float* sqsum, const unsigned* poison, int copies, double count, const float* gamma,
+                                 const float* beta, float eps, float* scale, float* shift, float* mean, float* invstd,
+                                 const void* y, int ldy, const void* res, int ldr, void* out, int ldo, int64_t pixels, int C,
+                                 int dtype, int nseg, void* stream) {
     if (sum == nullptr || sqsum == nullptr || gamma == nullptr || beta == nullptr || scale == nullptr || shift == nullptr ||
         mean == nullptr || invstd == nullptr || y == nullptr || out == nullptr || copies <= 0 || count <= 0.0 || pixels <= 0 ||
         C <= 0 || nseg < 1)
@@ -829,12 +881,27 @@
     SY_DISPATCH_DTYPE(dtype, SY_LAUNCH((bn_finalize_apply_kernel<T>), dim3(row_grid(pixels, CS, e, cap), nseg, nsl), dim3(kBlock), 0,
                                        stream, sum, sqsum, copies, count, gamma, beta, eps, scale, shift, mean, invstd,
                                        (const typename T::elem*)y, ldy, (const typename T::elem*)res, ldr,
-                                       (typename T::elem*)out, ldo, (long long)pixels, C, CS));
-}
-
-extern "C" int sy_bn_silu_bwd_reduce(const void* y, int ldy, const void* da, int ldda, const float* scale,
-                                     const float* shift, const float* mean, const float* invstd, float* sums,
-                                     int copies, int64_t pixels, int C, int dtype, int nseg, void* stream) {
+                                       (typename T::elem*)out, ldo, (long long)pixels, C, CS, poison));
+}
+extern "C" int sy_bn_finalize_apply(const float* sum, const float* sqsum, int copies, double count, const float* gamma,
+                                    const float* beta, float eps, float* scale, float* shift, float* mean, float* invstd,
+                                    const void* y, int ldy, const void* res, int ldr, void* out, int ldo, int64_t pixels, int C,
+                                    int dtype, int nseg, void* stream) {
+    return bn_finalize_apply_any(sum, sqsum, nullptr, copies, count, gamma, beta, eps, scale, shift, mean, invstd, y, ldy, res, ldr, out,
+                                 ldo, pixels, C, dtype, nseg, stream);
+}
+extern "C" int sy_bn_finalize_apply_fixed(const void* sum, const void* sqsum, const uint32_t* poison, int copies, double count,
+                                          const float* gamma, const float* beta, float eps, float* scale, float* shift, float* mean,
+                                          float* invstd, const void* y, int ldy, const void* res, int ldr, void* out, int ldo,
+                                          int64_t pixels, int C, int dtype, int nseg, void* stream) {
+    if (poison == nullptr || (((uintptr_t)sum | (uintptr_t)sqsum) & 7) != 0) return SY_ERR_ARG;
+    return bn_finalize_apply_any((const float*)sum, (const float*)sqsum, poison, copies, count, gamma, beta, eps, scale, shift, mean,
+                                 invstd, y, ldy, res, ldr, out, ldo, pixels, C, dtype, nseg, stream);
+}
+
+static int bn_silu_bwd_reduce_any(const void* y, int ldy, const void* da, int ldda, const float* scale,
+                                  const float* shift, const float* mean, const float* invstd, float* sums, unsigned* poison,
+                                  int copies, int64_t pixels, int C, int dtype, int nseg, void* stream) {
     if (y == nullptr || da == nullptr || sums == nullptr || pixels <= 0 || C <= 0 || copies <= 0 || nseg < 1) return SY_ERR_ARG;
     const int e = epc_of(dtype);
     if (C % e || ldy % e || ldda % e) return SY_ERR_UNSUPPORTED;
@@ -847,33 +914,64 @@
     const int nsl = C / CS;
     int cap = cap_reduce / (nseg * nsl);
     if (cap < 1) cap = 1;
-    SY_DISPATCH_DTYPE(dtype, SY_LAUNCH((bn_silu_bwd_reduce_kernel<T>), dim3(row_grid(pixels, CS, e, cap), nseg, nsl), dim3(kBlock), 0, stream,
+    const int gx = row_grid(pixels, CS, e, cap);
+    if (poison != nullptr && gx > kFixMaxAdders) return SY_ERR_UNSUPPORTED;
+    SY_DISPATCH_DTYPE(dtype, SY_LAUNCH((bn_silu_bwd_reduce_kernel<T>), dim3(gx, nseg, nsl), dim3(kBlock), 0, stream,
                                        (const typename T::elem*)y, ldy, (const typename T::elem*)da, ldda, scale, shift,
-                                       mean, invstd, sums, (long long)pixels, C, CS, copies));
-}
-
+                                       mean, invstd, sums, (long long)pixels, C, CS, copies, poison));
+}
+extern "C" int sy_bn_silu_bwd_reduce(const void* y, int ldy, const void* da, int ldda, const float* scale,
+                                     const float* shift, const float* mean, const float* invstd, float* sums,
+                                     int copies, int64_t pixels, int C, int dtype, int nseg, void* stream) {
+    return bn_silu_bwd_reduce_any(y, ldy, da, ldda, scale, shift, mean, invstd, sums, nullptr, copies, pixels, C, dtype, nseg, stream);
+}
+extern "C" int sy_bn_silu_bwd_reduce_fixed(const void* y, int ldy, const void* da, int ldda, const float* scale,
+                                           const float* shift, const float* mean, const float* invstd, void* sums, uint32_t* poison,
+                                           int copies, int64_t pixels, int C, int dtype, int nseg, void* stream) {
+    if (poison == nullptr || ((uintptr_t)sums & 7) != 0) return SY_ERR_ARG;
+    return bn_silu_bwd_reduce_any(y, ldy, da, ldda, scale, shift, mean, invstd, (float*)sums, poison, copies, pixels, C, dtype, nseg, stream);
+}
+
+static int bn_silu_bwd_apply_any(const void* y, int ldy, const void* da, int ldda, const float* scale,
+                                 const float* shift, const float* mean, const float* invstd, const float* gamma,
+                                 const float* sums, const unsigned* poison, int copies, void* dy, int lddy, int64_t pixels, int C,
+                                 float* dgamma, float* dbeta, void* dres, int lddres, int dres_accumulate, int dtype,
+                                 int nseg, void* stream) {
+    if (y == nullptr || da == nullptr || sums == nullptr || dy == nullptr || pixels <= 0 || C <= 0 || copies <= 0 || nseg < 1)
+        return SY_ERR_ARG;
+    const long long seg_sum_stride = (long long)copies * 2 * C * (poison != nullptr ? 2 * kFixBins : 1);
+    if (poison != nullptr && (dres_accumulate & 4)) return SY_ERR_UNSUPPORTED;
+    if ((dgamma == nullptr) != (dbeta == nullptr)) return SY_ERR_ARG;
+    const int e = epc_of(dtype);
+    if (C % e || ldy % e || ldda % e || lddy % e || (dres != nullptr && lddres % e)) return SY_ERR_UNSUPPORTED;
+    if (!chunk_rows_ok(C, e) || C > 1024) return SY_ERR_UNSUPPORTED;
+    static const int fold_inline = env_cap("SY_BN_FOLD_INLINE", 2);
+    if (copies > fold_inline && poison == nullptr) {
+        SY_LAUNCH(fold_replicas_kernel, dim3((2 * C + 63) / 64, nseg), dim3(kBlock), 0, stream,
+                  const_cast<float*>(sums), 2 * C, copies);
+        copies = 1;
+    }
+    const int cap_bapply = bn_cap(kCapBApply).load(std::memory_order_relaxed);
+    SY_DISPATCH_DTYPE(dtype, SY_LAUNCH((bn_silu_bwd_apply_kernel<T>), dim3(row_grid(pixels, C, e, cap_bapply / nseg), nseg), dim3(kBlock), 0, stream,
+                                       (const typename T::elem*)y, ldy, (const typename T::elem*)da, ldda, scale, shift,
+                                       mean, invstd, gamma, sums, (typename T::elem*)dy, lddy, (long long)pixels, C, copies,
+                                       dgamma, dbeta, seg_sum_stride, (typename T::elem*)dres, lddres, dres_accumulate, poison));
+}
 extern "C" int sy_bn_silu_bwd_apply(const void* y, int ldy, const void* da, int ldda, const float* scale,
                                     const float* shift, const float* mean, const float* invstd, const float* gamma,
                                     const float* sums, int copies, void* dy, int lddy, int64_t pixels, int C,
                                     float* dgamma, float* dbeta, void* dres, int lddres, int dres_accumulate, int dtype,
                                     int nseg, void* stream) {
-    if (y == nullptr || da == nullptr || sums == nullptr || dy == nullptr || pixels <= 0 || C <= 0 || copies <= 0 || nseg < 1)
-        return SY_ERR_ARG;
-    const long long seg_sum_stride = (long long)copies * 2 * C;
-    if ((dgamma == nullptr) != (dbeta == nullptr)) return SY_ERR_ARG;
-    const int e = epc_of(dtype);
-    if (C % e || ldy % e || ldda % e || lddy % e || (dres != nullptr && lddres % e)) return SY_ERR_UNSUPPORTED;
-    if (!chunk_rows_ok(C, e) || C > 1024) return SY_ERR_UNSUPPORTED;
-    static const int fold_inline = env_cap("SY_BN_FOLD_INLINE", 2);
-    if (copies > fold_inline) {
-        SY_LAUNCH(fold_replicas_kernel, dim3((2 * C + 63) / 64, nseg), dim3(kBlock), 0, stream,
-                  const_cast<float*>(sums), 2 * C, copies);
-        copies = 1;
-    }
-    const int cap_bapply = bn_cap(kCapBApply).load(std::memory_order_relaxed);
-    SY_DISPATCH_DTYPE(dtype, SY_LAUNCH((bn_silu_bwd_apply_kernel<T>), dim3(row_grid(pixels, C, e, cap_bapply / nseg), nseg), dim3(kBlock), 0, stream,
-                                       (const typename T::elem*)y, ldy, (const typename T::elem*)da, ldda, scale, shift,
-                                       mean, invstd, gamma, sums, (typename T::elem*)dy, lddy, (long long)pixels, C, copies,
-                                       dgamma, dbeta, seg_sum_stride, (typename T::elem*)dres, lddres, dres_accumulate));
+    return bn_silu_bwd_apply_any(y, ldy, da, ldda, scale, shift, mean, invstd, gamma, sums, nullptr, copies, dy, lddy, pixels, C, dgamma,
+                                 dbeta, dres, lddres, dres_accumulate, dtype, nseg, stream);
+}
+extern "C" int sy_bn_silu_bwd_apply_fixed(const void* y, int ldy, const void* da, int ldda, const float* scale,
+                                          const float* shift, const float* mean, const float* invstd, const float* gamma,
+                                          const void* sums, const uint32_t* poison, int copies, void* dy, int lddy, int64_t pixels,
+                                          int C, float* dgamma, float* dbeta, void* dres, int lddres, int dres_accumulate, int dtype,
+                                          int nseg, void* stream) {
+    if (poison == nullptr || ((uintptr_t)sums & 7) != 0) return SY_ERR_ARG;
+    return bn_silu_bwd_apply_any(y, ldy, da, ldda, scale, shift, mean, invstd, gamma, (const float*)sums, poison, copies, dy, lddy, pixels,
+                                 C, dgamma, dbeta, dres, lddres, dres_accumulate, dtype, nseg, stream);
 }
 SY_PROBE_READER(sy_probe_read_train_ops)
diff --git a/streamyolo_amd/ops.py b/streamyolo_amd/ops.py
--- a/streamyolo_amd/ops.py
+++ b/streamyolo_amd/ops.py
@@ -117,7 +117,12 @@
     d.scale, d.shift = _p(scale), _p(shift)
     d.res = None if res is None else res.ptr()
     d.stat_sum, d.stat_sqsum = (None, None) if stats is None else (stats[0].data_ptr(), stats[1].data_ptr())
+    if stats is not None and stats[0].dtype == torch.int64:
+        assert bn_reduce is None and len(stats) == 3 and stats[2].dtype == torch.int32
+        d.stat_fixed, d.stat_poison = 1, stats[2].data_ptr()
     d.stat_copies = 1 if stats is None else max(1, stats[0].numel() // ((2 if bn_reduce is not None else 1) * segments * (y.C if cout is None else cout)))
+    if d.stat_fixed:
+        d.stat_copies = max(1, d.stat_copies // fix_bins())
     d.stat_segments = segments
     d.N, d.H, d.W, d.Cin = x.N, x.H, x.W, x.C
     if y is not None:
@@ -300,16 +305,34 @@
 
 
 def bn_finalize(ssum, ssq, count, gamma, beta, eps, momentum, running_mean, running_var, scale, shift, mean, invstd,
-                nseg=1):
+                nseg=1, poison=None):
     C_ = gamma.numel()
+    if poison is not None:
+        assert ssum.dtype == torch.int64 and ssq.dtype == torch.int64
+        check(_lib.lib().sy_bn_finalize_fixed(ssum.data_ptr(), ssq.data_ptr(), poison.data_ptr(), C_, ssum.numel() // (nseg * C_ * fix_bins()),
+                                              float(count), gamma.data_ptr(), beta.data_ptr(), float(eps), float(momentum),
+                                              _p(running_mean), _p(running_var), scale.data_ptr(), shift.data_ptr(), _p(mean),
+                                              _p(invstd), nseg, stream_of(ssum)), "sy_bn_finalize_fixed")
+        return
+    assert ssum.dtype == torch.float32
     check(_lib.lib().sy_bn_finalize(ssum.data_ptr(), ssq.data_ptr(), C_, ssum.numel() // (nseg * C_), float(count),
                                     gamma.data_ptr(), beta.data_ptr(), float(eps), float(momentum), _p(running_mean),
                                     _p(running_var), scale.data_ptr(), shift.data_ptr(), _p(mean), _p(invstd), nseg,
                                     stream_of(ssum)), "sy_bn_finalize")
 
 
-def bn_finalize_apply(ssum, ssq, count, gamma, beta, eps, scale, shift, mean, invstd, y, out, res=None, nseg=1):
+def bn_finalize_apply(ssum, ssq, count, gamma, beta, eps, scale, shift, mean, invstd, y, out, res=None, nseg=1, poison=None):
     C_ = gamma.numel()
+    if poison is not None:
+        assert ssum.dtype == torch.int64 and ssq.dtype == torch.int64
+        check(_lib.lib().sy_bn_finalize_apply_fixed(ssum.data_ptr(), ssq.data_ptr(), poison.data_ptr(), ssum.numel() // (nseg * C_ * fix_bins()),
+                                                    float(count), gamma.data_ptr(), beta.data_ptr(), float(eps), scale.data_ptr(),
+                                                    shift.data_ptr(), mean.data_ptr(), invstd.data_ptr(), y.ptr(), y.ld,
+                                                    None if res is None else res.ptr(), 0 if res is None else res.ld, out.ptr(),
+                                                    out.ld, y.pixels // nseg, y.C, y.dtype, nseg, stream_of(y.buf)),
+              "sy_bn_finalize_apply_fixed")
+        return
+    assert ssum.dtype == torch.float32
     check(_lib.lib().sy_bn_finalize_apply(ssum.data_ptr(), ssq.data_ptr(), ssum.numel() // (nseg * C_), float(count),
                                           gamma.data_ptr(), beta.data_ptr(), float(eps), scale.data_ptr(), shift.data_ptr(),
                                           mean.data_ptr(), invstd.data_ptr(), y.ptr(), y.ld,
@@ -328,6 +351,11 @@
             for j, call in enumerate(calls):
                 ssum, ssq, count = call[:3]
                 e.sum[j], e.sqsum[j], e.count[j] = ssum.data_ptr(), ssq.data_ptr(), float(count)
+                if len(call) > 5 and call[5] is not None:
+                    assert ssum.dtype == torch.int64 and ssq.dtype == torch.int64
+                    e.fixed, e.poison[j] = 1, call[5].data_ptr()
+                else:
+                    assert ssum.dtype == torch.float32
             e.C = bn.num_features
             e.copies = calls[0][3] if len(calls[0]) > 3 else calls[0][0].numel() // e.C
             e.ld = calls[0][4] if len(calls[0]) > 4 else 0
@@ -366,6 +394,31 @@
     return dict(zip(BN_CAP_NAMES, [int(v) for v in g4]))
 
 
+_fix_layout = []
+
+
+def fix_layout():
+    if not _fix_layout:
+        s3 = (C.c_int32 * 3)()
+        check(_lib.lib().sy_fix_layout(s3), "sy_fix_layout")
+        _fix_layout.extend(int(v) for v in s3)
+    return tuple(_fix_layout)
+
+
+def fix_bins():
+    return fix_layout()[0]
+
+
+def fix_units():
+    bins, bits, lo = fix_layout()
+    return torch.tensor([2.0 ** (lo + b * bits - 23) for b in range(bins)], dtype=torch.float64)
+
+
+def fix_value(words, copies, C_):
+    w = words.detach().cpu().view(-1, copies, fix_bins(), C_).sum(1).double()
+    return (w * fix_units().view(1, -1, 1)).flip(1).sum(1)
+
+
 def zero(t):
     esz = t.element_size()
     if t.is_contiguous():
@@ -384,7 +437,15 @@
                                       out.ld, y.pixels // nseg, y.C, y.dtype, nseg, stream_of(y.buf)), "sy_bn_silu_apply")
 
 
-def bn_silu_bwd_reduce(y, da, scale, shift, mean, invstd, sums, nseg=1):
+def bn_silu_bwd_reduce(y, da, scale, shift, mean, invstd, sums, nseg=1, poison=None):
+    if poison is not None:
+        assert sums.dtype == torch.int64
+        check(_lib.lib().sy_bn_silu_bwd_reduce_fixed(y.ptr(), y.ld, da.ptr(), da.ld, scale.data_ptr(), shift.data_ptr(),
+                                                     mean.data_ptr(), invstd.data_ptr(), sums.data_ptr(), poison.data_ptr(),
+                                                     sums.numel() // (2 * y.C * nseg * fix_bins()), y.pixels // nseg, y.C, y.dtype, nseg,
+                                                     stream_of(y.buf)), "sy_bn_silu_bwd_reduce_fixed")
+        return
+    assert sums.dtype == torch.float32
     check(_lib.lib().sy_bn_silu_bwd_reduce(y.ptr(), y.ld, da.ptr(), da.ld, scale.data_ptr(), shift.data_ptr(),
                                            mean.data_ptr(), invstd.data_ptr(), sums.data_ptr(),
                                            sums.numel() // (2 * y.C * nseg), y.pixels // nseg, y.C, y.dtype, nseg,
@@ -392,14 +453,24 @@
 
 
 def bn_silu_bwd_apply(y, da, scale, shift, mean, invstd, gamma, sums, dy, dgamma=None, dbeta=None, nseg=1,
-                      dres=None, dres_accumulate=False, atomic_param_grads=False, raw_moment=False):
+                      dres=None, dres_accumulate=False, atomic_param_grads=False, raw_moment=False, poison=None):
     assert dres is None or (dres.C == y.C and dres.pixels == y.pixels)
+    flags = (1 if dres_accumulate else 0) | (2 if atomic_param_grads else 0) | (4 if raw_moment else 0)
+    if poison is not None:
+        assert sums.dtype == torch.int64
+        check(_lib.lib().sy_bn_silu_bwd_apply_fixed(y.ptr(), y.ld, da.ptr(), da.ld, scale.data_ptr(), shift.data_ptr(),
+                                                    mean.data_ptr(), invstd.data_ptr(), gamma.data_ptr(), sums.data_ptr(),
+                                                    poison.data_ptr(), sums.numel() // (2 * y.C * nseg * fix_bins()), dy.ptr(), dy.ld,
+                                                    y.pixels // nseg, y.C, _p(dgamma), _p(dbeta),
+                                                    None if dres is None else dres.ptr(), 0 if dres is None else dres.ld, flags,
+                                                    y.dtype, nseg, stream_of(y.buf)), "sy_bn_silu_bwd_apply_fixed")
+        return
+    assert sums.dtype == torch.float32
     check(_lib.lib().sy_bn_silu_bwd_apply(y.ptr(), y.ld, da.ptr(), da.ld, scale.data_ptr(), shift.data_ptr(),
                                           mean.data_ptr(), invstd.data_ptr(), gamma.data_ptr(), sums.data_ptr(),
                                           sums.numel() // (2 * y.C * nseg), dy.ptr(), dy.ld, y.pixels // nseg, y.C,
                                           _p(dgamma), _p(dbeta), None if dres is None else dres.ptr(),
-                                          0 if dres is None else dres.ld,
-                                          (1 if dres_accumulate else 0) | (2 if atomic_param_grads else 0) | (4 if raw_moment else 0), y.dtype, nseg,
+                                          0 if dres is None else dres.ld, flags, y.dtype, nseg,
                                           stream_of(y.buf)), "sy_bn_silu_bwd_apply")
 
 
diff --git a/streamyolo_amd/train_engine.py b/streamyolo_amd/train_engine.py
--- a/streamyolo_amd/train_engine.py
+++ b/streamyolo_amd/train_engine.py
@@ -14,6 +14,7 @@
 BNR_FUSION = __import__("os").environ.get("STREAMYOLO_BNR_FUSION", "0") != "0"
 BNR_TILES = (98, 100, 101, 109, 104, 107, 117, 118)
 EXACT_STATS = __import__("os").environ.get("STREAMYOLO_EXACT_STATS", "1") != "0"
+FIXED_STATS = __import__("os").environ.get("STREAMYOLO_FIXED_STATS", "1") != "0"
 BN_BAPPLY_BLOCKS_SCHEDULED = 512
 
 
@@ -276,20 +277,28 @@
         convs = [op for op in self.ops if op.kind == "conv"]
         tot_c = sum(op.y.C for op in convs)
         self.exact_stats = EXACT_STATS
+        self.fixed_stats = self.exact_stats and FIXED_STATS and self.dtype != ops.DT_F32 and not BNR_FUSION
         self.stat_copies = self.STAT_COPIES if self.STAT_COPIES > 0 else (32 if self.dtype == ops.DT_F32 else 4)
-        self.fused_finalize = ((_FUSED_FINALIZE == "1") or (_FUSED_FINALIZE == "auto" and self.dtype != ops.DT_F32)) and not self.exact_stats
+        self.fused_finalize = (((_FUSED_FINALIZE == "1") or (_FUSED_FINALIZE == "auto" and self.dtype != ops.DT_F32))
+                               and (self.fixed_stats or not self.exact_stats))
         reduce_cap = _schedule_bn_caps()
 
         def copies_of(op):
-            if not self.exact_stats:
+            if not self.exact_stats or self.fixed_stats:
                 return self.stat_copies, self.BWD_COPIES
             return max(self.stat_copies, op.y.N * op.y.H * ((op.y.W + 31) // 32)), max(self.BWD_COPIES, reduce_cap)
         for op in convs:
             op.stat_copies, op.bwd_copies = copies_of(op)
-        self.stat_arena = torch.zeros(2 * sum(op.stat_copies * op.y.C for op in convs), dtype=torch.float32, device=device)
-        self.bwd_arena = torch.zeros(2 * sum(op.bwd_copies * op.y.C for op in convs), dtype=torch.float32, device=device)
+        sdt = torch.int64 if self.fixed_stats else torch.float32
+        K = ops.fix_bins() if self.fixed_stats else 1
+        n_stat, n_bwd = 2 * K * sum(op.stat_copies * op.y.C for op in convs), 2 * K * sum(op.bwd_copies * op.y.C for op in convs)
+        n_poison = (tot_c + 1) // 2 if self.fixed_stats else 0
+        self.stat_arena = torch.zeros(n_stat + n_poison, dtype=sdt, device=device)
+        self.bwd_arena = torch.zeros(n_bwd + n_poison, dtype=sdt, device=device)
+        self.stat_poison = self.stat_arena[n_stat:].view(torch.int32) if self.fixed_stats else None
+        self.bwd_poison = self.bwd_arena[n_bwd:].view(torch.int32) if self.fixed_stats else None
         self.aff_arena = torch.empty(4 * tot_c, dtype=torch.float32, device=device)
-        sq0 = self.stat_arena.numel() // 2
+        sq0 = n_stat // 2
         off = 0
         max_raw = 0
         nf = self.n_frame_ops
@@ -304,21 +313,26 @@
         s_off = b_off = 0
         for unit in units:
             C, S = unit[0].y.C, len(unit)
-            SC, BC = unit[0].stat_copies, unit[0].bwd_copies
+            SC, BC = unit[0].stat_copies * K, unit[0].bwd_copies * K
             u_sum = self.stat_arena[s_off:s_off + SC * S * C]
             u_sq = self.stat_arena[sq0 + s_off:sq0 + s_off + SC * S * C]
             u_bsum = self.bwd_arena[b_off:b_off + 2 * BC * S * C]
             s_off += SC * S * C
             b_off += 2 * BC * S * C
             u_aff = tuple(self.aff_arena[k * tot_c + off:k * tot_c + off + S * C] for k in range(4))
+            u_poison = (self.stat_poison[off:off + S * C], self.bwd_poison[off:off + S * C]) if self.fixed_stats else (None, None)
             for s_, op in enumerate(unit):
                 op.stat = (u_sum[s_ * SC * C:(s_ + 1) * SC * C], u_sq[s_ * SC * C:(s_ + 1) * SC * C])
+                op.poison = tuple(None if t is None else t[s_ * C:(s_ + 1) * C] for t in u_poison)
+                if self.fixed_stats:
+                    op.stat = op.stat + (op.poison[0],)
                 op.bsum = u_bsum[s_ * 2 * BC * C:(s_ + 1) * 2 * BC * C]
                 op.aff = tuple(t[s_ * C:(s_ + 1) * C] for t in u_aff)
                 if op.yraw is None:
                     op.yraw = View.alloc(op.y.N, op.y.H, op.y.W, C, self.dtype, device)
                 max_raw = max(max_raw, 2 * op.y.pixels * C)
             unit[0].unit = (u_sum, u_sq, u_bsum, u_aff)
+            unit[0].unit_poison = u_poison
             off += S * C
         self.max_raw = max_raw
         self._bind_scratch()
@@ -434,7 +448,8 @@
                 if op.kind == "conv":
                     c0, ctot, SC = 0, op.y.C, (32 if op.stat_copies > 64 else op.stat_copies)
                     for m in base_convs(op.mod):
-                        mods.setdefault(id(m.bn), (m.bn, []))[1].append((op.stat[0][c0:], op.stat[1][c0:], op.y.pixels, SC, ctot))
+                        mods.setdefault(id(m.bn), (m.bn, []))[1].append((op.stat[0][c0:], op.stat[1][c0:], op.y.pixels, SC, ctot,
+                                                                         None if op.poison[0] is None else op.poison[0][c0:]))
                         c0 += m.bn.num_features
             self.run_table = ops.BnRunningTable(list(mods.values()), self.device, count_batches=True)
         self.run_table.run()
@@ -523,10 +538,11 @@
 
     def _bn_bwd(self, op, y, da, aff, gamma, bsum, dy, dgamma, dbeta, nseg=1, dres=None, acc=False, atomic=False):
         fused = getattr(op, "bnr_by", None) is not None
+        poison = (op.unit_poison[1] if nseg > 1 else op.poison[1]) if self.fixed_stats else None
         if not fused:
-            ops.bn_silu_bwd_reduce(y, da, *aff, bsum, nseg=nseg)
+            ops.bn_silu_bwd_reduce(y, da, *aff, bsum, nseg=nseg, poison=poison)
         ops.bn_silu_bwd_apply(y, da, *aff, gamma, bsum, dy, dgamma, dbeta, nseg=nseg, dres=dres, dres_accumulate=acc,
-                              atomic_param_grads=atomic, raw_moment=fused)
+                              atomic_param_grads=atomic, raw_moment=fused, poison=poison)
 
     def _bnr_producer(self, op, dx, acc, t):
         pre = op.pre_op
@@ -549,14 +565,15 @@
             t = ops.tuned_tile(ops.CONV_FWD, x2.dtype, x2.N, x2.H, x2.W, x2.C, y2.C, a.k, a.stride, self.device,
                                with_stats=True)
             a._tiles["fwd_stats2"] = t
-        ops.conv2d(x2, self.cache.conv_weight(a.mod), raw2, a.k, a.stride, stats=(u_sum, u_sq), tile=t,
-                   wfrag=self.cache.conv_weight_frag(a.mod) if t >= ops.TILE_WR else None, segments=2)
+        ps = a.unit_poison[0]
+        ops.conv2d(x2, self.cache.conv_weight(a.mod), raw2, a.k, a.stride, stats=(u_sum, u_sq) if ps is None else (u_sum, u_sq, ps),
+                   tile=t, wfrag=self.cache.conv_weight_frag(a.mod) if t >= ops.TILE_WR else None, segments=2)
         if self.fused_finalize:
             ops.bn_finalize_apply(u_sum, u_sq, a.y.pixels, gamma, beta, eps, scale, shift, mean, invstd, raw2, y2,
-                                  res=None if a.res is None else a.res.pair(), nseg=2)
+                                  res=None if a.res is None else a.res.pair(), nseg=2, poison=ps)
         else:
             ops.bn_finalize(u_sum, u_sq, a.y.pixels, gamma, beta, eps, mom, None, None, scale, shift, mean, invstd,
-                            nseg=2)
+                            nseg=2, poison=ps)
             ops.bn_silu_apply(raw2, scale, shift, y2, res=None if a.res is None else a.res.pair(), nseg=2)
 
     def _mark(self, kind, arg=None):
@@ -626,10 +643,10 @@
                        wfrag=self.cache.conv_weight_frag(op.mod) if t >= ops.TILE_WR else None)
             if self.fused_finalize:
                 ops.bn_finalize_apply(op.stat[0], op.stat[1], op.y.pixels, gamma, beta, eps, scale, shift, mean, invstd,
-                                      op.yraw, op.y, res=op.res)
+                                      op.yraw, op.y, res=op.res, poison=op.poison[0])
             else:
                 ops.bn_finalize(op.stat[0], op.stat[1], op.y.pixels, gamma, beta, eps, mom,
-                                None, None, scale, shift, mean, invstd)
+                                None, None, scale, shift, mean, invstd, poison=op.poison[0])
                 ops.bn_silu_apply(op.yraw, scale, shift, op.y, res=op.res)
         elif k == "resize":
             ops.resize_nearest(op.src, op.dst)
```

Result: slower. 348.7 frame-pairs/s (-1.4%).
